# LeapLabTHU/LAUDNet

Hardware: AMD Instinct MI355X
Metric: images/sec, LAUD-ResNet101 @224 bs256 (dynamic-inference hot path) (higher is better)
Workload: dtype bf16x3 (fp32 tensors; each fp32 product = 3 bf16 MFMA products of hi/lo splits, fp32 accumulate)

## Files before the change

include/ldn_hip.h:

```cpp
#ifndef LDN_HIP_H
#define LDN_HIP_H

#include <stddef.h>
#include <stdint.h>

#ifdef __cplusplus
extern "C" {
#endif

#define LDN_OK 0
#define LDN_EINVAL (-1)
#define LDN_EHIP (-2)

const char* ldn_last_error(void);
int ldn_version(void);
int ldn_debug_violations(int* count, int* first_code, int reset);
int ldn_plan_timeouts(int* count, int reset);
const int* ldn_fault_flag(void);
int ldn_device_cus(int* cus);
#define LDN_MATH_DEFAULT (-1)
#define LDN_MATH_FP32 0
#define LDN_MATH_BF16X3 1
int ldn_default_math_mode(void);

int ldn_spatial_masker(const float* x, int B, int Hi, int Wi, int C, const float* w ,
                       const float* bias , int g, int S, float* mask, float* logits, float* work,
                       const int32_t* carry_prefix, const float* carry_mask, void* stream);
size_t ldn_spatial_masker_workspace_bytes(int B, int Hi, int Wi, int C, int S);

int ldn_mask_to_index(const float* patch_mask, int B, int Sy, int Sx, int Ho, int Wo, int stride, int32_t* idx3,
                      int32_t* pos3, int32_t* idx1, int32_t* pos1, int32_t* nbr, int32_t* cnt,
                      int32_t* img_prefix3, int32_t* img_prefix1, float* stats, int32_t* work, void* stream);
size_t ldn_mask_to_index_workspace_bytes(int B, int Ho, int Wo, int stride);
int ldn_plan_work_zeroed(int yes);
int ldn_coarsen_cell_means(const float* fine, int B, int S, int C, float* coarse, void* stream);

int ldn_layer_index(const float* image_mask, int B, int Ho, int Wo, int stride, int tile_gy, int tile_gx, int32_t* idx3,
                    int32_t* pos3, int32_t* idx1, int32_t* pos1, int32_t* nbr, int32_t* cnt, int32_t* img_prefix3,
                    int32_t* img_prefix1, float* stats, void* stream);
int ldn_layer_head(const float* pool, int B, int nparts, int C, const float* w , const float* bias , int g,
                   float* mask , float* logits , void* stream);
int ldn_mask_plan_fits(int S, int Sx, int Ho, int Wo, int stride);
int ldn_mask_plan(const float* patch_mask, const float* pool, int C, const float* w, const float* bias, float* mask_out,
                  float* logits, int B, int S, int Sx, int Ho, int Wo, int stride, int patch_major, int32_t* idx3,
                  int32_t* pos3, int32_t* idx1, int32_t* pos1, int32_t* nbr, int32_t* cnt, int32_t* img_prefix3,
                  int32_t* img_prefix1, float* stats, int32_t* work, void* stream);

int ldn_gather_rows(const float* src, int ld_src, const int32_t* rows, const int32_t* count, int cap, int C,
                    float* packed, int ld_packed, void* stream);
int ldn_scatter_add_relu(const float* packed, int ld_packed, const int32_t* rows, const int32_t* count, int cap,
                         int C, const float* identity, int ld_id, float* out, int ld_out, void* stream);

int ldn_conv_rows(const float* a, int lda, const int32_t* a_rows, int taps, const int32_t* m_count, int m_cap,
                  const float* w, int cin, int cout, const float* scale, const float* shift, int relu,
                  const int32_t* relu_if_neg, const int32_t* out_rows, const float* residual, int ldr,
                  float* out, int ldo, int math_mode, void* stream);

int ldn_conv_rows_split(const float* a, int lda, const int32_t* a_rows, int taps, const int32_t* m_count, int m_cap,
                        const void* w_split, int cin, int cout, const float* scale, const float* shift, int relu,
                        const int32_t* relu_if_neg, const int32_t* out_rows, const float* residual, int ldr, float* out,
                        int ldo, const float* post_sub, const float* chan_mask, int rows_per_image, int shift_classes,
                        const int32_t* pix_map, int Hi, int Wi, int Ho, int Wo, int stride, const float* ln_stats,
                        const float* ln_c1, void* stream);
int ldn_conv_rows_f32(const float* a, int lda, const int32_t* a_rows, int taps, const int32_t* m_count, int m_cap,
                        const float* w, int cin, int cout, const float* scale, const float* shift, int relu,
                        const int32_t* relu_if_neg, const int32_t* out_rows, const float* residual, int ldr, float* out,
                        int ldo, const float* post_sub, const float* chan_mask, int rows_per_image, int shift_classes,
                        const int32_t* pix_map, int Hi, int Wi, int Ho, int Wo, int stride, const float* ln_stats,
                        const float* ln_c1, void* stream);

int ldn_hint_rows(int rows);

int ldn_wgrad_rows_ok(int cin, int cout, int taps);
size_t ldn_wgrad_rows_workspace_bytes(int m_cap, int cin, int cout, int taps);
int ldn_wgrad_rows(const float* dy, int lddy, const float* a, int lda, int a_valid, const int32_t* a_rows, int taps,
                   const int32_t* m_count, int m_cap, int cin, int cout, float* dw, float* work, int math_mode, void* stream);

int ldn_wgrad_grouped_rows_ok(int C, int gw);
size_t ldn_wgrad_grouped_rows_workspace_bytes(int m_cap, int C, int gw);
int ldn_wgrad_grouped_rows(const float* dy, int lddy, const float* a, int lda, int a_valid, const int32_t* nbr, const int32_t* m_count,
                           int m_cap, int C, int gw, float* dw, float* work, int math_mode, void* stream);

int ldn_rows_chanmask(float* u, int ldu, const int32_t* row_prefix, int B, const float* chan_mask, const int32_t* m_count, int m_cap,
                      int C, void* stream);

size_t ldn_rows_act_bwd_workspace_bytes(int m_cap, int C, int B);
int ldn_rows_act_bwd(const float* dh, int lddh, const float* u, int ldu, const float* post_sub, const float* scale, const float* shift,
                     const float* chan_mask, const int32_t* row_prefix, int B, const float* zy, int ldzy, const int32_t* m_count,
                     int m_cap, int C, float* du, int lddu, float* g_shift, float* g_scale_num, float* g_mask, float* work,
                     void* stream);

int ldn_conv_rows_pool(const float* a, int lda, const int32_t* a_rows, const int32_t* m_count, int m_cap, const void* w,
                       int cin, int cout, const float* scale, const float* shift, int relu, const int32_t* relu_if_neg,
                       const int32_t* out_rows, const float* residual, int ldr, float* out, int ldo, float* pool, int S,
                       int Sx, int Ho, int Wo, int math_mode, void* stream);

int ldn_conv_rows_ps(const float* a, int lda, int a_presplit, const int32_t* a_rows, const int32_t* m_count, int m_cap,
                     const void* w_split, int cin, int cout, const float* scale, const float* shift, int relu,
                     const int32_t* relu_if_neg, const int32_t* out_rows, const float* residual, int ldr, float* out, int ldo,
                     int out_presplit, float* pool, int S, int Sx, int Ho, int Wo, void* stream);
int ldn_conv3x3_rows_ps(const void* a_presplit, int lda, const int32_t* nbr, const int32_t* m_count, int m_cap, const void* w_split,
                        int cin, int cout, const float* scale, const float* shift, int relu, void* out, int ldo, int out_presplit,
                        int rows_hint, void* stream);
int ldn_row_stats(const float* x, int ld, int rows, int C, float eps, float* stats, void* stream);
int ldn_row_stats_list(const float* x, int ld, int rows, int C, float eps, const int32_t* list, const int32_t* count, float* stats,
                       void* stream);

int ldn_channel_masker_splits(int HW);
int ldn_channel_masker(const float* x, int B, int HW, int C, const float* w1, const float* b1, const float* w2,
                       const float* b2, int hidden, int G, int gran, const float* mask_in, float* mask,
                       float* logits, int32_t* ch_idx, int32_t* ch_cnt, float* work, const float* gap_partial,
                       int gap_splits, void* stream);
size_t ldn_channel_masker_workspace_bytes(int B, int HW, int C);

int ldn_forward_stats(const int32_t* cnt, int B, const float* denom, const float* st_in, int st_cols, const double* terms,
                      double static_flops, int n_blocks, float* st_out, float* perc, float* flops, void* stream);

int ldn_conv_image(const float* a, int lda, int B, int Hi, int Wi, int ksize, int stride, int Ho, int Wo,
                   const float* w, int cin, int cout, const int32_t* k_idx, const int32_t* k_cnt, int kgran,
                   const int32_t* n_idx, const int32_t* n_cnt, const float* scale, const float* shift,
                   int shift_classes, const float* post_sub, int relu, const float* residual, int ldr,
                   float* out, int ldo, float* colsum, int out_format, int math_mode, void* stream);

int ldn_bottleneck_head(const float* x, int ldx, int B, int HW, int cin, const void* w1_split, int width,
                        const int32_t* ch_idx, const int32_t* ch_cnt, const float* scale1, const float* shift1,
                        const float* post_sub1, void* h1_split, int ldh, void* stream);
int ldn_bottleneck_head_f32(const float* x, int ldx, int B, int HW, int cin, const float* w1, int width,
                            const int32_t* ch_idx, const int32_t* ch_cnt, const float* scale1, const float* shift1,
                            const float* post_sub1, float* h1, int ldh, void* stream);
int ldn_bottleneck_tail_f32(const void* h1, int ldh, int B, int H, int Wd, int stride, int width, const void* w2_pairs_f32,
                            const void* w3_pairs_f32, int cout, const int32_t* ch_idx, const int32_t* ch_cnt, const float* scale2,
                            const float* shift2_tab, const float* post_sub2, const float* shift3, const float* residual,
                            int ldr, float* out, int ldo, float* colsum, void* stream);
int ldn_bottleneck_tail_splits(int H, int Wd, int width, int stride);
int ldn_bottleneck_tail(const void* h1_split, int ldh, int B, int H, int Wd, int stride, int width, const void* w2_pairs,
                        const void* w3_pairs, int cout, const int32_t* ch_idx, const int32_t* ch_cnt, const float* scale2,
                        const float* shift2_tab, const float* post_sub2, const float* shift3, const float* residual,
                        int ldr, float* out, int ldo, float* colsum, void* stream);
size_t ldn_x_split_bytes(size_t pixels, int cin);
int ldn_bottleneck_head_split(const float* x, int ldx, int B, int HW, int cin, const void* w1_split, int width,
                              const int32_t* ch_idx, const int32_t* ch_cnt, const float* scale1, const float* shift1,
                              const float* post_sub1, void* h1_split, int ldh, void* x_split, void* stream);
int ldn_bottleneck_tail_proj_fits(int H, int Wd, int width, int cin);
int ldn_bottleneck_tail_proj(const void* h1_split, int ldh, int B, int H, int Wd, int width, const void* w2_pairs,
                             const void* w3_pairs, int cout, const int32_t* ch_idx, const int32_t* ch_cnt, const float* scale2,
                             const float* shift2_tab, const float* post_sub2, const float* shift3d, const void* x_split,
                             int cin, const void* wd_pairs, float* out, int ldo, float* colsum, void* stream);

int ldn_bottleneck_smallmap_fits(int H, int Wd, int cin, int width, int cout);
int ldn_bottleneck_smallmap(const float* x, int ldx, int B, int H, int Wd, int cin, int width, const void* w1_split,
                            const void* w2_pairs, const void* w3_pairs, int cout, const int32_t* ch_idx, const int32_t* ch_cnt,
                            const float* scale1, const float* shift1, const float* post_sub1, const float* scale2,
                            const float* shift2_tab, const float* post_sub2, const float* shift3, const float* residual, int ldr,
                            float* out, int ldo, float* colsum, void* stream);

typedef struct ldn_chain_block {
    const void* w1_split; const float* scale1; const float* shift1; const float* post_sub1;
    const void* w2_pairs; const void* w3_pairs; const float* scale2; const float* shift2_tab; const float* post_sub2;
    const float* shift3;
    const float* mw1; const float* mb1; const float* mw2; const float* mb2;
} ldn_chain_block;
int ldn_bottleneck_chain_fits(int H, int Wd, int C, int width, int hidden, int G);
int ldn_bottleneck_chain(const float* x_in, float* x_work, int ldx, int B, int H, int Wd, int C, int width,
                         const ldn_chain_block* blocks, int nblocks, int hidden, int G, int gran, const float* gap_in,
                         int gap_splits, float* colsum, float* masks, int32_t* ch_idx, int32_t* ch_cnt, void* h1_split,
                         int ldh, void* stream);
int ldn_bottleneck_chain_f32(const float* x_in, float* x_work, int ldx, int B, int H, int Wd, int C, int width,
                         const ldn_chain_block* blocks, int nblocks, int hidden, int G, int gran, const float* gap_in,
                         int gap_splits, float* colsum, float* masks, int32_t* ch_idx, int32_t* ch_cnt, float* h1,
                         int ldh, void* stream);

size_t ldn_stem_weight_bytes(int cout);
int ldn_stem_conv_pool(const float* x, int B, int H, int W, const void* w_frag, const float* shift, int cout, float* out,
                       int Hp, int Wp, void* stream);
int ldn_stem_gap_splits(int H, int W);
int ldn_stem_conv_pool_gap(const float* x, int B, int H, int W, const void* w_frag, const float* shift, int cout,
                           float* out, int Hp, int Wp, float* gap, void* stream);

size_t ldn_stem3_weight_bytes(int cout);
int ldn_stem3_conv(const float* x, int B, int H, int W, const void* w_frag, const float* shift, int cout, int relu, float* out,
                   int Ho, int Wo, void* stream);

int ldn_conv_packed(const float* a, int lda, int B, const int32_t* row_prefix, const int32_t* m_count, int m_cap,
                    const int32_t* a_map, int taps, const int32_t* out_map, const int32_t* pix_map, int Hi, int Wi,
                    int Ho, int Wo, int stride, const float* w, int cin, int cout, const int32_t* k_idx,
                    const int32_t* k_cnt, int kgran, const int32_t* n_idx, const int32_t* n_cnt, const float* scale,
                    const float* shift, int shift_classes, const float* post_sub, int relu,
                    const int32_t* relu_if_neg, const float* residual, int ldr, float* out, int ldo, int math_mode,
                    void* stream);

int ldn_grouped_conv3x3_rows(const float* a, int lda, const int32_t* nbr, const int32_t* m_count, int m_cap,
                             const float* w, int C, int group_width, const float* scale, const float* shift, int relu,
                             float* out, int ldo, void* stream);
size_t ldn_grouped16_weight_bytes(int C);
int ldn_grouped16_conv3x3_rows(const float* a, int lda, const int32_t* nbr, const int32_t* m_count, int m_cap,
                               const void* w_frag, int C, const float* scale, const float* shift, int relu, float* out,
                               int ldo, void* stream);

int ldn_grouped16_images_fit(int Hi, int Wi, int C);
int ldn_grouped16_conv3x3_images(const float* a, int lda, const int32_t* m_count, int images_cap, int Hi, int Wi, int Ho, int Wo,
                                 int stride, const void* w_frag, int C, const float* scale, const float* shift, int relu, float* out,
                                 int ldo, void* stream);
int ldn_grouped_conv3x3_image(const float* a, int lda, int B, int Hi, int Wi, int stride, int Ho, int Wo, const float* w,
                              int C, int group_width, const int32_t* ch_idx, const int32_t* ch_cnt, const float* scale,
                              const float* shift, int relu, float* out, int ldo, void* stream);
int ldn_se_packed(float* a, int lda, const int32_t* row_prefix, int B, int C, int S, const float* w1, const float* b1,
                  const float* w2, const float* b2, const int32_t* ch_idx, const int32_t* ch_cnt, int max_rows_per_image,
                  float* work, void* stream);
size_t ldn_se_packed_workspace_bytes(int B, int C, int max_rows_per_image);

int ldn_grouped16_images_bands(int Hi, int Wi, int Ho, int stride, int C);
int ldn_grouped16_conv3x3_images_gap(const float* a, int lda, const int32_t* m_count, int images_cap, int Hi, int Wi, int Ho, int Wo,
                                     int stride, const void* w_frag, int C, const float* scale, const float* shift, int relu, float* out,
                                     int ldo, float* gap_partial, void* stream);
int ldn_se_gate_slots(const float* gap_partial, int splits, const int32_t* m_count, int images_cap, int rows_per_image, int C, int S,
                      const float* w1, const float* b1, const float* w2, const float* b2, float* gate, void* stream);
int ldn_conv_rows_gated(const float* a, int lda, const int32_t* m_count, int m_cap, const void* w_split, int cin, int cout,
                        const float* scale, const float* shift, int relu, const int32_t* relu_if_neg, const int32_t* out_rows,
                        const float* residual, int ldr, float* out, int ldo, const float* gate, int gate_rows, void* stream);

int ldn_packed_mha(const float* qkv, int ld_qkv, const int32_t* tok_rows, const int32_t* img_prefix, int B, int heads,
                   int head_dim, int max_tokens, float scale, float* out, int ldo, void* stream);
int ldn_packed_mha_heads(const float* qkv, int ld_qkv, const int32_t* tok_rows, const int32_t* img_prefix, int B, int heads,
                         int head_dim, int max_tokens, float scale, const float* head_keep, float* out, int ldo, void* stream);

#ifdef __cplusplus
}
#endif
#endif
```

laudnet_amd/_lib.py:

```python
from __future__ import annotations

import ctypes as C
import os

import torch

_PKG = os.path.dirname(os.path.abspath(__file__))
LIB_PATH = os.environ.get("LDN_LIB_PATH", os.path.join(_PKG, "libldn_hip.so"))

_P = C.c_void_p
_I = C.c_int

SIGNATURES = {
    "ldn_last_error": ([], C.c_char_p),
    "ldn_version": ([], _I),
    "ldn_debug_violations": ([C.POINTER(_I), C.POINTER(_I), _I], _I),
    "ldn_plan_timeouts": ([C.POINTER(_I), _I], _I),
    "ldn_fault_flag": ([], C.POINTER(_I)),
    "ldn_device_cus": ([C.POINTER(_I)], _I),
    "ldn_default_math_mode": ([], _I),
    "ldn_spatial_masker": ([_P, _I, _I, _I, _I, _P, _P, _I, _I, _P, _P, _P, _P, _P, _P], _I),
    "ldn_spatial_masker_workspace_bytes": ([_I, _I, _I, _I, _I], C.c_size_t),
    "ldn_mask_to_index": ([_P, _I, _I, _I, _I, _I, _I, _P, _P, _P, _P, _P, _P, _P, _P, _P, _P, _P], _I),
    "ldn_mask_to_index_workspace_bytes": ([_I, _I, _I, _I], C.c_size_t),
    "ldn_mask_plan_fits": ([_I, _I, _I, _I, _I], _I),
    "ldn_hint_rows": ([_I], _I),
    "ldn_layer_index": ([_P, _I, _I, _I, _I, _I, _I, _P, _P, _P, _P, _P, _P, _P, _P, _P, _P], _I),
    "ldn_layer_head": ([_P, _I, _I, _I, _P, _P, _I, _P, _P, _P], _I),
    "ldn_mask_plan": ([_P, _P, _I, _P, _P, _P, _P, _I, _I, _I, _I, _I, _I, _I, _P, _P, _P, _P, _P, _P, _P, _P, _P, _P, _P], _I),
    "ldn_conv_rows_pool": ([_P, _I, _P, _P, _I, _P, _I, _I, _P, _P, _I, _P, _P, _P, _I, _P, _I, _P, _I, _I, _I, _I, _I, _P], _I),
    "ldn_conv_rows_ps": ([_P, _I, _I, _P, _P, _I, _P, _I, _I, _P, _P, _I, _P, _P, _P, _I, _P, _I, _I, _P, _I, _I, _I, _I, _P], _I),
    "ldn_conv3x3_rows_ps": ([_P, _I, _P, _P, _I, _P, _I, _I, _P, _P, _I, _P, _I, _I, _I, _P], _I),
    "ldn_gather_rows": ([_P, _I, _P, _P, _I, _I, _P, _I, _P], _I),
    "ldn_scatter_add_relu": ([_P, _I, _P, _P, _I, _I, _P, _I, _P, _I, _P], _I),
    "ldn_conv_rows": ([_P, _I, _P, _I, _P, _I, _P, _I, _I, _P, _P, _I, _P, _P, _P, _I, _P, _I, _I, _P], _I),
    "ldn_conv_rows_split": ([_P, _I, _P, _I, _P, _I, _P, _I, _I, _P, _P, _I, _P, _P, _P, _I, _P, _I, _P, _P, _I, _I, _P, _I, _I, _I,
                             _I, _I, _P, _P, _P], _I),
    "ldn_conv_rows_f32": ([_P, _I, _P, _I, _P, _I, _P, _I, _I, _P, _P, _I, _P, _P, _P, _I, _P, _I, _P, _P, _I, _I, _P, _I, _I, _I,
                             _I, _I, _P, _P, _P], _I),
    "ldn_wgrad_rows_ok": ([_I, _I, _I], _I),
    "ldn_wgrad_rows_workspace_bytes": ([_I, _I, _I, _I], C.c_size_t),
    "ldn_wgrad_rows": ([_P, _I, _P, _I, _I, _P, _I, _P, _I, _I, _I, _P, _P, _I, _P], _I),
    "ldn_wgrad_grouped_rows_ok": ([_I, _I], _I),
    "ldn_wgrad_grouped_rows_workspace_bytes": ([_I, _I, _I], C.c_size_t),
    "ldn_wgrad_grouped_rows": ([_P, _I, _P, _I, _I, _P, _P, _I, _I, _I, _P, _P, _I, _P], _I),
    "ldn_rows_chanmask": ([_P, _I, _P, _I, _P, _P, _I, _I, _P], _I),
    "ldn_rows_act_bwd_workspace_bytes": ([_I, _I, _I], C.c_size_t),
    "ldn_rows_act_bwd": ([_P, _I, _P, _I, _P, _P, _P, _P, _P, _I, _P, _I, _P, _I, _I, _P, _I, _P, _P, _P, _P, _P], _I),
    "ldn_row_stats": ([_P, _I, _I, _I, C.c_float, _P, _P], _I),
    "ldn_row_stats_list": ([_P, _I, _I, _I, C.c_float, _P, _P, _P, _P], _I),
    "ldn_channel_masker_splits": ([_I], _I),
    "ldn_channel_masker": ([_P, _I, _I, _I, _P, _P, _P, _P, _I, _I, _I, _P, _P, _P, _P, _P, _P, _P, _I, _P], _I),
    "ldn_channel_masker_workspace_bytes": ([_I, _I, _I], C.c_size_t),
    "ldn_forward_stats": ([_P, _I, _P, _P, _I, _P, C.c_double, _I, _P, _P, _P, _P], _I),
    "ldn_conv_packed": ([_P, _I, _I, _P, _P, _I, _P, _I, _P, _P, _I, _I, _I, _I, _I, _P, _I, _I, _P, _P, _I, _P, _P, _P, _P,
                         _I, _P, _I, _P, _P, _I, _P, _I, _I, _P], _I),
    "ldn_grouped_conv3x3_rows": ([_P, _I, _P, _P, _I, _P, _I, _I, _P, _P, _I, _P, _I, _P], _I),
    "ldn_grouped16_weight_bytes": ([_I], C.c_size_t),
    "ldn_grouped16_conv3x3_rows": ([_P, _I, _P, _P, _I, _P, _I, _P, _P, _I, _P, _I, _P], _I),
    "ldn_grouped16_images_fit": ([_I, _I, _I], _I),
    "ldn_grouped16_conv3x3_images": ([_P, _I, _P, _I, _I, _I, _I, _I, _I, _P, _I, _P, _P, _I, _P, _I, _P], _I),
    "ldn_plan_work_zeroed": ([_I], _I),
    "ldn_coarsen_cell_means": ([_P, _I, _I, _I, _P, _P], _I),
    "ldn_grouped16_images_bands": ([_I, _I, _I, _I, _I], _I),
    "ldn_grouped16_conv3x3_images_gap": ([_P, _I, _P, _I, _I, _I, _I, _I, _I, _P, _I, _P, _P, _I, _P, _I, _P, _P], _I),
    "ldn_se_gate_slots": ([_P, _I, _P, _I, _I, _I, _I, _P, _P, _P, _P, _P, _P], _I),
    "ldn_conv_rows_gated": ([_P, _I, _P, _I, _P, _I, _I, _P, _P, _I, _P, _P, _P, _I, _P, _I, _P, _I, _P], _I),
    "ldn_grouped_conv3x3_image": ([_P, _I, _I, _I, _I, _I, _I, _I, _P, _I, _I, _P, _P, _P, _P, _I, _P, _I, _P], _I),
    "ldn_se_packed": ([_P, _I, _P, _I, _I, _I, _P, _P, _P, _P, _P, _P, _I, _P, _P], _I),
    "ldn_se_packed_workspace_bytes": ([_I, _I, _I], C.c_size_t),
    "ldn_conv_image": ([_P, _I, _I, _I, _I, _I, _I, _I, _I, _P, _I, _I, _P, _P, _I, _P, _P, _P, _P, _I, _P, _I,
                        _P, _I, _P, _I, _P, _I, _I, _P], _I),
    "ldn_bottleneck_head": ([_P, _I, _I, _I, _I, _P, _I, _P, _P, _P, _P, _P, _P, _I, _P], _I),
    "ldn_bottleneck_head_f32": ([_P, _I, _I, _I, _I, _P, _I, _P, _P, _P, _P, _P, _P, _I, _P], _I),
    "ldn_bottleneck_tail_splits": ([_I, _I, _I, _I], _I),
    "ldn_bottleneck_tail": ([_P, _I, _I, _I, _I, _I, _I, _P, _P, _I, _P, _P, _P, _P, _P, _P, _P, _I, _P, _I, _P, _P], _I),
    "ldn_bottleneck_tail_f32": ([_P, _I, _I, _I, _I, _I, _I, _P, _P, _I, _P, _P, _P, _P, _P, _P, _P, _I, _P, _I, _P, _P], _I),
    "ldn_x_split_bytes": ([C.c_size_t, _I], C.c_size_t),
    "ldn_bottleneck_head_split": ([_P, _I, _I, _I, _I, _P, _I, _P, _P, _P, _P, _P, _P, _I, _P, _P], _I),
    "ldn_bottleneck_tail_proj_fits": ([_I, _I, _I, _I], _I),
    "ldn_bottleneck_tail_proj": ([_P, _I, _I, _I, _I, _I, _P, _P, _I, _P, _P, _P, _P, _P, _P, _P, _I, _P, _P, _I, _P, _P], _I),
    "ldn_stem_weight_bytes": ([_I], C.c_size_t),
    "ldn_stem_conv_pool": ([_P, _I, _I, _I, _P, _P, _I, _P, _I, _I, _P], _I),
    "ldn_stem_gap_splits": ([_I, _I], _I),
    "ldn_stem_conv_pool_gap": ([_P, _I, _I, _I, _P, _P, _I, _P, _I, _I, _P, _P], _I),
    "ldn_stem3_weight_bytes": ([_I], C.c_size_t),
    "ldn_stem3_conv": ([_P, _I, _I, _I, _P, _P, _I, _I, _P, _I, _I, _P], _I),
    "ldn_packed_mha": ([_P, _I, _P, _P, _I, _I, _I, _I, C.c_float, _P, _I, _P], _I),
    "ldn_packed_mha_heads": ([_P, _I, _P, _P, _I, _I, _I, _I, C.c_float, _P, _P, _I, _P], _I),
    "ldn_bottleneck_chain_fits": ([_I, _I, _I, _I, _I, _I], _I),
    "ldn_bottleneck_smallmap_fits": ([_I, _I, _I, _I, _I], _I),
    "ldn_bottleneck_smallmap": ([_P, _I, _I, _I, _I, _I, _I, _P, _P, _P, _I, _P, _P, _P, _P, _P, _P, _P, _P, _P, _P, _I, _P, _I, _P, _P], _I),
    "ldn_bottleneck_chain": ([_P, _P, _I, _I, _I, _I, _I, _I, _P, _I, _I, _I, _I, _P, _I, _P, _P, _P, _P, _P, _I, _P], _I),
    "ldn_bottleneck_chain_f32": ([_P, _P, _I, _I, _I, _I, _I, _I, _P, _I, _I, _I, _I, _P, _I, _P, _P, _P, _P, _P, _I, _P], _I),
}

_lib = None


class LdnError(RuntimeError):
    pass


def load():
    global _lib
    if _lib is not None:
        return _lib
    if not os.path.exists(LIB_PATH):
        raise LdnError(f"{LIB_PATH} not found: build it with `python -m laudnet_amd.build` "
                       "(laudnet_amd has no CPU or PyTorch fallback for the hot path)")
    lib = C.CDLL(LIB_PATH)
    for name, (argtypes, restype) in SIGNATURES.items():
        fn = getattr(lib, name)
        fn.argtypes = argtypes
        fn.restype = restype
    _lib = lib
    return lib


def ptr(t):
    if t is None:
        return None
    return C.c_void_p(t.data_ptr())


def stream_ptr(t=None):
    return C.c_void_p(torch.cuda.current_stream(t.device if t is not None else None).cuda_stream)


_SYNC_CALLS = os.environ.get("LDN_SYNC_CALLS", "0") != "0"
_n_calls = 0


_fault = None


def _arm_fault_flag():
    global _fault
    if _fault is None:
        p = load().ldn_fault_flag()
        _fault = p if p else False


def check(status: int, what: str, fault_ok: bool = False):
    if status != 0:
        msg = load().ldn_last_error()
        raise LdnError(f"{what} failed ({status}): {msg.decode() if msg else '?'}")
    if _fault and not fault_ok and _fault[0] != 0:
        raise LdnError(f"{what}: a device-side bounded wait ran into its time bound since the last reset -- results computed since are "
                       "invalid (ops.plan_timeouts() counts the events, ops.plan_timeouts(reset=True) re-arms)")
    if _SYNC_CALLS:
        global _n_calls
        import sys
        import torch
        _n_calls += 1
        print(f"[ldn] {_n_calls} {what} ...", end="", file=sys.stderr, flush=True)
        if torch.cuda.is_current_stream_capturing():
            print(" (capturing)", file=sys.stderr, flush=True)
            return
        torch.cuda.synchronize()
        print(" ok", file=sys.stderr, flush=True)


def require_device(*tensors):
    cur = None
    for t in tensors:
        if t is None:
            continue
        if not t.is_cuda:
            raise LdnError("laudnet_amd ops need tensors on a HIP device (cuda:N); there is no CPU path")
        if cur is None:
            cur = torch.cuda.current_device()
            if _fault is None:
                _arm_fault_flag()
        if t.device.index != cur:
            raise LdnError(f"tensor on {t.device} but the current device is cuda:{cur}: wrap the call in "
                           f"torch.cuda.device({t.device.index}) (kernels are launched on the current device's stream)")
```

laudnet_amd/csrc/ldn_chain_ld.h:

```cpp
#pragma once
#include "ldn_common.h"

namespace ldn {

#ifndef LDN_LD_PRIO
#define LDN_LD_PRIO 0
#endif
#ifndef LDN_LD_R2MAX
#define LDN_LD_R2MAX 4
#endif
#ifndef LDN_LD3_ABLATE
#define LDN_LD3_ABLATE 0
#endif
#ifndef LDN_LD3_DEFER
#define LDN_LD3_DEFER 0
#endif
#ifndef LDN_LD3_STORE_STEP
#define LDN_LD3_STORE_STEP 1
#endif
#ifndef LDN_LD2_STAGED
#define LDN_LD2_STAGED 0
#endif
#ifndef LDN_LD3_STAGED
#define LDN_LD3_STAGED 1
#endif

constexpr int LD_SYNC_OFF = T_KIDX_BYTES;
constexpr int LD_SYNC_BYTES = 256;
constexpr int LD_LOADER = 7;
constexpr int LD_SPIN_LIMIT = 1 << 20;

__device__ unsigned g_ld_stalls = 0u;
__device__ int* g_ld_fault_dev = nullptr;
#ifdef LDN_TRACE
__device__ unsigned long long* g_ld_trace = nullptr;
#define LT(x) x = __builtin_amdgcn_s_memtime();
#define LD_TIMED(slot, stmt) { const unsigned long long t0_ = __builtin_amdgcn_s_memtime(); stmt; q.t[slot] += __builtin_amdgcn_s_memtime() - t0_; }
#define LD_SPAN(slot, a, b) q.t[slot] += (b) - (a);
#else
#define LT(x)
#define LD_TIMED(slot, stmt) { stmt; }
#define LD_SPAN(slot, a, b)
#endif

struct LdSync {
    unsigned landed;
    unsigned pad0[15];
    unsigned done[16];
    unsigned pad1[32];
};
static_assert(sizeof(LdSync) == LD_SYNC_BYTES, "LdSync layout");

struct LdSeq {
    unsigned base;
    unsigned seen;
#ifdef LDN_TRACE
    unsigned long long t[8];
#endif
};

__device__ __forceinline__ unsigned ld_lds_read(const unsigned* p) {
    unsigned v;
    asm volatile("ds_read_b32 %0, %1\n\ts_waitcnt lgkmcnt(0)" : "=&v"(v) : "v"(lds_off(p)) : "memory");
    return v;
}
__device__ __forceinline__ void ld_lds_write(unsigned* p, unsigned v) {
    asm volatile("ds_write_b32 %0, %1\n\ts_nop 0" ::"v"(lds_off(p)), "v"(v) : "memory");
}

__device__ __forceinline__ void ld_wait_landed(LdSync* sy, unsigned need, unsigned& seen) {
    if (seen >= need) return;
    for (int spin = 0;; ++spin) {
        seen = __builtin_amdgcn_readfirstlane(ld_lds_read(&sy->landed));
        if (seen >= need) break;
        if (spin >= LD_SPIN_LIMIT) {
            if ((threadIdx.x & 63) == 0) {
                atomicAdd(&g_ld_stalls, 1u);
                if (g_ld_fault_dev) __hip_atomic_store(g_ld_fault_dev, 1, __ATOMIC_RELAXED, __HIP_MEMORY_SCOPE_SYSTEM);
            }
            seen = 0x7fffffffu;
            break;
        }
        __builtin_amdgcn_s_sleep(2);
    }
}
__device__ __forceinline__ void ld_post_done(LdSync* sy, int wave, unsigned seq_plus_1) {
    asm volatile("" ::: "memory");
    if ((threadIdx.x & 63) == 0) ld_lds_write(&sy->done[wave], seq_plus_1);
    asm volatile("" ::: "memory");
}
__device__ __forceinline__ void ld_wait_done(LdSync* sy, int ncomp, unsigned need, bool& dead) {
    if (dead) return;
    const int lane = threadIdx.x & 63;
    for (int spin = 0;; ++spin) {
        const unsigned v = ld_lds_read(&sy->done[lane & 15]);
        if (__ballot(lane < ncomp && v < need) == 0ull) break;
        if (spin >= LD_SPIN_LIMIT) {
            if (lane == 0) {
                atomicAdd(&g_ld_stalls, 1u);
                if (g_ld_fault_dev) __hip_atomic_store(g_ld_fault_dev, 1, __ATOMIC_RELAXED, __HIP_MEMORY_SCOPE_SYSTEM);
            }
            dead = true;
            break;
        }
        __builtin_amdgcn_s_sleep(2);
    }
}
#ifdef LDN_DEBUG
__device__ int g_chain_stall = -1;
#endif
__device__ __forceinline__ void ld_publish(LdSync* sy, unsigned landed) {
#ifdef LDN_DEBUG
    if ((int)blockIdx.x == g_chain_stall) return;
#endif
    asm volatile("" ::: "memory");
    if ((threadIdx.x & 63) == 0) ld_lds_write(&sy->landed, landed);
    asm volatile("" ::: "memory");
}


__device__ __forceinline__ u32x4 ld_global16(const unsigned char* sbase, unsigned off) {
    typedef const __attribute__((address_space(1))) u32x4* gptr;
    return *(gptr)(sbase + off);
}

__device__ __forceinline__ f32x4 ld_global_f4(const float* ptr) {
    typedef const __attribute__((address_space(1))) f32x4* gptr;
    return *(gptr)(ptr);
}

__device__ __forceinline__ unsigned ld_bias(int i) { return (unsigned)(3 - (i & 3)) * 1024u; }
template <int MAXP>
__device__ __forceinline__ void ld_dma_run(const unsigned (&vo)[MAXP], int n, const unsigned char* sbase, unsigned lds_base) {
    const void* sb = uniform_ptr(sbase - 3072);
#pragma unroll
    for (int g = 0; g < MAXP / 4; ++g) {
        if (4 * g >= n) break;
        const unsigned v4[4] = {vo[4 * g], vo[4 * g + 1], vo[4 * g + 2], vo[4 * g + 3]};
        dma16_pieces_abl<4>(v4, sb, (unsigned)__builtin_amdgcn_readfirstlane((int)(lds_base + (unsigned)g * 4096u)));
    }
}

template <int NS>
__device__ __forceinline__ void head_ld(const HeadArgs& p, const int b, unsigned char* const smem, const int lds_total, const int tid, LdSeq& q) {
    constexpr int W = NS * 32;
    constexpr int MAXP = NS * 4;
    int* const s_nidx = reinterpret_cast<int*>(smem);
    LdSync* const sy = reinterpret_cast<LdSync*>(smem + LD_SYNC_OFF);
    float* const s_tab = reinterpret_cast<float*>(smem + LD_SYNC_OFF + LD_SYNC_BYTES);
    unsigned char* const s_ring = smem + LD_SYNC_OFF + LD_SYNC_BYTES + 3 * W * 4;

    const int lane = tid & 63;
    const int wave = __builtin_amdgcn_readfirstlane(tid >> 6);
    const int l31 = lane & 31, h = lane >> 5;
    const int npix = p.HW;
    const long row0 = (long)b * p.HW;
    const int ncomp = ceil_div(npix, 32);

    const int Nb = min(p.n_cnt[b], W);
    const int nsub = __builtin_amdgcn_readfirstlane(ceil_div(Nb, 32));
    const int nwp = __builtin_amdgcn_readfirstlane(4 * max(nsub, 1));
    const int wslot = nwp * 1024;
    if (tid < W + 32) s_nidx[tid] = tid < Nb ? p.n_idx[(size_t)b * W + tid] : -1;
    if (tid < LD_SYNC_BYTES / 4) reinterpret_cast<unsigned*>(sy)[tid] = 0u;
    __syncthreads();
    for (int i = tid; i < 3 * W; i += 512) {
        const int k = i / W, n = i - k * W;
        const int ch = s_nidx[n];
        const float* src = k == 0 ? p.sc1 : (k == 1 ? p.sh1 : p.ps1);
        s_tab[i] = ch >= 0 ? src[ch] : 0.f;
    }
    const int avail = lds_total - (LD_SYNC_OFF + LD_SYNC_BYTES + 3 * W * 4);
    int DX = 3;
    if ((avail - ncomp * DX * 4096) / wslot < 3) DX = 2;
    DX = __builtin_amdgcn_readfirstlane(DX);
    const int RW = __builtin_amdgcn_readfirstlane(min(4, (avail - ncomp * DX * 4096) / wslot));
    unsigned char* const s_x = s_ring + RW * wslot;
    const int nchunks = p.cin / 32;
    const unsigned base = q.base;
    q.base = base + (unsigned)nchunks;
#ifdef LDN_TRACE
    unsigned long long ta, tb, tc;
    LT(ta)
#endif

    if (wave == LD_LOADER) {
        if (nsub == 0) return;
        unsigned wo[MAXP];
#pragma unroll
        for (int i = 0; i < MAXP; ++i) {
            const int rw = 8 * i + (lane >> 3);
            const int ch = s_nidx[min(rw, max(Nb, 1) - 1)];
            wo[i] = (unsigned)(max(ch, 0) * p.cin * 4 + (((lane & 7) ^ ((rw >> 1) & 7)) << 4)) + ld_bias(i);
        }
        const unsigned lds_w = lds_off(s_ring);
        bool dead = false;
        int slot = 0;
        for (int c = 0; c < nchunks; ++c) {
            if (c >= RW) LD_TIMED(5, ld_wait_done(sy, ncomp, base + (unsigned)(c - RW + 1), dead))
            ld_dma_run<MAXP>(wo, nwp, p.w1s + (long)c * 128, lds_w + (unsigned)slot * (unsigned)wslot);
            slot = slot + 1 == RW ? 0 : slot + 1;
            if (c > 0) { wait_vm_rt<62, 63>(nwp); ld_publish(sy, base + (unsigned)c); }
        }
        wait_vm<0>();
        ld_publish(sy, base + (unsigned)nchunks);
        LT(tb)
        LD_SPAN(0, ta, tb)
        return;
    }
    if (wave >= ncomp) return;

    const unsigned lds_x = lds_off(s_x) + (unsigned)wave * (unsigned)(DX * 4096);
    unsigned char* const my_x = s_x + wave * DX * 4096;
    unsigned xo[4];
#pragma unroll
    for (int i = 0; i < 4; ++i) {
        const int rl = 8 * i + (lane >> 3);
        const int r = wave * 32 + rl;
        xo[i] = (unsigned)((min(r, npix - 1) * p.ldx) * 4 + (((lane & 7) ^ ((rl >> 1) & 7)) << 4)) + ld_bias(i);
    }
    const unsigned char* const xbase = reinterpret_cast<const unsigned char*>(p.x + row0 * p.ldx) - 3072;
    auto dma_x = [&](int c, int xs) {
        const int cc = min(c, nchunks - 1);
        dma16_pieces_abl<4>(xo, uniform_ptr(xbase + (long)cc * 128), (unsigned)__builtin_amdgcn_readfirstlane((int)(lds_x + (unsigned)xs * 4096u)));
    };

    f32x16 acc[NS];
#pragma unroll
    for (int j = 0; j < NS; ++j)
#pragma unroll
        for (int r = 0; r < 16; ++r) acc[j][r] = 0.f;

    if (nsub == 0) return;
    for (int c = 0; c < DX - 1; ++c) dma_x(c, c);
    const unsigned xsw = ((unsigned)l31 >> 1) & 7u;
    bf16x8 bh[2], bl[2];
    int xs = 0, ws_i = 0;
    for (int c = 0; c < nchunks; ++c) {
        wait_vm_rt<15, 16>(4 * (DX - 2));
        {
            const unsigned char* xsl = my_x + xs * 4096 + l31 * 128;
#pragma unroll
            for (int half = 0; half < 2; ++half) {
                const unsigned sl = 4u * half + 2u * h;
                const f32x4 x0 = *reinterpret_cast<const f32x4*>(xsl + ((sl ^ xsw) << 4));
                const f32x4 x1 = *reinterpret_cast<const f32x4*>(xsl + (((sl + 1) ^ xsw) << 4));
#pragma unroll
                for (int e = 0; e < 8; ++e) {
                    const float v = e < 4 ? x0[e] : x1[e - 4];
                    const __bf16 hb = (__bf16)v;
                    bh[half][e] = hb;
                    bl[half][e] = (__bf16)(v - (float)hb);
                }
            }
        }
        dma_x(c + DX - 1, xs == 0 ? DX - 1 : xs - 1);
        LD_TIMED(5, ld_wait_landed(sy, base + (unsigned)c + 1u, q.seen))
        const unsigned char* ws = s_ring + ws_i * wslot + l31 * 128;
        bf16x8 a0h, a0l, a1h, a1l;
        const unsigned sl0 = 2u * h, sl1 = 4u + 2u * h;
        auto frag0 = [&](int j) {
            a0h = *reinterpret_cast<const bf16x8*>(ws + j * 4096 + ((sl0 ^ xsw) << 4));
            a0l = *reinterpret_cast<const bf16x8*>(ws + j * 4096 + (((sl0 + 1) ^ xsw) << 4));
        };
        auto frag1 = [&](int j) {
            a1h = *reinterpret_cast<const bf16x8*>(ws + j * 4096 + ((sl1 ^ xsw) << 4));
            a1l = *reinterpret_cast<const bf16x8*>(ws + j * 4096 + (((sl1 + 1) ^ xsw) << 4));
        };
#define LDN_HEADLD_STEP(J)                                                                                \
        frag1(J);                                                                                         \
        __builtin_amdgcn_sched_barrier(0);                                                                \
        LDN_K16(false, acc[J], a0h, a0l, bh[0], bl[0])                                                    \
        __builtin_amdgcn_sched_barrier(0);                                                                \
        if (J > 0) frag0(J > 0 ? J - 1 : 0);                                                              \
        __builtin_amdgcn_sched_barrier(0);                                                                \
        LDN_K16(false, acc[J], a1h, a1l, bh[1], bl[1])                                                    \
        __builtin_amdgcn_sched_barrier(0);
        if (nsub > 0) {
            frag0(nsub - 1);
            switch (nsub) {
                default:
                    if constexpr (NS >= 8) { LDN_HEADLD_STEP(7) }
                    [[fallthrough]];
                case 7:
                    if constexpr (NS >= 8) { LDN_HEADLD_STEP(6) }
                    [[fallthrough]];
                case 6:
                    if constexpr (NS >= 8) { LDN_HEADLD_STEP(5) }
                    [[fallthrough]];
                case 5:
                    if constexpr (NS >= 8) { LDN_HEADLD_STEP(4) }
                    [[fallthrough]];
                case 4:
                    if constexpr (NS >= 4) { LDN_HEADLD_STEP(3) }
                    [[fallthrough]];
                case 3:
                    if constexpr (NS >= 4) { LDN_HEADLD_STEP(2) }
                    [[fallthrough]];
                case 2:
                    LDN_HEADLD_STEP(1)
                    [[fallthrough]];
                case 1:
                    LDN_HEADLD_STEP(0)
            }
        }
#undef LDN_HEADLD_STEP
        ld_post_done(sy, wave, base + (unsigned)c + 1u);
        xs = xs + 1 == DX ? 0 : xs + 1;
        ws_i = ws_i + 1 == RW ? 0 : ws_i + 1;
    }
    wait_vm<0>();
    LT(tb)
    LD_SPAN(0, ta, tb)

    const int pm = wave * 32 + l31;
    unsigned char* orow = p.h1 + (row0 + min(pm, npix - 1)) * p.h1_row_bytes;
#pragma unroll
    for (int j = 0; j < NS; ++j) {
        if (j >= nsub) continue;
#pragma unroll
        for (int q4 = 0; q4 < 4; ++q4) {
            const int n0 = 32 * j + 8 * q4 + 4 * h;
            const f32x4 sc = *reinterpret_cast<const f32x4*>(s_tab + n0);
            const f32x4 sh = *reinterpret_cast<const f32x4*>(s_tab + W + n0);
            const f32x4 ps = *reinterpret_cast<const f32x4*>(s_tab + 2 * W + n0);
            unsigned hi2[2], lo2[2];
#pragma unroll
            for (int d = 0; d < 2; ++d) {
                const float v0 = fmaxf(acc[j][4 * q4 + 2 * d] * sc[2 * d] + sh[2 * d], 0.f) - ps[2 * d];
                const float v1 = fmaxf(acc[j][4 * q4 + 2 * d + 1] * sc[2 * d + 1] + sh[2 * d + 1], 0.f) - ps[2 * d + 1];
                const bf16x2 hh = {(__bf16)v0, (__bf16)v1};
                const bf16x2 ll = {(__bf16)(v0 - (float)hh[0]), (__bf16)(v1 - (float)hh[1])};
                hi2[d] = __builtin_bit_cast(unsigned, hh);
                lo2[d] = __builtin_bit_cast(unsigned, ll);
            }
            u32x4 outv;
#pragma unroll
            for (int d = 0; d < 2; ++d) {
                const auto r = __builtin_amdgcn_permlane32_swap(hi2[d], lo2[d], false, false);
                outv[d] = r[0];
                outv[2 + d] = r[1];
            }
            if (pm < npix) *reinterpret_cast<u32x4*>(orow + (4 * j + q4) * 32 + h * 16) = outv;
        }
    }
    LT(tc)
    LD_SPAN(1, tb, tc)
}

constexpr int LD_CW = 32;
template <int NS>
__device__ __forceinline__ void tail_ld(const TailArgs& p, const int b, unsigned char* const smem, const int lds_total, const int tid, LdSeq& q) {
    constexpr int W = NS * 32;
    constexpr int MAXP = NS * 4;
    constexpr int MAXH = 28;
    constexpr int NP = W;
    constexpr int W3_ROW = LD_CW * 8;
    int* const s_kidx = reinterpret_cast<int*>(smem);
    LdSync* const sy = reinterpret_cast<LdSync*>(smem + LD_SYNC_OFF);
    unsigned char* const s_lo = smem + LD_SYNC_OFF + LD_SYNC_BYTES;
    unsigned char* const s_h1 = s_lo;
    unsigned char* const s_w2 = s_h1 + 2 * p.slice_bytes;
    unsigned char* const s_w3 = s_lo;
    unsigned char* const s_scr = smem + lds_total - 7 * 4096;
    float* const s_tab = reinterpret_cast<float*>(s_scr - 18 * NP * 4);

    int lane = tid & 63;
    const int wave = __builtin_amdgcn_readfirstlane(tid >> 6);
    int l31 = lane & 31, h = lane >> 5;
    const int npix = p.Ho * p.Wo;
    const int ncomp = ceil_div(npix, 32);
    const int NR = npix, NRp = round_up(NR, 8);
    const int ZR = NRp;
    const long pix0 = (long)b * npix;

    const int Kb = min(p.k_cnt[b], W);
    const int nsub = __builtin_amdgcn_readfirstlane(ceil_div(Kb, 32));
    const int Kp = nsub * 32;
    const int P2 = __builtin_amdgcn_readfirstlane(Kp / 8);
    const int slot2 = Kp * 128, slot3 = Kp * 128;
    if (tid < W + 32) s_kidx[tid] = tid < Kb ? p.k_idx[(size_t)b * W + tid] : -1;
    if (tid < 64) reinterpret_cast<float*>(s_h1 + (tid >> 5) * p.slice_bytes + ZR * 128)[tid & 31] = 0.f;
    __syncthreads();

    const int avail2 = lds_total - (LD_SYNC_OFF + LD_SYNC_BYTES) - 2 * p.slice_bytes;
    const int R2 = __builtin_amdgcn_readfirstlane(nsub > 0 ? min(LDN_LD_R2MAX, avail2 / slot2) : LDN_LD_R2MAX);
    const int avail3 = lds_total - (LD_SYNC_OFF + LD_SYNC_BYTES) - 18 * NP * 4 - 7 * 4096;
    const int R3 = __builtin_amdgcn_readfirstlane(nsub > 0 ? min(4, avail3 / slot3) : 4);
    const int nchunks = nsub * 9;
    const int nchunk3 = p.cout / LD_CW;
    const int nq = NRp / 8;
    const unsigned base2 = q.base, base3 = base2 + (unsigned)nchunks;
    q.base = base3 + (unsigned)nchunk3;
    constexpr int TMIN = 3;
    static_assert(TMIN == 3 && MAXH == 28, "the slice schedule below is written out for taps 3 .. 8 and <= 28 pieces");

    const bool loader = wave == LD_LOADER;
    const bool consumer = wave < ncomp;
#ifdef LDN_TRACE
    unsigned long long ta, tb, tc, td;
    LT(ta)
#endif
    bool dead = false;

    f32x16 acc[NS];
    if (loader) {
#if LDN_LD2_STAGED
        constexpr int NH = NS / 2;
        const int nhi = (nsub + 1) / 2;
        unsigned colo[NH];
        unsigned dsto[NH];
        const int hp = max(Kp / 2, 1);
#pragma unroll
        for (int i = 0; i < NH; ++i) {
            const int e = 64 * i + lane;
            const int gh = e / hp, v = e - gh * hp;
            const int ch = 2 * v < Kb ? s_kidx[2 * v] : 0;
            colo[i] = (unsigned)((ch >> 1) * 16);
            dsto[i] = gh < 2 ? ((unsigned)(gh * Kp * 32 + v * 32) | (unsigned)gh) : ~0u;
        }
        unsigned ro[2][NH][4];
        auto slice_rows = [&](int s_) {
#pragma unroll
            for (int hf = 0; hf < 2; ++hf)
#pragma unroll
                for (int i = 0; i < NH; ++i) {
                    const int gh = (int)(dsto[i] & 1u);
#pragma unroll
                    for (int qq = 0; qq < 4; ++qq) {
                        const int kch = s_kidx[32 * s_ + 2 * (8 * hf + 4 * gh + qq)];
                        ro[hf][i][qq] = (unsigned)((max(kch, 0) >> 1) * (W / 2) * 16) + colo[i];
                    }
                }
        };
        u32x4 LA[NH][4], LB[NH][4];
        auto load_half = [&](int t_, int hf, u32x4 (&L_)[NH][4]) {
            const unsigned char* src = reinterpret_cast<const unsigned char*>(uniform_ptr(p.w2p + (long)t_ * ((W / 2) * (W / 2) * 16)));
#pragma unroll
            for (int i = 0; i < NH; ++i)
                if (i < nhi)
#pragma unroll
                    for (int qq = 0; qq < 4; ++qq) L_[i][qq] = ld_global16(src, ro[hf][i][qq]);
        };
        auto store_half = [&](unsigned char* slotp, int hf, const u32x4 (&L_)[NH][4]) {
            const int lo = Kp * 16;
            unsigned char* hb = slotp + hf * (Kp * 64);
#pragma unroll
            for (int i = 0; i < NH; ++i)
                if (i < nhi && dsto[i] != ~0u) {
                    unsigned char* d = hb + (dsto[i] & ~31u);
                    *reinterpret_cast<u32x4*>(d) = u32x4{L_[i][0][0], L_[i][1][0], L_[i][2][0], L_[i][3][0]};
                    *reinterpret_cast<u32x4*>(d + lo) = u32x4{L_[i][0][1], L_[i][1][1], L_[i][2][1], L_[i][3][1]};
                    *reinterpret_cast<u32x4*>(d + 16) = u32x4{L_[i][0][2], L_[i][1][2], L_[i][2][2], L_[i][3][2]};
                    *reinterpret_cast<u32x4*>(d + lo + 16) = u32x4{L_[i][0][3], L_[i][1][3], L_[i][2][3], L_[i][3][3]};
                }
        };
        const unsigned lds_h1 = lds_off(s_h1);
        const unsigned char* const h1b = p.h1 + pix0 * p.h1_row_bytes;
        auto h1_piece = [&](int i, const void* sb, unsigned dst) {
            const int r = 8 * i + (lane >> 3);
            const unsigned o = (unsigned)(min(r, NR - 1) * (int)p.h1_row_bytes + (((lane & 7) ^ ((r >> 1) & 7)) << 4));
            dma16_pieces<1>({o}, sb, (unsigned)__builtin_amdgcn_readfirstlane((int)(dst + (unsigned)i * 1024u)));
        };
        if (nchunks > 0) {
            const void* sb0 = uniform_ptr(h1b);
            for (int i = 0; i < nq; ++i) h1_piece(i, sb0, lds_h1);
            slice_rows(0);
            load_half(0, 0, LA);
            load_half(0, 1, LB);
        }
        int slot = 0;
        int sn = 0, tn = 1;
        for (int c = 0; c < nchunks; ++c) {
            const int sc = c / 9, tc = c - 9 * sc;
            const bool nxt = c + 1 < nchunks;
            if (c >= R2) LD_TIMED(6, ld_wait_done(sy, ncomp, base2 + (unsigned)(c - R2 + 1), dead))
            if (tc == 0) wait_vm<0>();
            unsigned char* const slotp = s_w2 + slot * slot2;
            slot = slot + 1 == R2 ? 0 : slot + 1;
            store_half(slotp, 0, LA);
            if (nxt) {
                if (tn == 0) slice_rows(sn);
                load_half(tn, 0, LA);
            }
            store_half(slotp, 1, LB);
            ld_publish(sy, base2 + (unsigned)c + 1u);
            if (nxt) load_half(tn, 1, LB);
            if (tc >= TMIN && sc + 1 < nsub) {
                const void* hsb = uniform_ptr(h1b + (long)(sc + 1) * 128);
                const unsigned hdst = lds_h1 + (unsigned)((sc + 1) & 1) * (unsigned)p.slice_bytes;
                for (int i = tc - TMIN; i < nq; i += 6) h1_piece(i, hsb, hdst);
            }
            if (++tn == 9) { tn = 0; ++sn; }
        }
#else
        unsigned ho[MAXH];
#pragma unroll
        for (int i = 0; i < MAXH; ++i) {
            const int r = 8 * i + (lane >> 3);
            ho[i] = (unsigned)(min(r, NR - 1) * (int)p.h1_row_bytes + (((lane & 7) ^ ((r >> 1) & 7)) << 4));
        }
        unsigned un[MAXP];
        unsigned no[MAXP];
        const int hp = max(Kp / 2, 1);
#pragma unroll
        for (int i = 0; i < MAXP; ++i) {
            const int e = 64 * i + lane;
            const int u = min(e / hp, 15), v = e - (e / hp) * hp;
            const int ch = 2 * v < Kb ? s_kidx[2 * v] : 0;
            un[i] = (unsigned)u;
            no[i] = (unsigned)((ch >> 1) * 16) + ld_bias(i);
        }
        const unsigned lds_h1 = lds_off(s_h1), lds_w2 = lds_off(s_w2);
        const unsigned char* const h1b = p.h1 + pix0 * p.h1_row_bytes;
        if (nchunks > 0) {
#pragma unroll
            for (int i = 0; i < MAXH; ++i)
                if (i < nq) dma16_pieces<1>({ho[i]}, uniform_ptr(h1b), (unsigned)__builtin_amdgcn_readfirstlane((int)(lds_h1 + (unsigned)i * 1024u)));
        }
        int slot = 0;
        for (int s = 0; s < nsub; ++s) {
            unsigned vo[MAXP];
#pragma unroll
            for (int i = 0; i < MAXP; ++i) {
                const int kch = s_kidx[32 * s + 2 * (int)un[i]];
                vo[i] = (unsigned)((max(kch, 0) >> 1) * (W / 2) * 16) + no[i];
            }
            const unsigned char* const hsrc = h1b + (long)(s + 1) * 128;
            const unsigned hdst = lds_h1 + (unsigned)((s + 1) & 1) * (unsigned)p.slice_bytes;
            const bool more = s + 1 < nsub;
            for (int t = 0; t < 9; ++t) {
                const int c = 9 * s + t;
                if (c >= R2) LD_TIMED(6, ld_wait_done(sy, ncomp, base2 + (unsigned)(c - R2 + 1), dead))
                ld_dma_run<MAXP>(vo, P2, p.w2p + (long)t * ((W / 2) * (W / 2) * 16), lds_w2 + (unsigned)slot * (unsigned)slot2);
                slot = slot + 1 == R2 ? 0 : slot + 1;
                int pieces = P2;
                if (t >= TMIN && more) {
                    const void* hsb = uniform_ptr(hsrc);
#define LDN_LD_H1(I) if ((I) < nq) { dma16_pieces<1>({ho[(I)]}, hsb, (unsigned)__builtin_amdgcn_readfirstlane((int)(hdst + (unsigned)(I) * 1024u))); ++pieces; }
                    switch (t) {
                        case 3: LDN_LD_H1(0) LDN_LD_H1(6) LDN_LD_H1(12) LDN_LD_H1(18) LDN_LD_H1(24) break;
                        case 4: LDN_LD_H1(1) LDN_LD_H1(7) LDN_LD_H1(13) LDN_LD_H1(19) LDN_LD_H1(25) break;
                        case 5: LDN_LD_H1(2) LDN_LD_H1(8) LDN_LD_H1(14) LDN_LD_H1(20) LDN_LD_H1(26) break;
                        case 6: LDN_LD_H1(3) LDN_LD_H1(9) LDN_LD_H1(15) LDN_LD_H1(21) LDN_LD_H1(27) break;
                        case 7: LDN_LD_H1(4) LDN_LD_H1(10) LDN_LD_H1(16) LDN_LD_H1(22) break;
                        default: LDN_LD_H1(5) LDN_LD_H1(11) LDN_LD_H1(17) LDN_LD_H1(23) break;
                    }
#undef LDN_LD_H1
                }
                if (c > 0) { wait_vm_rt<62, 63>(pieces); ld_publish(sy, base2 + (unsigned)c); }
            }
        }
#endif
        wait_vm<0>();
        ld_publish(sy, base2 + (unsigned)nchunks);
        LT(tb)
        LD_SPAN(2, ta, tb)
        __syncthreads();
#if LDN_LD3_STAGED
        unsigned so[NS][4];
#pragma unroll
        for (int i = 0; i < NS; ++i)
#pragma unroll
            for (int qq = 0; qq < 4; ++qq) {
                const int u = 16 * i + 8 * ((lane >> 5) & 1) + 2 * ((lane >> 4) & 1) + (qq & 1) + 4 * (qq >> 1);
                const int kch = 2 * u < Kp ? s_kidx[2 * u] : -1;
                so[i][qq] = (unsigned)(((long)(max(kch, 0) >> 1) * p.cout + 2 * (lane & 15)) * 8);
            }
        u32x4 L[NS][4];
        auto load_chunk = [&](int cc) {
            const unsigned char* src = reinterpret_cast<const unsigned char*>(uniform_ptr(p.w3p + (long)cc * (LD_CW * 8)));
#pragma unroll
            for (int i = 0; i < NS; ++i)
                if (i < nsub)
#pragma unroll
                    for (int qq = 0; qq < 4; ++qq) L[i][qq] = ld_global16(src, so[i][qq]);
        };
        auto store_chunk = [&](unsigned char* slotp) {
#pragma unroll
            for (int i = 0; i < NS; ++i)
                if (i < nsub) {
                    unsigned char* d = slotp + (4 * i + (lane >> 4)) * 1024 + (lane & 15) * 32;
                    *reinterpret_cast<u32x4*>(d) = u32x4{L[i][0][0], L[i][1][0], L[i][2][0], L[i][3][0]};
                    *reinterpret_cast<u32x4*>(d + 512) = u32x4{L[i][0][1], L[i][1][1], L[i][2][1], L[i][3][1]};
                    *reinterpret_cast<u32x4*>(d + 16) = u32x4{L[i][0][2], L[i][1][2], L[i][2][2], L[i][3][2]};
                    *reinterpret_cast<u32x4*>(d + 528) = u32x4{L[i][0][3], L[i][1][3], L[i][2][3], L[i][3][3]};
                }
        };
        if (nchunk3 > 0 && nsub > 0) load_chunk(0);
        __syncthreads();
        if (nsub > 0) {
            int slot3i = 0;
            for (int cc = 0; cc < nchunk3; ++cc) {
                if (cc >= R3) LD_TIMED(7, ld_wait_done(sy, ncomp, base3 + (unsigned)(cc - R3 + 1), dead))
                store_chunk(s_w3 + slot3i * slot3);
                slot3i = slot3i + 1 == R3 ? 0 : slot3i + 1;
                ld_publish(sy, base3 + (unsigned)cc + 1u);
                if (cc + 1 < nchunk3) load_chunk(cc + 1);
            }
        }
#else
        const unsigned lds_w3 = lds_off(s_w3);
        unsigned w3o[MAXP];
#pragma unroll
        for (int i = 0; i < MAXP; ++i) {
            const int u = 4 * i + (lane >> 4);
            const int kch = 2 * u < Kp ? s_kidx[2 * u] : -1;
            w3o[i] = (unsigned)(((long)(max(kch, 0) >> 1) * p.cout + 2 * (lane & 15)) * 8) + ld_bias(i);
        }
        if (nchunk3 > 0 && nsub > 0) ld_dma_run<MAXP>(w3o, P2, p.w3p, lds_w3);
        __syncthreads();
        if (nsub > 0) {
            int slot3i = 1 == R3 ? 0 : 1;
            for (int cc = 1; cc < nchunk3; ++cc) {
                if (cc >= R3) LD_TIMED(7, ld_wait_done(sy, ncomp, base3 + (unsigned)(cc - R3 + 1), dead))
                ld_dma_run<MAXP>(w3o, P2, p.w3p + (long)cc * (LD_CW * 8), lds_w3 + (unsigned)slot3i * (unsigned)slot3);
                slot3i = slot3i + 1 == R3 ? 0 : slot3i + 1;
                wait_vm_rt<62, 63>(P2);
                ld_publish(sy, base3 + (unsigned)cc);
            }
            wait_vm<0>();
        }
#endif
        ld_publish(sy, base3 + (unsigned)nchunk3);
        LT(tc)
        LD_SPAN(4, tb, tc)
        return;
    }

    const int pm = wave * 32 + l31;
    const bool pvalid = pm < npix;
    const int oy = pm / p.Wo, ox = pm % p.Wo;
    const int cls = (((oy - 1 < 0) | ((oy + 1 >= p.Hi) << 1)) * 4 + ((ox - 1 < 0) | ((ox + 1 >= p.Wi) << 1)));
    if (consumer) {
#pragma unroll
        for (int j = 0; j < NS; ++j)
#pragma unroll
            for (int r = 0; r < 16; ++r) acc[j][r] = 0.f;
        int trow[9];
#pragma unroll
        for (int t = 0; t < 9; ++t) {
            const int iy = oy + t / 3 - 1, ix = ox + t % 3 - 1;
            const bool ok = pvalid && iy >= 0 && iy < p.Hi && ix >= 0 && ix < p.Wi;
            trow[t] = ok ? iy * p.Wi + ix : ZR;
        }
        const unsigned RL = (unsigned)Kp * 8u;
        unsigned arow[8];
#pragma unroll
        for (int i = 0; i < 8; ++i) arow[i] = (unsigned)(4 * h + (i & 3) + 8 * (i >> 2)) * RL + (unsigned)l31 * 8u;
        unsigned bq[4];
#pragma unroll
        for (int i = 0; i < 4; ++i) bq[i] = (unsigned)((2 * (i >> 1) + h) * Kp * 32 + (i & 1) * Kp * 16 + l31 * 16);
#ifndef LDN_LD2_STYLE
#define LDN_LD2_STYLE 1
#endif
#ifndef LDN_LD_ABLATE
#define LDN_LD_ABLATE 0
#endif
#if LDN_LD_ABLATE & 2
#define LD_ABL_RD(PTR_, I_) (u32x2{(unsigned)(I_) + (unsigned)l31, (unsigned)(I_) * 3u + (unsigned)h})
#else
#define LD_ABL_RD(PTR_, I_) (*reinterpret_cast<const u32x2*>(PTR_))
#endif
#if LDN_LD_ABLATE & 1
#define LD_ABL_HI(E_) (u32x4{E_[0][0], E_[0][1], E_[1][0], E_[1][1]})
#define LD_ABL_LO(E_) (u32x4{E_[2][0], E_[2][1], E_[3][0], E_[3][1]})
#else
#define LD_ABL_HI(E_) (u32x4{E_[0][0], E_[1][0], E_[2][0], E_[3][0]})
#define LD_ABL_LO(E_) (u32x4{E_[0][1], E_[1][1], E_[2][1], E_[3][1]})
#endif
#if LDN_LD_ABLATE & 4
#define LD_ABL_K16(ACC_, AH_, AL_, BH_, BL_) asm volatile("" ::"v"(AH_), "v"(AL_), "v"(BH_), "v"(BL_));
#else
#define LD_ABL_K16(ACC_, AH_, AL_, BH_, BL_) LDN_K16(false, ACC_, AH_, AL_, BH_, BL_)
#endif
#if LDN_LD2_STYLE == 1
        int slot = 0;
        for (int s = 0; s < nsub; ++s) {
            const unsigned char* hs = s_h1 + (s & 1) * p.slice_bytes;
#pragma unroll
            for (int t = 0; t < 9; ++t) {
                const int c = 9 * s + t;
                LD_TIMED(6, ld_wait_landed(sy, base2 + (unsigned)c + 1u, q.seen))
                const unsigned char* ws = s_w2 + slot * slot2;
                slot = slot + 1 == R2 ? 0 : slot + 1;
                {
                    const unsigned rbase = (unsigned)trow[t] * 128u, rx = ((unsigned)trow[t] >> 1) & 7u;
                    bf16x8 bh[2], bl[2];
#pragma unroll
                    for (int half = 0; half < 2; ++half) {
                        const unsigned sl = 2u * (2u * half + h);
                        bh[half] = *reinterpret_cast<const bf16x8*>(hs + rbase + ((sl ^ rx) << 4));
                        bl[half] = *reinterpret_cast<const bf16x8*>(hs + rbase + (((sl + 1) ^ rx) << 4));
                    }
#if LDN_LD2_STAGED
#pragma unroll
                    for (int j = 0; j < NS; ++j) {
                        if (j < nsub) {
                            const bf16x8 ah0 = *reinterpret_cast<const bf16x8*>(ws + bq[0] + j * 512);
                            const bf16x8 al0 = *reinterpret_cast<const bf16x8*>(ws + bq[1] + j * 512);
                            const bf16x8 ah1 = *reinterpret_cast<const bf16x8*>(ws + bq[2] + j * 512);
                            const bf16x8 al1 = *reinterpret_cast<const bf16x8*>(ws + bq[3] + j * 512);
                            LDN_K16(false, acc[j], ah0, al0, bh[0], bl[0])
                            LDN_K16(false, acc[j], ah1, al1, bh[1], bl[1])
                            __builtin_amdgcn_sched_group_barrier(0x100, 4, 0);
                            __builtin_amdgcn_sched_group_barrier(0x008, 6, 0);
                        }
                    }
                }
#else
#pragma unroll
                    for (int j = 0; j < NS; ++j) {
                        if (j < nsub) {
                            u32x2 e0[4], e1[4];
#pragma unroll
                            for (int qq = 0; qq < 4; ++qq) e0[qq] = LD_ABL_RD(ws + arow[qq] + j * 256, qq);
#pragma unroll
                            for (int qq = 0; qq < 4; ++qq) e1[qq] = LD_ABL_RD(ws + arow[4 + qq] + j * 256, 4 + qq);
                            {
                                const u32x4 ahu = LD_ABL_HI(e0);
                                const u32x4 alu = LD_ABL_LO(e0);
                                const bf16x8 ah = __builtin_bit_cast(bf16x8, ahu), al = __builtin_bit_cast(bf16x8, alu);
                                LD_ABL_K16(acc[j], ah, al, bh[0], bl[0])
                            }
                            {
                                const u32x4 ahu = LD_ABL_HI(e1);
                                const u32x4 alu = LD_ABL_LO(e1);
                                const bf16x8 ah = __builtin_bit_cast(bf16x8, ahu), al = __builtin_bit_cast(bf16x8, alu);
                                LD_ABL_K16(acc[j], ah, al, bh[1], bl[1])
                            }
                            __builtin_amdgcn_sched_group_barrier(0x100, 8, 0);
                            __builtin_amdgcn_sched_group_barrier(0x008, 6, 0);
                        }
                    }
                }
#endif
                ld_post_done(sy, wave, base2 + (unsigned)c + 1u);
            }
        }
#else
        struct Ent { u32x2 e0[4], e1[4]; };
        bf16x8 bh[2], bl[2];
        Ent cur;
        auto rdB = [&](const unsigned char* hs_, int tr, bf16x8 (&dh)[2], bf16x8 (&dl)[2]) {
            asm volatile("" : "+v"(tr));
            const unsigned rbase = (unsigned)tr * 128u, rx = ((unsigned)tr >> 1) & 7u;
#pragma unroll
            for (int half = 0; half < 2; ++half) {
                const unsigned sl = 2u * (2u * half + h);
                dh[half] = *reinterpret_cast<const bf16x8*>(hs_ + rbase + ((sl ^ rx) << 4));
                dl[half] = *reinterpret_cast<const bf16x8*>(hs_ + rbase + (((sl + 1) ^ rx) << 4));
            }
        };
        auto rdBh = [&](const unsigned char* hs_, int tr, int half, bf16x8& dh, bf16x8& dl) {
            asm volatile("" : "+v"(tr));
            const unsigned rbase = (unsigned)tr * 128u, rx = ((unsigned)tr >> 1) & 7u;
            const unsigned sl = 2u * (2u * half + h);
            dh = *reinterpret_cast<const bf16x8*>(hs_ + rbase + ((sl ^ rx) << 4));
            dl = *reinterpret_cast<const bf16x8*>(hs_ + rbase + (((sl + 1) ^ rx) << 4));
        };
        auto rdE = [&](const unsigned char* ws_, int j, Ent& d) {
#pragma unroll
            for (int qq = 0; qq < 4; ++qq) d.e0[qq] = *reinterpret_cast<const u32x2*>(ws_ + arow[qq] + j * 256);
#pragma unroll
            for (int qq = 0; qq < 4; ++qq) d.e1[qq] = *reinterpret_cast<const u32x2*>(ws_ + arow[4 + qq] + j * 256);
        };
#define LDN_LD2_ASM(E_, AH_, AL_)                                                                         \
            const bf16x8 AH_ = __builtin_bit_cast(bf16x8, (u32x4{E_[0][0], E_[1][0], E_[2][0], E_[3][0]})); \
            const bf16x8 AL_ = __builtin_bit_cast(bf16x8, (u32x4{E_[0][1], E_[1][1], E_[2][1], E_[3][1]}));
#define LDN_LD2_STEP(J) {                                                                                 \
            Ent nxt;                                                                                      \
            rdE(ws, J - 1, nxt);                                                                          \
            __builtin_amdgcn_sched_barrier(0);                                                            \
            { LDN_LD2_ASM(cur.e0, ah0, al0) LDN_LD2_ASM(cur.e1, ah1, al1)                                 \
              LDN_K16(false, acc[J], ah0, al0, bh[0], bl[0])                                              \
              LDN_K16(false, acc[J], ah1, al1, bh[1], bl[1]) }                                            \
            __builtin_amdgcn_sched_barrier(0);                                                            \
            cur = nxt; }
        int slot = 0;
        const unsigned char* ws = s_w2;
        bool pre = false;
        for (int s = 0; s < nsub; ++s) {
            const unsigned char* hs = s_h1 + (s & 1) * p.slice_bytes;
#pragma unroll
            for (int t = 0; t < 9; ++t) {
                const int c = 9 * s + t;
                if (!pre) {
                    LD_TIMED(6, ld_wait_landed(sy, base2 + (unsigned)c + 1u, q.seen))
                    rdB(hs, trow[t], bh, bl);
                    rdE(ws, nsub - 1, cur);
                }
                slot = slot + 1 == R2 ? 0 : slot + 1;
                const unsigned char* wsn = s_w2 + slot * slot2;
                const unsigned char* hsn = t == 8 ? s_h1 + ((s + 1) & 1) * p.slice_bytes : hs;
                const int trn = trow[(t + 1) % 9];
                switch (nsub) {
                    default:
                        if constexpr (NS >= 8) LDN_LD2_STEP(7)
                        [[fallthrough]];
                    case 7:
                        if constexpr (NS >= 8) LDN_LD2_STEP(6)
                        [[fallthrough]];
                    case 6:
                        if constexpr (NS >= 8) LDN_LD2_STEP(5)
                        [[fallthrough]];
                    case 5:
                        if constexpr (NS >= 8) LDN_LD2_STEP(4)
                        [[fallthrough]];
                    case 4:
                        if constexpr (NS >= 4) LDN_LD2_STEP(3)
                        [[fallthrough]];
                    case 3:
                        if constexpr (NS >= 4) LDN_LD2_STEP(2)
                        [[fallthrough]];
                    case 2:
                        LDN_LD2_STEP(1)
                        [[fallthrough]];
                    case 1: {
                        LDN_LD2_ASM(cur.e0, ah0, al0) LDN_LD2_ASM(cur.e1, ah1, al1)
                        __builtin_amdgcn_sched_barrier(0);
                        pre = false;
                        if (c + 1 < nchunks) {
                            const unsigned need = base2 + (unsigned)c + 2u;
                            if (q.seen < need) q.seen = __builtin_amdgcn_readfirstlane(ld_lds_read(&sy->landed));
                            pre = q.seen >= need;
                        }
                        if (pre) rdE(wsn, nsub - 1, cur);
                        __builtin_amdgcn_sched_barrier(0);
                        LDN_K16(false, acc[0], ah0, al0, bh[0], bl[0])
                        __builtin_amdgcn_sched_barrier(0);
                        if (pre) rdBh(hsn, trn, 0, bh[0], bl[0]);
                        __builtin_amdgcn_sched_barrier(0);
                        LDN_K16(false, acc[0], ah1, al1, bh[1], bl[1])
                        __builtin_amdgcn_sched_barrier(0);
                        if (pre) rdBh(hsn, trn, 1, bh[1], bl[1]);
                    }
                }
                ld_post_done(sy, wave, base2 + (unsigned)c + 1u);
                ws = wsn;
            }
        }
#undef LDN_LD2_ASM
#undef LDN_LD2_STEP
#endif
    }
    LT(tb)
    LD_SPAN(2, ta, tb)
    __syncthreads();
    asm volatile("" : "+v"(lane));
    l31 = lane & 31;
    h = lane >> 5;

    {
        const int t7 = tid;
        constexpr int TB = 5;
        for (int i = t7; i < NP; i += 448) {
            const int ch = i < Kb ? s_kidx[i] : -1;
            const float a = p.sc2[max(ch, 0)], c = p.ps2[max(ch, 0)];
            s_tab[i] = ch >= 0 ? a : 0.f;
            s_tab[NP + i] = ch >= 0 ? c : 0.f;
        }
        for (int i0 = t7; i0 < 16 * NP; i0 += 448 * TB) {
            float v[TB];
#pragma unroll
            for (int u = 0; u < TB; ++u) {
                const int i = min(i0 + 448 * u, 16 * NP - 1);
                const int k = i / NP, n = i - k * NP;
                const int ch = n < Kb ? s_kidx[n] : -1;
                const float x = p.sh2[k * W + max(ch, 0)];
                v[u] = ch >= 0 ? x : 0.f;
            }
#pragma unroll
            for (int u = 0; u < TB; ++u)
                if (i0 + 448 * u < 16 * NP) s_tab[2 * NP + i0 + 448 * u] = v[u];
        }
    }
    __syncthreads();

    if (!consumer) return;

#pragma unroll
    for (int j = 0; j < NS; ++j) {
        float v[16];
#pragma unroll
        for (int q4 = 0; q4 < 4; ++q4) {
            const int n0 = 32 * j + 8 * q4 + 4 * h;
            const f32x4 sc = *reinterpret_cast<const f32x4*>(s_tab + n0);
            const f32x4 ps = *reinterpret_cast<const f32x4*>(s_tab + NP + n0);
            const f32x4 sh = *reinterpret_cast<const f32x4*>(s_tab + 2 * NP + cls * NP + n0);
#pragma unroll
            for (int e = 0; e < 4; ++e)
                v[4 * q4 + e] = fmaxf(acc[j][4 * q4 + e] * sc[e] + sh[e], 0.f) - ps[e];
        }
#pragma unroll
        for (int t = 0; t < 2; ++t)
#pragma unroll
            for (int d = 0; d < 4; ++d) {
                const float x0 = v[8 * t + 2 * d], x1 = v[8 * t + 2 * d + 1];
                const bf16x2 hi = {(__bf16)x0, (__bf16)x1};
                const bf16x2 lo = {(__bf16)(x0 - (float)hi[0]), (__bf16)(x1 - (float)hi[1])};
                acc[j][8 * t + d] = __builtin_bit_cast(float, hi);
                acc[j][8 * t + 4 + d] = __builtin_bit_cast(float, lo);
            }
        asm volatile("" : "+v"(acc[j]) :: "memory");
        __builtin_amdgcn_sched_barrier(0);
    }
    auto frag_hi = [&](int j, int t) -> bf16x8 {
        const f32x4 x = {acc[j][8 * t], acc[j][8 * t + 1], acc[j][8 * t + 2], acc[j][8 * t + 3]};
        return __builtin_bit_cast(bf16x8, x);
    };
    auto frag_lo = [&](int j, int t) -> bf16x8 {
        const f32x4 x = {acc[j][8 * t + 4], acc[j][8 * t + 5], acc[j][8 * t + 6], acc[j][8 * t + 7]};
        return __builtin_bit_cast(bf16x8, x);
    };

    LT(tc)
    LD_SPAN(3, tb, tc)
    const int trw = lane >> 3, tcq = lane & 7;
    const unsigned a3_lane = (unsigned)(2 * h * W3_ROW + l31 * 8);
    const unsigned a3q = (unsigned)(h * 1024 + l31 * 16);
    float* const scr = reinterpret_cast<float*>(s_scr + wave * 4096);
#if LDN_LD3_DEFER && LDN_LD3_STAGED
    int slot = 0;
    f32x4 res[4], xr[4], sh;
    int c0p = 0;
    auto epi_read = [&]() {
        __builtin_amdgcn_wave_barrier();
#pragma unroll
        for (int it = 0; it < 4; ++it) {
            const int row = trw + 8 * it;
            xr[it] = *reinterpret_cast<const f32x4*>(scr + row * 32 + ((tcq ^ (row & 7)) << 2));
        }
    };
    auto epi_store = [&]() {
        wait_vm<0>();
        asm volatile("" : "+v"(res[0]), "+v"(res[1]), "+v"(res[2]), "+v"(res[3]), "+v"(sh));
        f32x4 csum = {0.f, 0.f, 0.f, 0.f};
#pragma unroll
        for (int it = 0; it < 4; ++it) {
            const int prow = wave * 32 + trw + 8 * it;
            f32x4 x = xr[it] + sh + res[it];
#pragma unroll
            for (int e = 0; e < 4; ++e) x[e] = fmaxf(x[e], 0.f);
            if (prow < npix) {
                __builtin_nontemporal_store(x, reinterpret_cast<f32x4*>(p.out + (size_t)(pix0 + prow) * p.ldo + c0p + tcq * 4));
                csum += x;
            }
        }
        xr[0] = csum;
    };
    auto epi_gap = [&]() {
        if (p.colsum) {
            f32x4 csum = xr[0];
#pragma unroll
            for (int e = 0; e < 4; ++e) csum[e] = sum_lane_bits_345(csum[e]);
            if (trw == 0) *reinterpret_cast<f32x4*>(p.colsum + ((size_t)b * 8 + wave) * p.cout + c0p + tcq * 4) = csum;
        }
    };
    for (int cc = 0; cc < nchunk3; ++cc) {
        const int c0 = cc * LD_CW;
        const bool pend = cc > 0;
        f32x16 acc3;
#pragma unroll
        for (int r = 0; r < 16; ++r) acc3[r] = 0.f;
        LD_TIMED(7, ld_wait_landed(sy, base3 + (unsigned)cc + 1u, q.seen))
        const unsigned char* ws = s_w3 + slot * slot3;
        slot = slot + 1 == R3 ? 0 : slot + 1;
        const int js = min(LDN_LD3_STORE_STEP, nsub - 1), jg = min(js + 1, nsub - 1);
        bool todo = pend;
#pragma unroll
        for (int j = 0; j < NS; ++j) {
            if (j < nsub) {
                bf16x8 ah[2], al[2];
#pragma unroll
                for (int t = 0; t < 2; ++t) {
                    ah[t] = *reinterpret_cast<const bf16x8*>(ws + a3q + (4 * j + 2 * t) * 1024);
                    al[t] = *reinterpret_cast<const bf16x8*>(ws + a3q + (4 * j + 2 * t) * 1024 + 512);
                }
#pragma unroll
                for (int t = 0; t < 2; ++t) {
                    const bf16x8 hb = frag_hi(j, t), lb = frag_lo(j, t);
                    LDN_K16(false, acc3, ah[t], al[t], hb, lb)
                }
                __builtin_amdgcn_sched_group_barrier(0x100, 4, 0);
                __builtin_amdgcn_sched_group_barrier(0x008, 6, 0);
                if (pend) {
                    if (j == 0) epi_read();
                    if (j == js) epi_store();
                    if (j == jg) { epi_gap(); todo = false; }
                }
            }
        }
        if (todo) { epi_read(); epi_store(); epi_gap(); }
        ld_post_done(sy, wave, base3 + (unsigned)cc + 1u);
        __builtin_amdgcn_wave_barrier();
#pragma unroll
        for (int q4 = 0; q4 < 4; ++q4) {
            const f32x4 v = {acc3[4 * q4], acc3[4 * q4 + 1], acc3[4 * q4 + 2], acc3[4 * q4 + 3]};
            *reinterpret_cast<f32x4*>(scr + l31 * 32 + (((2 * q4 + h) ^ (l31 & 7)) << 2)) = v;
        }
#pragma unroll
        for (int it = 0; it < 4; ++it) {
            const int prow = wave * 32 + trw + 8 * it;
            const float* src = (p.residual && prow < npix) ? p.residual + (size_t)(pix0 + prow) * p.ldr + c0 + tcq * 4 : g_tail_zero;
            res[it] = __builtin_nontemporal_load(reinterpret_cast<const f32x4*>(src));
        }
        sh = ld_global_f4(p.sh3 + c0 + tcq * 4);
        c0p = c0;
    }
    if (nchunk3 > 0) { epi_read(); epi_store(); epi_gap(); }
#else
    int slot = 0;
    for (int cc = 0; cc < nchunk3; ++cc) {
        const int c0 = cc * LD_CW;
        f32x4 res[4];
#pragma unroll
        for (int it = 0; it < 4; ++it) {
            const int prow = wave * 32 + trw + 8 * it;
            const float* src = (p.residual && prow < npix) ? p.residual + (size_t)(pix0 + prow) * p.ldr + c0 + tcq * 4 : g_tail_zero;
#if LDN_LD3_ABLATE & 3
            res[it] = f32x4{(float)prow, 0.f, 1.f, 2.f};
#else
            res[it] = __builtin_nontemporal_load(reinterpret_cast<const f32x4*>(src));
#endif
        }
        f32x4 sh = ld_global_f4(p.sh3 + c0 + tcq * 4);
        f32x16 acc3;
#pragma unroll
        for (int r = 0; r < 16; ++r) acc3[r] = 0.f;
        LD_TIMED(7, ld_wait_landed(sy, base3 + (unsigned)cc + 1u, q.seen))
        const unsigned char* ws = s_w3 + slot * slot3;
        slot = slot + 1 == R3 ? 0 : slot + 1;
#if LDN_LD3_STAGED
#pragma unroll
        for (int j = 0; j < NS; ++j) {
            if (j < nsub) {
                bf16x8 ah[2], al[2];
#pragma unroll
                for (int t = 0; t < 2; ++t) {
                    ah[t] = *reinterpret_cast<const bf16x8*>(ws + a3q + (4 * j + 2 * t) * 1024);
                    al[t] = *reinterpret_cast<const bf16x8*>(ws + a3q + (4 * j + 2 * t) * 1024 + 512);
                }
#pragma unroll
                for (int t = 0; t < 2; ++t) {
                    const bf16x8 hb = frag_hi(j, t), lb = frag_lo(j, t);
#if LDN_LD3_ABLATE & 4
                    asm volatile("" :: "v"(ah[t]), "v"(al[t]), "v"(hb), "v"(lb));
#else
                    LDN_K16(false, acc3, ah[t], al[t], hb, lb)
#endif
                }
                __builtin_amdgcn_sched_group_barrier(0x100, 4, 0);
                __builtin_amdgcn_sched_group_barrier(0x008, 6, 0);
            }
        }
#else
#pragma unroll
        for (int j = 0; j < NS; ++j) {
            if (j < nsub) {
                u32x2 e[2][4];
#pragma unroll
                for (int t = 0; t < 2; ++t)
#pragma unroll
                    for (int qq = 0; qq < 4; ++qq)
                        e[t][qq] = *reinterpret_cast<const u32x2*>(ws + a3_lane + (16 * j + 8 * t + (qq & 1) + 4 * (qq >> 1)) * W3_ROW);
#pragma unroll
                for (int t = 0; t < 2; ++t) {
                    const u32x4 ahu = {e[t][0][0], e[t][1][0], e[t][2][0], e[t][3][0]};
                    const u32x4 alu = {e[t][0][1], e[t][1][1], e[t][2][1], e[t][3][1]};
                    const bf16x8 ah = __builtin_bit_cast(bf16x8, ahu), al = __builtin_bit_cast(bf16x8, alu);
                    const bf16x8 hb = frag_hi(j, t), lb = frag_lo(j, t);
                    LDN_K16(false, acc3, ah, al, hb, lb)
                }
                __builtin_amdgcn_sched_group_barrier(0x100, 8, 0);
                __builtin_amdgcn_sched_group_barrier(0x008, 6, 0);
            }
        }
#endif
        ld_post_done(sy, wave, base3 + (unsigned)cc + 1u);
#if LDN_LD3_ABLATE & 1
        asm volatile("" :: "v"(acc3), "v"(res[0]), "v"(res[3]), "v"(sh));
        continue;
#endif
        wait_vm<0>();
        asm volatile("" : "+v"(res[0]), "+v"(res[1]), "+v"(res[2]), "+v"(res[3]), "+v"(sh));
#pragma unroll
        for (int q4 = 0; q4 < 4; ++q4) {
            const f32x4 v = {acc3[4 * q4], acc3[4 * q4 + 1], acc3[4 * q4 + 2], acc3[4 * q4 + 3]};
            *reinterpret_cast<f32x4*>(scr + l31 * 32 + (((2 * q4 + h) ^ (l31 & 7)) << 2)) = v;
        }
        asm volatile("s_waitcnt lgkmcnt(0)" ::: "memory");
        __builtin_amdgcn_wave_barrier();
        f32x4 csum = {0.f, 0.f, 0.f, 0.f};
#pragma unroll
        for (int it = 0; it < 4; ++it) {
            const int row = trw + 8 * it, prow = wave * 32 + row;
            f32x4 x = *reinterpret_cast<const f32x4*>(scr + row * 32 + ((tcq ^ (row & 7)) << 2));
            x = x + sh + res[it];
#pragma unroll
            for (int e = 0; e < 4; ++e) x[e] = fmaxf(x[e], 0.f);
            if (prow < npix) {
#if !(LDN_LD3_ABLATE & 2)
                __builtin_nontemporal_store(x, reinterpret_cast<f32x4*>(p.out + (size_t)(pix0 + prow) * p.ldo + c0 + tcq * 4));
#endif
                csum += x;
            }
        }
        if (p.colsum) {
#pragma unroll
            for (int e = 0; e < 4; ++e) csum[e] = sum_lane_bits_345(csum[e]);
            if (trw == 0) *reinterpret_cast<f32x4*>(p.colsum + ((size_t)b * 8 + wave) * p.cout + c0 + tcq * 4) = csum;
        }
        asm volatile("s_waitcnt lgkmcnt(0)" ::: "memory");
        __builtin_amdgcn_wave_barrier();
    }
#endif
    LT(td)
    LD_SPAN(4, tc, td)
}

template <int NS>
__global__ __launch_bounds__(512, 2) void k_chain_ld(const ChainArgs p) {
    constexpr int W = NS * 32;
    extern __shared__ __attribute__((aligned(16))) unsigned char smem[];
    const int b = blockIdx.x;
    const int HW = p.H * p.Wd;
    {
        const int wave = threadIdx.x >> 6, lane = threadIdx.x & 63;
        if (wave >= ceil_div(HW, 32))
            for (int c = lane * 4; c < p.C; c += 256)
                *reinterpret_cast<f32x4*>(p.colsum + ((size_t)b * 8 + wave) * p.C + c) = f32x4{0.f, 0.f, 0.f, 0.f};
    }
#if LDN_LD_PRIO
    {
        const int w = __builtin_amdgcn_readfirstlane(threadIdx.x >> 6);
        if (w == LD_LOADER) __builtin_amdgcn_s_setprio(3);
        else if (w >= 4) __builtin_amdgcn_s_setprio(LDN_LD_PRIO);
    }
#endif
    LdSeq q;
#ifdef LDN_TRACE
    for (int k = 0; k < 8; ++k) q.t[k] = 0;
    unsigned long long c0, c1, c2, c3, c4, c5, c6, am = 0, ah = 0, at = 0, af = 0;
#endif
    for (int i = 0; i < p.nblocks; ++i) {
        CT(c0)
        const ChainBlock* cb = p.blocks + i;
        float* const mask_i = p.masks + (size_t)i * p.B * p.G;
        int32_t* const idx_i = p.ch_idx + (size_t)i * p.B * W;
        int32_t* const cnt_i = p.ch_cnt + (size_t)i * p.B;
        const float* const xin = i == 0 ? p.x_in : p.x_work;
        {
            float* const s_f = reinterpret_cast<float*>(smem);
            int* const s_w = reinterpret_cast<int*>(s_f + p.C + (p.hidden > 0 ? p.hidden : 1) + 2 * p.G);
            channel_mlp_body<512>(b, i == 0 ? p.gap_in : p.colsum, HW, p.C, i == 0 ? p.gap_splits : 8, uniform_ptr(cb->mw1),
                                  uniform_ptr(cb->mb1), uniform_ptr(cb->mw2), uniform_ptr(cb->mb2), p.hidden, p.G, p.gran, nullptr,
                                  mask_i, nullptr, idx_i, cnt_i, s_f, s_w, nullptr, true);
        }
        CT(c1)
        phase_fence();
        CT(c2)
        q.base = 0u;
        q.seen = 0u;
        {
            HeadArgs ha;
            ha.x = xin; ha.ldx = p.ldx; ha.B = p.B; ha.HW = HW; ha.cin = p.C; ha.W = W;
            ha.w1s = uniform_ptr(cb->w1s); ha.n_idx = idx_i; ha.n_cnt = cnt_i;
            ha.sc1 = uniform_ptr(cb->sc1); ha.sh1 = uniform_ptr(cb->sh1); ha.ps1 = uniform_ptr(cb->ps1);
            ha.h1 = p.h1; ha.h1_row_bytes = p.h1_row_bytes; ha.pix_per_blk = HW; ha.mblocks = 1; ha.xs = nullptr;
            head_ld<NS>(ha, b, smem, p.lds_total, opaque_tid(), q);
        }
        CT(c3)
        phase_fence();
        CT(c4)
        {
            TailArgs ta;
            ta.h1 = p.h1; ta.h1_row_bytes = p.h1_row_bytes;
            ta.B = p.B; ta.Hi = p.H; ta.Wi = p.Wd; ta.Ho = p.H; ta.Wo = p.Wd; ta.W = W; ta.cout = p.C;
            ta.w2p = uniform_ptr(cb->w2p); ta.w3p = uniform_ptr(cb->w3p); ta.k_idx = idx_i; ta.k_cnt = cnt_i;
            ta.sc2 = uniform_ptr(cb->sc2); ta.sh2 = uniform_ptr(cb->sh2); ta.ps2 = uniform_ptr(cb->ps2); ta.sh3 = uniform_ptr(cb->sh3);
            ta.residual = xin; ta.ldr = p.ldx; ta.out = p.x_work; ta.ldo = p.ldx; ta.colsum = p.colsum;
            ta.rows_per_blk = p.H; ta.mblocks = 1; ta.slice_bytes = p.slice_bytes; ta.pxs = nullptr; ta.pw = nullptr;
            tail_ld<NS>(ta, b, smem, p.lds_total, opaque_tid(), q);
        }
        CT(c5)
        phase_fence();
        CT(c6)
#ifdef LDN_TRACE
        am += c1 - c0; ah += c3 - c2; at += c5 - c4; af += (c2 - c1) + (c4 - c3) + (c6 - c5);
#endif
    }
#ifdef LDN_TRACE
    if (g_chain_trace && threadIdx.x == 0) {
        unsigned long long* r = g_chain_trace + (size_t)b * 4;
        r[0] = am; r[1] = ah; r[2] = at; r[3] = af;
    }
    if (g_ld_trace && (threadIdx.x & 63) == 0) {
        unsigned long long* r = g_ld_trace + ((size_t)b * 8 + (threadIdx.x >> 6)) * 8;
        for (int k = 0; k < 8; ++k) r[k] = q.t[k];
    }
#endif
}

}
```

laudnet_amd/csrc/ldn_tail.hip:

```cpp
#include "ldn_common.h"
#include "ldn_mlp.h"
#include <type_traits>
#include <stdlib.h>

namespace ldn {

struct TailArgs {
    const unsigned char* h1; long h1_row_bytes;
    int B, Hi, Wi, Ho, Wo, W, cout;
    const unsigned char* w2p;
    const unsigned char* w3p;
    const int32_t* k_idx; const int32_t* k_cnt;
    const float* sc2; const float* sh2; const float* ps2;
    const float* sh3;
    const float* residual; int ldr; float* out; int ldo;
    float* colsum;
    int rows_per_blk, mblocks;
    int slice_bytes;
    const unsigned char* pxs; const unsigned char* pw;
};
constexpr int T_PROJ_CIN = 64;

__device__ __attribute__((aligned(16))) float g_tail_zero[4] = {0.f, 0.f, 0.f, 0.f};

#ifndef LDN_TAIL_PRIO
#define LDN_TAIL_PRIO 0
#endif
#ifdef LDN_TRACE
__device__ unsigned long long* g_tail_trace = nullptr;
__device__ unsigned long long* g_chain_trace = nullptr;
__device__ unsigned long long* g_head_trace = nullptr;
#define TT(x) x = __builtin_amdgcn_s_memtime();
#define TT_ADD(acc, a, b) acc += (b) - (a);
#else
#define TT(x)
#define TT_ADD(acc, a, b)
#endif

#ifndef LDN_TAIL_ABLATE
#define LDN_TAIL_ABLATE 0
#endif
#if LDN_TAIL_ABLATE & 4
template <typename A, typename B, typename C> __device__ __forceinline__ C t_mfma_bf16(A a, B b, C c) { asm volatile("" ::"v"(a), "v"(b)); return c; }
#else
#define t_mfma_bf16(a, b, c) __builtin_amdgcn_mfma_f32_32x32x16_bf16(a, b, c, 0, 0, 0)
#endif

__device__ __forceinline__ void dma16_abl(const void* gsrc, unsigned lds_base) {
#if LDN_TAIL_ABLATE & 1
    return;
#endif
    dma16(gsrc, lds_base);
}
template <int NF> __device__ __forceinline__ void dma16_pieces_abl(const unsigned (&vo)[4], const void* sbase, unsigned lds_base) {
#if LDN_TAIL_ABLATE & 1
    return;
#endif
    dma16_pieces<NF>(vo, sbase, lds_base);
}

#define LDN_K16(F32_, ACC_, AH_, AL_, BH_, BL_) \
    if constexpr (F32_) { \
        const f32x4 ka0_ = __builtin_bit_cast(f32x4, AH_), ka1_ = __builtin_bit_cast(f32x4, AL_); \
        const f32x4 kb0_ = __builtin_bit_cast(f32x4, BH_), kb1_ = __builtin_bit_cast(f32x4, BL_); \
        _Pragma("unroll") for (int ki_ = 0; ki_ < 4; ++ki_) ACC_ = __builtin_amdgcn_mfma_f32_32x32x2f32(ka0_[ki_], kb0_[ki_], ACC_, 0, 0, 0); \
        _Pragma("unroll") for (int ki_ = 0; ki_ < 4; ++ki_) ACC_ = __builtin_amdgcn_mfma_f32_32x32x2f32(ka1_[ki_], kb1_[ki_], ACC_, 0, 0, 0); \
    } else { \
        ACC_ = t_mfma_bf16(AL_, BH_, ACC_); \
        ACC_ = t_mfma_bf16(AH_, BL_, ACC_); \
        ACC_ = t_mfma_bf16(AH_, BH_, ACC_); \
    }

constexpr int T_KIDX_BYTES = 1280;
constexpr int T_W2_SLOTS = 3;

#define LDN_TAIL_CHUNK_MFMA(WS_, HS_, TR_) {                                                                  \
            const unsigned char* ws = (WS_); \
            const unsigned rbase = (unsigned)(TR_) * 128u, rx = ((unsigned)(TR_) >> 1) & 7u; \
            bf16x8 bh[2], bl[2]; \
    _Pragma("unroll") \
            for (int half = 0; half < 2; ++half) { \
                const unsigned sl = 2u * (2u * half + h); \
                bh[half] = *reinterpret_cast<const bf16x8*>((HS_) + rbase + ((sl ^ rx) << 4)); \
                bl[half] = *reinterpret_cast<const bf16x8*>((HS_) + rbase + (((sl + 1) ^ rx) << 4)); \
            } \
    _Pragma("unroll") \
            for (int j = 0; j < NS; ++j) { \
                if (j < nsub) { \
                    u32x2 e0[4], e1[4]; \
    _Pragma("unroll") \
                    for (int q = 0; q < 4; ++q) e0[q] = *reinterpret_cast<const u32x2*>(ws + a_lane + q * W2_ROW + j * 256); \
    _Pragma("unroll") \
                    for (int q = 0; q < 4; ++q) e1[q] = *reinterpret_cast<const u32x2*>(ws + a_lane + (8 + q) * W2_ROW + j * 256); \
                     \
                     \
                    { \
                        const u32x4 ahu = F32 ? u32x4{e0[0][0], e0[0][1], e0[1][0], e0[1][1]} : u32x4{e0[0][0], e0[1][0], e0[2][0], e0[3][0]}; \
                        const u32x4 alu = F32 ? u32x4{e0[2][0], e0[2][1], e0[3][0], e0[3][1]} : u32x4{e0[0][1], e0[1][1], e0[2][1], e0[3][1]}; \
                        const bf16x8 ah = __builtin_bit_cast(bf16x8, ahu), al = __builtin_bit_cast(bf16x8, alu); \
                        LDN_K16(F32, acc[j], ah, al, bh[0], bl[0]) \
                    } \
                    { \
                        const u32x4 ahu = F32 ? u32x4{e1[0][0], e1[0][1], e1[1][0], e1[1][1]} : u32x4{e1[0][0], e1[1][0], e1[2][0], e1[3][0]}; \
                        const u32x4 alu = F32 ? u32x4{e1[2][0], e1[2][1], e1[3][0], e1[3][1]} : u32x4{e1[0][1], e1[1][1], e1[2][1], e1[3][1]}; \
                        const bf16x8 ah = __builtin_bit_cast(bf16x8, ahu), al = __builtin_bit_cast(bf16x8, alu); \
                        LDN_K16(F32, acc[j], ah, al, bh[1], bl[1]) \
                    } \
                    __builtin_amdgcn_sched_group_barrier(0x100, 8, 0); \
                    __builtin_amdgcn_sched_group_barrier(0x008, 6, 0); \
                } \
            } \
}

template <int NS, int ST = 1, bool PROJ = false, bool F32 = false>
__device__ __forceinline__ void tail_body(const TailArgs& p, const int b, const int mb, unsigned char* const smem, const int tid) {
    static_assert(!PROJ || (NS == 2 && ST == 1), "the folded projection exists for the 64-wide stride-1 block (stage 1's first block)");
    static_assert(!(PROJ && F32), "the folded projection is a bf16x3 form");
    constexpr int W = NS * 32;
    constexpr int SLICE_BUFS = ST == 2 ? 2 : (NS == 2 ? 1 : 2);
    constexpr int W2_ROW = NS * 256;
    constexpr int W2_SLOT = 16 * W2_ROW;
    constexpr int CW = (NS == 8 || PROJ) ? 32 : 64;
    constexpr int NCS = CW / 32;
    constexpr int W3_ROW = CW * 8;
    constexpr int RPI = 1024 / W3_ROW;
    constexpr int PROWS = PROJ ? T_PROJ_CIN / 2 : 0;
    constexpr int W3_SLOT = (W / 2 + PROWS) * W3_ROW;
    constexpr int NP = W;
    int* const s_kidx = reinterpret_cast<int*>(smem);
    unsigned char* const s_h1 = smem + T_KIDX_BYTES;
    unsigned char* const s_w2 = s_h1 + SLICE_BUFS * p.slice_bytes;
    unsigned char* const s_w3 = smem + T_KIDX_BYTES;
    float* const s_tab = reinterpret_cast<float*>(s_w3 + 2 * W3_SLOT);
    unsigned char* const s_scr = reinterpret_cast<unsigned char*>(s_tab + 18 * NP);

    int lane = tid & 63;
    const int wave = __builtin_amdgcn_readfirstlane(tid >> 6);
    int l31 = lane & 31, h = lane >> 5;
#ifdef LDN_TRACE
    unsigned long long tr0, tr1 = 0, tr2 = 0, tr3 = 0, tr4 = 0, ta = 0, tb = 0, w2wait = 0, w3wait = 0, w3bar = 0, w3epi = 0, w3k = 0;
    TT(tr0)
#endif
    const int y0 = mb * p.rows_per_blk;
    const int rows = min(p.rows_per_blk, p.Ho - y0);
    const int npix = rows * p.Wo;
    const int yin0 = max(ST * y0 - 1, 0), yin1 = min(ST * (y0 + rows - 1) + 1, p.Hi - 1);
    const int NR = (yin1 - yin0 + 1) * p.Wi;
    const int NRp = round_up(NR, 8);
    const int ZR = ST == 2 ? p.slice_bytes / 128 - 1 : NRp;
    int plo[4] = {0, 0, 0, 0}, pw[4] = {1, 1, 1, 1}, pn[4] = {0, 0, 0, 0}, clo[4] = {0, 0, 0, 0};
    if constexpr (ST == 2) {
#pragma unroll
        for (int g = 0; g < 4; ++g) {
            const int py = g >> 1, px = g & 1;
            const int rlo = py ? max(y0 - 1, 0) : y0;
            const int rhi = min(y0 + rows - 1, (p.Hi - 1 - py) >> 1);
            const int chi = min(p.Wo - 1, (p.Wi - 1 - px) >> 1);
            plo[g] = rlo; clo[g] = 0;
            pw[g] = max(chi + 1, 1);
            pn[g] = (rhi >= rlo && chi >= 0 && p.Hi - 1 - py >= 0 && p.Wi - 1 - px >= 0) ? (rhi - rlo + 1) * (chi + 1) : 0;
        }
    }
    const long in_row0 = (long)b * p.Hi * p.Wi + (long)yin0 * p.Wi;
    const long out_row0 = (long)b * p.Ho * p.Wo + (long)y0 * p.Wo;

    const int Kb = min(p.k_cnt[b], W);
    const int nsub = ceil_div(Kb, 32);
    const int Kp = nsub * 32;
    if (tid < W + 32) s_kidx[tid] = tid < Kb ? p.k_idx[(size_t)b * W + tid] : -1;
    LDN_DCHECK(p.k_cnt[b] >= 0 && p.k_cnt[b] <= W && (p.k_cnt[b] & 1) == 0, 301);
    if (tid < Kb) {
        const int ch = p.k_idx[(size_t)b * W + tid];
        LDN_DCHECK(ch >= 0 && ch < W, 302);
        LDN_DCHECK((tid & 1) ? (ch == p.k_idx[(size_t)b * W + tid - 1] + 1) : ((ch & 1) == 0), 303);
// ... 349 lines not shown
            }
            }
            f32x4 sh = *reinterpret_cast<const f32x4*>(p.sh3 + c0 + tc * 4);
            f32x16 acc3;
            TT(ta)
#pragma unroll
            for (int r = 0; r < 16; ++r) acc3[r] = 0.f;
#pragma unroll
            for (int j = 0; j < NS; ++j) {
                if (j < nsub && active) {
                    u32x2 e[2][4];
#pragma unroll
                    for (int t = 0; t < 2; ++t)
#pragma unroll
                        for (int q = 0; q < 4; ++q)
                            e[t][q] = *reinterpret_cast<const u32x2*>(ws + a3_lane + (16 * j + 8 * t + (q & 1) + 4 * (q >> 1)) * W3_ROW + cs * 256);
#pragma unroll
                    for (int t = 0; t < 2; ++t) {
                        const u32x4 ahu = F32 ? u32x4{e[t][0][0], e[t][0][1], e[t][1][0], e[t][1][1]} : u32x4{e[t][0][0], e[t][1][0], e[t][2][0], e[t][3][0]};
                        const u32x4 alu = F32 ? u32x4{e[t][2][0], e[t][2][1], e[t][3][0], e[t][3][1]} : u32x4{e[t][0][1], e[t][1][1], e[t][2][1], e[t][3][1]};
                        const bf16x8 ah = __builtin_bit_cast(bf16x8, ahu), al = __builtin_bit_cast(bf16x8, alu);
                        const bf16x8 hb = frag_hi(j, t), lb = frag_lo(j, t);
                        LDN_K16(F32, acc3, ah, al, hb, lb)
                    }
                    __builtin_amdgcn_sched_group_barrier(0x100, 8, 0);
                    __builtin_amdgcn_sched_group_barrier(0x008, 6, 0);
                }
            }
            if constexpr (PROJ) {
                if (active) {
#pragma unroll
                    for (int jj = 0; jj < T_PROJ_CIN / 32; ++jj) {
                        u32x2 e[2][4];
#pragma unroll
                        for (int t = 0; t < 2; ++t)
#pragma unroll
                            for (int q = 0; q < 4; ++q)
                                e[t][q] = *reinterpret_cast<const u32x2*>(ws + a3_lane + (Kp / 2 + 16 * jj + 8 * t + (q & 1) + 4 * (q >> 1)) * W3_ROW + cs * 256);
#pragma unroll
                        for (int t = 0; t < 2; ++t) {
                            const u32x4 ahu = {e[t][0][0], e[t][1][0], e[t][2][0], e[t][3][0]};
                            const u32x4 alu = {e[t][0][1], e[t][1][1], e[t][2][1], e[t][3][1]};
                            const bf16x8 ah = __builtin_bit_cast(bf16x8, ahu), al = __builtin_bit_cast(bf16x8, alu);
                            acc3 = t_mfma_bf16(al, pjh[2 * jj + t], acc3);
                            acc3 = t_mfma_bf16(ah, pjl[2 * jj + t], acc3);
                            acc3 = t_mfma_bf16(ah, pjh[2 * jj + t], acc3);
                        }
                        __builtin_amdgcn_sched_group_barrier(0x100, 8, 0);
                        __builtin_amdgcn_sched_group_barrier(0x008, 6, 0);
                    }
                }
            }
            TT(tb)
            TT_ADD(w3k, ta, tb)
            if (cs == NCS - 1) wait_vm<0>();
            if constexpr (PROJ) asm volatile("" : "+v"(sh));
            else asm volatile("" : "+v"(res[0]), "+v"(res[PROJ ? 0 : 1]), "+v"(res[PROJ ? 0 : 2]), "+v"(res[PROJ ? 0 : 3]), "+v"(sh));
            TT(ta)
            TT_ADD(w3wait, tb, ta)
#pragma unroll
            for (int q4 = 0; q4 < 4; ++q4) {
                const f32x4 v = {acc3[4 * q4], acc3[4 * q4 + 1], acc3[4 * q4 + 2], acc3[4 * q4 + 3]};
                *reinterpret_cast<f32x4*>(scr + l31 * 32 + (((2 * q4 + h) ^ (l31 & 7)) << 2)) = v;
            }
            asm volatile("s_waitcnt lgkmcnt(0)" ::: "memory");
            __builtin_amdgcn_wave_barrier();
            f32x4 csum = {0.f, 0.f, 0.f, 0.f};
#pragma unroll
            for (int it = 0; it < 4; ++it) {
                const int row = trw + 8 * it, prow = wave * 32 + row;
                f32x4 x = *reinterpret_cast<const f32x4*>(scr + row * 32 + ((tc ^ (row & 7)) << 2));
                if constexpr (PROJ) x = x + sh;
                else x = x + sh + res[PROJ ? 0 : it];
#pragma unroll
                for (int e = 0; e < 4; ++e) x[e] = fmaxf(x[e], 0.f);
                if (prow < npix) {
                    __builtin_nontemporal_store(x, reinterpret_cast<f32x4*>(p.out + (size_t)(out_row0 + prow) * p.ldo + c0 + tc * 4));
                    csum += x;
                }
            }
            if (p.colsum) {
#pragma unroll
                for (int e = 0; e < 4; ++e) csum[e] = sum_lane_bits_345(csum[e]);
                if (trw == 0)
                    *reinterpret_cast<f32x4*>(p.colsum + ((size_t)b * (p.mblocks * 8) + mb * 8 + wave) * p.cout + c0 + tc * 4) = csum;
            }
            asm volatile("s_waitcnt lgkmcnt(0)" ::: "memory");
            __builtin_amdgcn_wave_barrier();
            TT(tb)
            TT_ADD(w3epi, ta, tb)
        }
        TT(ta)
        lds_barrier();
        TT(tb)
        TT_ADD(w3bar, ta, tb)
    }
#ifdef LDN_TRACE
    TT(tr4)
    if (g_tail_trace && lane == 0) {
        unsigned long long* r = g_tail_trace + (((size_t)mb * p.B + b) * 8 + wave) * 12;
        r[0] = tr0; r[1] = tr1; r[2] = tr2; r[3] = tr3; r[4] = tr4; r[5] = w2wait; r[6] = w3k; r[7] = w3wait; r[8] = w3epi; r[9] = w3bar;
        r[10] = nsub; r[11] = 0;
    }
#endif
}

template <int NS, int ST, bool PROJ = false, bool F32 = false>
__global__ __launch_bounds__(512, ((NS == 2 && ST == 1) ? 4 : 2)) void k_tail(const TailArgs p) {
    extern __shared__ __attribute__((aligned(16))) unsigned char smem[];
    tail_body<NS, ST, PROJ, F32>(p, blockIdx.x % p.B, blockIdx.x / p.B, smem, threadIdx.x);
}

LDN_DEFINE_TU_VIOLATIONS(tu_violations_tail)

static int tail_region_pixels(int R, int Hi, int Wi, int st) {
    if (st == 2) return min(R + 1, (Hi + 1) / 2) * ((Wi - 1) / 2 + 1);
    return min(R + 2, Hi) * Wi;
}

static size_t tail_lds2(int R, int Hi, int Wi, int NS, int st) {
    const int nr = tail_region_pixels(R, Hi, Wi, st);
    const size_t slice = (size_t)round_up((round_up(nr, 8) + 1) * 128, 1024);
    return (size_t)T_KIDX_BYTES + (st == 2 ? 2 : (NS == 2 ? 1 : 2)) * slice + (size_t)T_W2_SLOTS * 16 * NS * 256;
}

static int tail_rows_per_block(int Hi, int Wi, int NS, int st, int* mblocks) {
    const int Ho = (Hi - 1) / st + 1, Wo = (Wi - 1) / st + 1;
    int R = 256 / Wo;
    if (R < 1) return 0;
    if (R > Ho) R = Ho;
    auto fits = [&](int r) {
        return tail_lds2(r, Hi, Wi, NS, st) <= 160 * 1024 && (st == 2 || NS == 2 || round_up(tail_region_pixels(r, Hi, Wi, st), 8) / 8 <= 72);
    };
    while (R > 1 && !fits(R)) --R;
    if (!fits(R)) return 0;
    const int mbk = ceil_div(Ho, R);
    *mblocks = mbk;
    int best = ceil_div(Ho, mbk), best_waves = 1 << 30;
    for (int r = ceil_div(Ho, mbk); r <= R; ++r) {
        if (r * (mbk - 1) >= Ho) break;
        int waves = 0;
        for (int i = 0; i < mbk; ++i) waves += ceil_div(min(r, Ho - r * i) * Wo, 32);
        if (waves < best_waves) { best_waves = waves; best = r; }
    }
    return best;
}

template <int NS, int ST, bool PROJ = false, bool F32 = false>
static int launch_tail(TailArgs& a, hipStream_t st) {
    constexpr int W = NS * 32;
    const int R = a.rows_per_blk;
    const int nr = tail_region_pixels(R, a.Hi, a.Wi, ST);
    a.slice_bytes = round_up((round_up(nr, 8) + 1) * 128, 1024);
    const size_t lds2 = tail_lds2(R, a.Hi, a.Wi, NS, ST);
    const size_t lds3 = (size_t)T_KIDX_BYTES + 2 * (size_t)(W / 2 + (PROJ ? T_PROJ_CIN / 2 : 0)) * ((NS == 8 || PROJ) ? 32 : 64) * 8 + (size_t)18 * W * 4 + 8 * 4096;
    const size_t lds = lds2 > lds3 ? lds2 : lds3;
    LDN_REQUIRE(lds <= 160 * 1024, "ldn_bottleneck_tail: %zu B of LDS exceed 160 KiB (map %dx%d, width %d)", lds, a.Ho, a.Wo, W);
    LDN_REQUIRE(ST == 2 || NS == 2 || round_up(nr, 8) / 8 <= 72, "ldn_bottleneck_tail: input region of %d pixels too large for the slice pipeline", nr);
    LDN_REQUIRE(allow_dynamic_lds(reinterpret_cast<const void*>(&k_tail<NS, ST, PROJ, F32>), lds), "k_tail: cannot reserve %zu B of LDS", lds);
    hipLaunchKernelGGL((k_tail<NS, ST, PROJ, F32>), dim3((unsigned)a.B * a.mblocks), dim3(512), lds, st, a);
    LDN_CHECK_LAUNCH("k_tail");
    return LDN_OK;
}

}

using namespace ldn;

#ifdef LDN_TRACE
extern "C" int ldn_debug_set_chain_trace(void* buf) {
    unsigned long long* q = static_cast<unsigned long long*>(buf);
    return hipMemcpyToSymbol(HIP_SYMBOL(g_chain_trace), &q, sizeof(q)) == hipSuccess ? 0 : -2;
}
extern "C" int ldn_debug_set_ld_trace(void* buf);
extern "C" int ldn_debug_set_head_trace(void* buf) {
    unsigned long long* q = static_cast<unsigned long long*>(buf);
    return hipMemcpyToSymbol(HIP_SYMBOL(g_head_trace), &q, sizeof(q)) == hipSuccess ? 0 : -2;
}
extern "C" int ldn_debug_set_tail_trace(void* buf) {
    unsigned long long* q = static_cast<unsigned long long*>(buf);
    return hipMemcpyToSymbol(HIP_SYMBOL(g_tail_trace), &q, sizeof(q)) == hipSuccess ? 0 : -2;
}
#endif

extern "C" int ldn_bottleneck_tail_splits(int H, int Wd, int width, int stride) {
    int mbk = 0;
    if (H < 1 || Wd < 1 || (stride != 1 && stride != 2) || (Wd - 1) / stride + 1 > 256 || (width != 64 && width != 128 && width != 256)) return 0;
    if (tail_rows_per_block(H, Wd, width / 32, stride, &mbk) == 0) return 0;
    return mbk * 8;
}

static int bottleneck_tail_impl(const void* h1_split, int ldh, int B, int H, int Wd, int stride, int width, const void* w2_pairs,
                                const void* w3_pairs, int cout, const int32_t* ch_idx, const int32_t* ch_cnt,
                                const float* scale2, const float* shift2_tab, const float* post_sub2,
                                const float* shift3, const float* residual, int ldr, float* out, int ldo,
                                float* colsum, const void* x_split, const void* wd_pairs, bool f32, void* stream);

extern "C" int ldn_bottleneck_tail(const void* h1_split, int ldh, int B, int H, int Wd, int stride, int width, const void* w2_pairs,
                                   const void* w3_pairs, int cout, const int32_t* ch_idx, const int32_t* ch_cnt,
                                   const float* scale2, const float* shift2_tab, const float* post_sub2,
                                   const float* shift3, const float* residual, int ldr, float* out, int ldo,
                                   float* colsum, void* stream) {
    return bottleneck_tail_impl(h1_split, ldh, B, H, Wd, stride, width, w2_pairs, w3_pairs, cout, ch_idx, ch_cnt, scale2, shift2_tab,
                                post_sub2, shift3, residual, ldr, out, ldo, colsum, nullptr, nullptr, false, stream);
}

extern "C" int ldn_bottleneck_tail_f32(const void* h1, int ldh, int B, int H, int Wd, int stride, int width, const void* w2_pairs_f32,
                                       const void* w3_pairs_f32, int cout, const int32_t* ch_idx, const int32_t* ch_cnt,
                                       const float* scale2, const float* shift2_tab, const float* post_sub2,
                                       const float* shift3, const float* residual, int ldr, float* out, int ldo,
                                       float* colsum, void* stream) {
    return bottleneck_tail_impl(h1, ldh, B, H, Wd, stride, width, w2_pairs_f32, w3_pairs_f32, cout, ch_idx, ch_cnt, scale2, shift2_tab,
                                post_sub2, shift3, residual, ldr, out, ldo, colsum, nullptr, nullptr, true, stream);
}

extern "C" int ldn_bottleneck_tail_proj_fits(int H, int Wd, int width, int cin) {
    int mbk = 0;
    if (H < 1 || Wd < 1 || Wd > 256 || width != 64 || cin != ldn::T_PROJ_CIN) return 0;
    return ldn::tail_rows_per_block(H, Wd, 2, 1, &mbk) > 0 ? 1 : 0;
}

extern "C" int ldn_bottleneck_tail_proj(const void* h1_split, int ldh, int B, int H, int Wd, int width, const void* w2_pairs,
                                        const void* w3_pairs, int cout, const int32_t* ch_idx, const int32_t* ch_cnt,
                                        const float* scale2, const float* shift2_tab, const float* post_sub2, const float* shift3d,
                                        const void* x_split, int cin, const void* wd_pairs, float* out, int ldo,
                                        float* colsum, void* stream) {
    LDN_REQUIRE(x_split && wd_pairs, "ldn_bottleneck_tail_proj: null pointer");
    LDN_REQUIRE(width == 64 && cin == ldn::T_PROJ_CIN, "ldn_bottleneck_tail_proj: the folded projection exists for width 64, cin 64 (got %d, %d; ldn_bottleneck_tail_proj_fits == 0)", width, cin);
    LDN_REQUIRE((uintptr_t)x_split % 16 == 0 && (uintptr_t)wd_pairs % 16 == 0, "ldn_bottleneck_tail_proj: x_split / wd_pairs must be 16-byte aligned");
    return bottleneck_tail_impl(h1_split, ldh, B, H, Wd, 1, width, w2_pairs, w3_pairs, cout, ch_idx, ch_cnt, scale2, shift2_tab,
                                post_sub2, shift3d, nullptr, 0, out, ldo, colsum, x_split, wd_pairs, false, stream);
}

static int bottleneck_tail_impl(const void* h1_split, int ldh, int B, int H, int Wd, int stride, int width, const void* w2_pairs,
                                const void* w3_pairs, int cout, const int32_t* ch_idx, const int32_t* ch_cnt,
                                const float* scale2, const float* shift2_tab, const float* post_sub2,
                                const float* shift3, const float* residual, int ldr, float* out, int ldo,
                                float* colsum, const void* x_split, const void* wd_pairs, bool f32, void* stream) {
    LDN_REQUIRE(h1_split && w2_pairs && w3_pairs && ch_idx && ch_cnt && scale2 && shift2_tab && post_sub2 && shift3 && out,
                "ldn_bottleneck_tail: null pointer");
    LDN_REQUIRE(width == 64 || width == 128 || width == 256, "ldn_bottleneck_tail: width must be 64, 128 or 256 (got %d)", width);
    LDN_REQUIRE(stride == 1 || stride == 2, "ldn_bottleneck_tail: stride must be 1 or 2 (got %d)", stride);
    LDN_REQUIRE(B > 0 && H > 0 && Wd > 0 && (Wd - 1) / stride + 1 <= 256, "ldn_bottleneck_tail: bad geometry (output map width must be <= 256)");
    LDN_REQUIRE(cout > 0 && cout % 64 == 0, "ldn_bottleneck_tail: cout must be a multiple of 64 (got %d)", cout);
    LDN_REQUIRE(ldh >= width && ldh % 8 == 0, "ldn_bottleneck_tail: ldh must be a multiple of 8 and >= width");
    LDN_REQUIRE(ldo >= cout && ldo % 4 == 0 && (!residual || (ldr >= cout && ldr % 4 == 0)), "ldn_bottleneck_tail: bad ldo / ldr");
    LDN_REQUIRE((uintptr_t)h1_split % 16 == 0 && (uintptr_t)w2_pairs % 16 == 0 && (uintptr_t)w3_pairs % 16 == 0 &&
                (uintptr_t)out % 16 == 0 && (uintptr_t)residual % 16 == 0 && (uintptr_t)shift3 % 16 == 0 && (uintptr_t)colsum % 16 == 0,
                "ldn_bottleneck_tail: pointers must be 16-byte aligned");
    LDN_REQUIRE((long)9 * (width / 2) * (width / 2) * 16 < (1L << 31), "ldn_bottleneck_tail: weights too large");
    TailArgs a{};
    a.h1 = static_cast<const unsigned char*>(h1_split);
    a.h1_row_bytes = (long)ldh * 4;
    a.B = B; a.Hi = H; a.Wi = Wd; a.Ho = (H - 1) / stride + 1; a.Wo = (Wd - 1) / stride + 1; a.W = width; a.cout = cout;
    a.w2p = static_cast<const unsigned char*>(w2_pairs);
    a.w3p = static_cast<const unsigned char*>(w3_pairs);
    a.k_idx = ch_idx; a.k_cnt = ch_cnt;
    a.sc2 = scale2; a.sh2 = shift2_tab; a.ps2 = post_sub2; a.sh3 = shift3;
    a.residual = residual; a.ldr = ldr; a.out = out; a.ldo = ldo; a.colsum = colsum;
    a.pxs = static_cast<const unsigned char*>(x_split); a.pw = static_cast<const unsigned char*>(wd_pairs);
    a.rows_per_blk = tail_rows_per_block(H, Wd, width / 32, stride, &a.mblocks);
    LDN_REQUIRE(a.rows_per_blk > 0, "ldn_bottleneck_tail: a %dx%d map of width %d (stride %d) does not fit the workgroup (ldn_bottleneck_tail_splits == 0)", H, Wd, width, stride);
    hipStream_t st = static_cast<hipStream_t>(stream);
    if (f32) {
        LDN_REQUIRE(!x_split, "ldn_bottleneck_tail: the folded projection is a bf16x3 form");
        if (stride == 2) {
            if (width == 64) return launch_tail<2, 2, false, true>(a, st);
            if (width == 128) return launch_tail<4, 2, false, true>(a, st);
            return launch_tail<8, 2, false, true>(a, st);
        }
        if (width == 64) return launch_tail<2, 1, false, true>(a, st);
        if (width == 128) return launch_tail<4, 1, false, true>(a, st);
        return launch_tail<8, 1, false, true>(a, st);
    }
    if (stride == 2) {
        if (width == 64) return launch_tail<2, 2>(a, st);
        if (width == 128) return launch_tail<4, 2>(a, st);
        return launch_tail<8, 2>(a, st);
    }
    if (x_split) return launch_tail<2, 1, true>(a, st);
    if (width == 64) return launch_tail<2, 1>(a, st);
    if (width == 128) return launch_tail<4, 1>(a, st);
    return launch_tail<8, 1>(a, st);
}

namespace ldn {

struct HeadArgs {
    const float* x; int ldx;
    int B, HW, cin, W;
    const unsigned char* w1s;
    const int32_t* n_idx; const int32_t* n_cnt;
    const float* sc1; const float* sh1; const float* ps1;
    unsigned char* h1; long h1_row_bytes;
    int pix_per_blk, mblocks;
    unsigned char* xs;
};

constexpr int H_XROWS = 256;

template <int NS, bool F32 = false, bool PRE_ROWS = false>
__device__ __forceinline__ void head_body(const HeadArgs& p, const int b, const int mb, unsigned char* const smem, const int lds_total, const int tid) {
    constexpr int W = NS * 32;
    int* const s_nidx = reinterpret_cast<int*>(smem);
    float* const s_tab = reinterpret_cast<float*>(smem + T_KIDX_BYTES);
    unsigned char* const s_ring = smem + T_KIDX_BYTES + 3 * W * 4;
// ... 306 lines not shown
    };

    if (!active) {
        dma_w_all(0);
        for (int S = 0; S < nstep; ++S) {
            wait_vm<0>();
            lds_barrier();
            dma_w_all(S + 1);
        }
        wait_vm<0>();
        return;
    }

    f32x16 acc[NS];
#pragma unroll
    for (int j = 0; j < NS; ++j)
#pragma unroll
        for (int r = 0; r < 16; ++r) acc[j][r] = 0.f;

    bf16x8 bh[2][2], bl[2][2];
    f32x4 raw[4];
    const unsigned xsw = ((unsigned)l31 >> 1) & 7u;
    auto read_raw = [&](int s) {
        const unsigned char* xs = my_r + (s & 1) * RSLOT + l31 * 128;
#pragma unroll
        for (int half = 0; half < 2; ++half) {
            const unsigned sl = 4u * half + 2u * h;
            raw[2 * half] = *reinterpret_cast<const f32x4*>(xs + ((sl ^ xsw) << 4));
            raw[2 * half + 1] = *reinterpret_cast<const f32x4*>(xs + (((sl + 1) ^ xsw) << 4));
        }
    };
    auto split_b = [&](int half, bf16x8 (&dh)[2], bf16x8 (&dl)[2]) {
#pragma unroll
        for (int e = 0; e < 8; ++e) {
            const float v = e < 4 ? raw[2 * half][e] : raw[2 * half + 1][e - 4];
            const __bf16 hb = (__bf16)v;
            dh[half][e] = hb;
            dl[half][e] = (__bf16)(v - (float)hb);
        }
    };

    dma_w_all(0);
#pragma unroll
    for (int k = 0; k < 4; ++k) dma_r(0, k);
#pragma unroll
    for (int k = 0; k < 4; ++k) dma_r(1, k);
    wait_vm<4>();
    read_raw(0);
    split_b(0, bh[0], bl[0]);
    split_b(1, bh[0], bl[0]);
    asm volatile("s_waitcnt lgkmcnt(0)" ::: "memory");
    __builtin_amdgcn_sched_barrier(0);
#pragma unroll
    for (int k = 0; k < 4; ++k) dma_r(2, k);
    wait_vm<4>();

    auto step = [&](int S, auto cur_c) {
        constexpr int CUR = decltype(cur_c)::value;
        wait_vm<4>();
        lds_barrier();
        const unsigned char* wsl = s_w + (S & 1) * WSLOT + l31 * 128;
        int stage = 0;
        auto extra = [&]() {
            if (stage == 0) dma_w_all(S + 1);
            else if (stage == 1) { wait_vm_rt<15, 16>(4 + 2 * nw); read_raw(S + 1); }
            else if (stage == 2) split_b(0, bh[CUR ^ 1], bl[CUR ^ 1]);
            else if (stage == 3) split_b(1, bh[CUR ^ 1], bl[CUR ^ 1]);
            else if (stage == 4) {
                asm volatile("s_waitcnt lgkmcnt(0)" ::: "memory");
#pragma unroll
                for (int k = 0; k < 4; ++k) dma_r(S + 3, k);
            }
            ++stage;
        };
#pragma unroll
        for (int half = 0; half < 2; ++half) {
            const unsigned uu = 2u * (2u * half + h);
#pragma unroll
            for (int j = 0; j < NS; ++j) {
                if (j < nsub) {
                    const bf16x8 ah = *reinterpret_cast<const bf16x8*>(wsl + j * 4096 + ((uu ^ xsw) << 4));
                    const bf16x8 al = *reinterpret_cast<const bf16x8*>(wsl + j * 4096 + (((uu + 1) ^ xsw) << 4));
                    acc[j] = t_mfma_bf16(al, bh[CUR][half], acc[j]);
                    acc[j] = t_mfma_bf16(ah, bl[CUR][half], acc[j]);
                    acc[j] = t_mfma_bf16(ah, bh[CUR][half], acc[j]);
                    __builtin_amdgcn_sched_group_barrier(0x100, 2, 0);
                    __builtin_amdgcn_sched_group_barrier(0x008, 3, 0);
                }
                if (j <= 2 && j < nsub) { __builtin_amdgcn_sched_barrier(0); extra(); __builtin_amdgcn_sched_barrier(0); }
            }
        }
        while (stage < 5) extra();
        __builtin_amdgcn_sched_barrier(0);
    };
    for (int S = 0; S < nstep; S += 2) {
        step(S, std::integral_constant<int, 0>{});
        step(S + 1, std::integral_constant<int, 1>{});
    }
    wait_vm<0>();

    const int pm = wave * 32 + l31;
    unsigned char* orow = p.h1 + (row0 + min(pm, npix - 1)) * p.h1_row_bytes;
#pragma unroll
    for (int j = 0; j < NS; ++j) {
        if (j >= nsub) continue;
#pragma unroll
        for (int q4 = 0; q4 < 4; ++q4) {
            const int n0 = 32 * j + 8 * q4 + 4 * h;
            const f32x4 sc = *reinterpret_cast<const f32x4*>(s_tab + n0);
            const f32x4 sh = *reinterpret_cast<const f32x4*>(s_tab + W + n0);
            const f32x4 ps = *reinterpret_cast<const f32x4*>(s_tab + 2 * W + n0);
            unsigned hi2[2], lo2[2];
#pragma unroll
            for (int d = 0; d < 2; ++d) {
                const float v0 = fmaxf(acc[j][4 * q4 + 2 * d] * sc[2 * d] + sh[2 * d], 0.f) - ps[2 * d];
                const float v1 = fmaxf(acc[j][4 * q4 + 2 * d + 1] * sc[2 * d + 1] + sh[2 * d + 1], 0.f) - ps[2 * d + 1];
                const bf16x2 hh = {(__bf16)v0, (__bf16)v1};
                const bf16x2 ll = {(__bf16)(v0 - (float)hh[0]), (__bf16)(v1 - (float)hh[1])};
                hi2[d] = __builtin_bit_cast(unsigned, hh);
                lo2[d] = __builtin_bit_cast(unsigned, ll);
            }
            u32x4 outv;
#pragma unroll
            for (int d = 0; d < 2; ++d) {
                const auto r = __builtin_amdgcn_permlane32_swap(hi2[d], lo2[d], false, false);
                outv[d] = r[0];
                outv[2 + d] = r[1];
            }
            if (pm < npix) *reinterpret_cast<u32x4*>(orow + (4 * j + q4) * 32 + h * 16) = outv;
        }
    }
}

template <int NS, bool F32 = false>
__global__ __launch_bounds__(512, 2) void k_head(const HeadArgs p) {
    extern __shared__ __attribute__((aligned(16))) unsigned char smem[];
#ifdef LDN_HEAD_V2
    if constexpr (!F32) {
        if (p.xs == nullptr && p.cin % 64 == 0) {
            head_body2<NS>(p, blockIdx.x % p.B, blockIdx.x / p.B, smem, threadIdx.x);
            return;
        }
    }
#endif
#ifdef LDN_HEAD_NO_PRE
    head_body<NS, F32, false>(p, blockIdx.x % p.B, blockIdx.x / p.B, smem, 160 * 1024, threadIdx.x);
#else
    head_body<NS, F32, true>(p, blockIdx.x % p.B, blockIdx.x / p.B, smem, 160 * 1024, threadIdx.x);
#endif
}

template <int NS, bool F32 = false>
static int launch_head(HeadArgs& a, hipStream_t st) {
    const size_t lds = 160 * 1024;
    LDN_REQUIRE(allow_dynamic_lds(reinterpret_cast<const void*>(&k_head<NS, F32>), lds), "k_head: cannot reserve %zu B of LDS", lds);
    hipLaunchKernelGGL((k_head<NS, F32>), dim3((unsigned)a.B * a.mblocks), dim3(512), lds, st, a);
    LDN_CHECK_LAUNCH("k_head");
    return LDN_OK;
}

}

static int bottleneck_head_impl(const float* x, int ldx, int B, int HW, int cin, const void* w1_split, int width,
                                const int32_t* ch_idx, const int32_t* ch_cnt, const float* scale1, const float* shift1,
                                const float* post_sub1, void* h1_split, int ldh, void* x_split, bool f32, void* stream);

extern "C" int ldn_bottleneck_head(const float* x, int ldx, int B, int HW, int cin, const void* w1_split, int width,
                                   const int32_t* ch_idx, const int32_t* ch_cnt, const float* scale1, const float* shift1,
                                   const float* post_sub1, void* h1_split, int ldh, void* stream) {
    return bottleneck_head_impl(x, ldx, B, HW, cin, w1_split, width, ch_idx, ch_cnt, scale1, shift1, post_sub1, h1_split, ldh, nullptr, false, stream);
}

extern "C" int ldn_bottleneck_head_f32(const float* x, int ldx, int B, int HW, int cin, const float* w1, int width,
                                       const int32_t* ch_idx, const int32_t* ch_cnt, const float* scale1, const float* shift1,
                                       const float* post_sub1, float* h1, int ldh, void* stream) {
    return bottleneck_head_impl(x, ldx, B, HW, cin, w1, width, ch_idx, ch_cnt, scale1, shift1, post_sub1, h1, ldh, nullptr, true, stream);
}

extern "C" size_t ldn_x_split_bytes(size_t pixels, int cin) { return ((pixels + 31) / 32) * (size_t)cin * 128; }

extern "C" int ldn_bottleneck_head_split(const float* x, int ldx, int B, int HW, int cin, const void* w1_split, int width,
                                         const int32_t* ch_idx, const int32_t* ch_cnt, const float* scale1, const float* shift1,
                                         const float* post_sub1, void* h1_split, int ldh, void* x_split, void* stream) {
    LDN_REQUIRE(x_split && (uintptr_t)x_split % 16 == 0, "ldn_bottleneck_head_split: x_split must be a 16-byte aligned buffer of ldn_x_split_bytes(B * HW, cin) bytes");
    return bottleneck_head_impl(x, ldx, B, HW, cin, w1_split, width, ch_idx, ch_cnt, scale1, shift1, post_sub1, h1_split, ldh, x_split, false, stream);
}

static int bottleneck_head_impl(const float* x, int ldx, int B, int HW, int cin, const void* w1_split, int width,
                                const int32_t* ch_idx, const int32_t* ch_cnt, const float* scale1, const float* shift1,
                                const float* post_sub1, void* h1_split, int ldh, void* x_split, bool f32, void* stream) {
    using namespace ldn;
    LDN_REQUIRE(x && w1_split && ch_idx && ch_cnt && scale1 && shift1 && post_sub1 && h1_split, "ldn_bottleneck_head: null pointer");
    LDN_REQUIRE(width == 64 || width == 128 || width == 256, "ldn_bottleneck_head: width must be 64, 128 or 256 (got %d)", width);
    LDN_REQUIRE(B > 0 && HW > 0 && cin > 0 && cin % 32 == 0, "ldn_bottleneck_head: cin must be a multiple of 32 (got %d)", cin);
    LDN_REQUIRE(ldx >= cin && ldx % 4 == 0 && ldh >= width && ldh % 8 == 0, "ldn_bottleneck_head: bad ldx / ldh");
    LDN_REQUIRE((uintptr_t)x % 16 == 0 && (uintptr_t)w1_split % 16 == 0 && (uintptr_t)h1_split % 16 == 0, "ldn_bottleneck_head: pointers must be 16-byte aligned");
    HeadArgs a{};
    a.x = x; a.ldx = ldx; a.B = B; a.HW = HW; a.cin = cin; a.W = width;
    a.w1s = static_cast<const unsigned char*>(w1_split);
    a.n_idx = ch_idx; a.n_cnt = ch_cnt; a.sc1 = scale1; a.sh1 = shift1; a.ps1 = post_sub1;
    a.h1 = static_cast<unsigned char*>(h1_split); a.h1_row_bytes = (long)ldh * 4;
    a.xs = static_cast<unsigned char*>(x_split);
    a.mblocks = ceil_div(HW, 256);
    a.pix_per_blk = ceil_div(HW, a.mblocks);
    if (const int up = round_up(a.pix_per_blk, 32); up <= 256 && (long)up * (a.mblocks - 1) < HW) a.pix_per_blk = up;
    hipStream_t st = static_cast<hipStream_t>(stream);
    if (f32) {
        if (width == 64) return launch_head<2, true>(a, st);
        if (width == 128) return launch_head<4, true>(a, st);
        return launch_head<8, true>(a, st);
    }
    if (width == 64) return launch_head<2>(a, st);
    if (width == 128) return launch_head<4>(a, st);
    return launch_head<8>(a, st);
}

namespace ldn {

struct ChainBlock {
    const unsigned char* w1s; const float* sc1; const float* sh1; const float* ps1;
    const unsigned char* w2p; const unsigned char* w3p; const float* sc2; const float* sh2; const float* ps2; const float* sh3;
    const float* mw1; const float* mb1; const float* mw2; const float* mb2;
};
static_assert(sizeof(ChainBlock) == 14 * 8, "ChainBlock must mirror ldn_chain_block");

struct ChainArgs {
    const ChainBlock* blocks; int nblocks;
    const float* x_in; float* x_work; int ldx;
    int B, H, Wd, C;
    int hidden, G, gran;
    const float* gap_in; int gap_splits;
    float* colsum;
    float* masks; int32_t* ch_idx; int32_t* ch_cnt;
    unsigned char* h1; long h1_row_bytes;
    int slice_bytes, lds_total;
};

__device__ __forceinline__ void phase_fence() {
    __builtin_amdgcn_fence(__ATOMIC_RELEASE, "workgroup");
    __syncthreads();
    __builtin_amdgcn_fence(__ATOMIC_ACQUIRE, "workgroup");
    asm volatile("s_dcache_inv\n\ts_waitcnt lgkmcnt(0)" ::: "memory");
}

__device__ __forceinline__ int opaque_tid() {
    int t = threadIdx.x;
    asm volatile("" : "+v"(t));
    return t;
}

#ifdef LDN_TRACE
#define CT(x) x = __builtin_amdgcn_s_memtime();
#else
#define CT(x)
#endif

template <int NS, bool F32 = false>
__global__ __launch_bounds__(512, (NS == 2 ? 4 : 2)) void k_chain(const ChainArgs p) {
    constexpr int W = NS * 32;
    extern __shared__ __attribute__((aligned(16))) unsigned char smem[];
    const int b = blockIdx.x;
    const int HW = p.H * p.Wd;
#ifdef LDN_TRACE
    unsigned long long c0, c1, c2, c3, c4, c5, c6, am = 0, ah = 0, at = 0, af = 0;
#endif
    for (int i = 0; i < p.nblocks; ++i) {
        CT(c0)
        const ChainBlock* cb = p.blocks + i;
        float* const mask_i = p.masks + (size_t)i * p.B * p.G;
        int32_t* const idx_i = p.ch_idx + (size_t)i * p.B * W;
        int32_t* const cnt_i = p.ch_cnt + (size_t)i * p.B;
        const float* const xin = i == 0 ? p.x_in : p.x_work;
        {
            float* const s_f = reinterpret_cast<float*>(smem);
            int* const s_w = reinterpret_cast<int*>(s_f + p.C + (p.hidden > 0 ? p.hidden : 1) + 2 * p.G);
            channel_mlp_body<512>(b, i == 0 ? p.gap_in : p.colsum, HW, p.C, i == 0 ? p.gap_splits : 8, uniform_ptr(cb->mw1),
                                  uniform_ptr(cb->mb1), uniform_ptr(cb->mw2), uniform_ptr(cb->mb2), p.hidden, p.G, p.gran, nullptr,
                                  mask_i, nullptr, idx_i, cnt_i, s_f, s_w);
        }
        CT(c1)
        phase_fence();
        CT(c2)
        {
            HeadArgs ha;
            ha.x = xin; ha.ldx = p.ldx; ha.B = p.B; ha.HW = HW; ha.cin = p.C; ha.W = W;
            ha.w1s = uniform_ptr(cb->w1s); ha.n_idx = idx_i; ha.n_cnt = cnt_i;
            ha.sc1 = uniform_ptr(cb->sc1); ha.sh1 = uniform_ptr(cb->sh1); ha.ps1 = uniform_ptr(cb->ps1);
            ha.h1 = p.h1; ha.h1_row_bytes = p.h1_row_bytes; ha.pix_per_blk = HW; ha.mblocks = 1; ha.xs = nullptr;
#ifdef LDN_HEAD_V2
            if constexpr (!F32) head_body2<NS>(ha, b, 0, smem, opaque_tid());
            else
#endif
            head_body<NS, F32>(ha, b, 0, smem, p.lds_total, opaque_tid());
        }
        CT(c3)
        phase_fence();
        CT(c4)
        {
            TailArgs ta;
            ta.h1 = p.h1; ta.h1_row_bytes = p.h1_row_bytes;
            ta.B = p.B; ta.Hi = p.H; ta.Wi = p.Wd; ta.Ho = p.H; ta.Wo = p.Wd; ta.W = W; ta.cout = p.C;
            ta.w2p = uniform_ptr(cb->w2p); ta.w3p = uniform_ptr(cb->w3p); ta.k_idx = idx_i; ta.k_cnt = cnt_i;
            ta.sc2 = uniform_ptr(cb->sc2); ta.sh2 = uniform_ptr(cb->sh2); ta.ps2 = uniform_ptr(cb->ps2); ta.sh3 = uniform_ptr(cb->sh3);
            ta.residual = xin; ta.ldr = p.ldx; ta.out = p.x_work; ta.ldo = p.ldx; ta.colsum = p.colsum;
            ta.rows_per_blk = p.H; ta.mblocks = 1; ta.slice_bytes = p.slice_bytes; ta.pxs = nullptr; ta.pw = nullptr;
            tail_body<NS, 1, false, F32>(ta, b, 0, smem, opaque_tid());
        }
        CT(c5)
        phase_fence();
        CT(c6)
#ifdef LDN_TRACE
        am += c1 - c0; ah += c3 - c2; at += c5 - c4; af += (c2 - c1) + (c4 - c3) + (c6 - c5);
#endif
    }
#ifdef LDN_TRACE
    if (g_chain_trace && threadIdx.x == 0) {
        unsigned long long* r = g_chain_trace + (size_t)b * 4;
        r[0] = am; r[1] = ah; r[2] = at; r[3] = af;
    }
#endif
}

}
#include "ldn_chain_ld.h"
namespace ldn {

static bool chain_fits(int H, int Wd, int width, int C, int hidden, int G) {
    const int NS = width / 32;
    const int nr = H * Wd;
    const size_t slice = (size_t)round_up((round_up(nr, 8) + 1) * 128, 1024);
    const size_t lds2 = (size_t)T_KIDX_BYTES + (NS == 2 ? 1 : 2) * slice + (size_t)T_W2_SLOTS * 16 * NS * 256;
    const size_t lds3 = (size_t)T_KIDX_BYTES + 2 * (size_t)(width / 2) * (NS == 8 ? 32 : 64) * 8 + (size_t)18 * width * 4 + 8 * 4096;
    const size_t ldsm = (size_t)(C + (hidden > 0 ? hidden : 1) + 2 * G) * 4 + 64;
    const size_t lds1 = (size_t)T_KIDX_BYTES + 3 * (size_t)width * 4 + 2 * (size_t)(round_up(nr, 32) + width) * 128;
    const size_t lds = 160 * 1024;
    return lds2 <= lds && lds3 <= lds && ldsm <= lds && lds1 <= lds && round_up(nr, 8) / 8 <= 72;
}

template <int NS, bool F32 = false>
static int launch_chain(ChainArgs& a, hipStream_t st) {
    constexpr int W = NS * 32;
    const int nr = a.H * a.Wd;
    a.slice_bytes = round_up((round_up(nr, 8) + 1) * 128, 1024);
    const size_t lds = 160 * 1024;
    LDN_REQUIRE(chain_fits(a.H, a.Wd, W, a.C, a.hidden, a.G), "ldn_bottleneck_chain: the phases need more than 160 KiB of LDS (map %dx%d, width %d; ldn_bottleneck_chain_fits == 0)", a.H, a.Wd, W);
    a.lds_total = (int)lds;
    if constexpr (!F32 && NS >= 4) {
        static const bool use_ld = [] { const char* e = getenv("LDN_CHAIN_LD"); return !(e && atoi(e) == 0); }();
        if (use_ld && nr <= 224) {
            {
                static bool armed[64] = {};
                int dev = 0;
                hipStreamCaptureStatus cs = hipStreamCaptureStatusNone;
                if (hipGetDevice(&dev) == hipSuccess && dev >= 0 && dev < 64 && !armed[dev] && hipStreamIsCapturing(st, &cs) == hipSuccess &&
                    cs == hipStreamCaptureStatusNone) {
                    int* d = fault_word_dev();
                    if (d && hipMemcpyToSymbol(HIP_SYMBOL(g_ld_fault_dev), &d, sizeof(d)) == hipSuccess) armed[dev] = true;
                    else (void)hipGetLastError();
                }
            }
            LDN_REQUIRE(allow_dynamic_lds(reinterpret_cast<const void*>(&k_chain_ld<NS>), lds), "k_chain_ld: cannot reserve %zu B of LDS", lds);
            hipLaunchKernelGGL((k_chain_ld<NS>), dim3((unsigned)a.B), dim3(512), lds, st, a);
            LDN_CHECK_LAUNCH("k_chain_ld");
            return LDN_OK;
        }
    }
    LDN_REQUIRE(allow_dynamic_lds(reinterpret_cast<const void*>(&k_chain<NS, F32>), lds), "k_chain: cannot reserve %zu B of LDS", lds);
    hipLaunchKernelGGL((k_chain<NS, F32>), dim3((unsigned)a.B), dim3(512), lds, st, a);
    LDN_CHECK_LAUNCH("k_chain");
    return LDN_OK;
}

}

#ifdef LDN_TRACE
extern "C" int ldn_debug_set_ld_trace(void* buf) {
    unsigned long long* q = static_cast<unsigned long long*>(buf);
    return hipMemcpyToSymbol(HIP_SYMBOL(ldn::g_ld_trace), &q, sizeof(q)) == hipSuccess ? 0 : -2;
}
#endif
namespace ldn {
int tu_chain_stalls(unsigned* count, int reset) {
    unsigned v = 0u;
    if (hipMemcpyFromSymbol(&v, HIP_SYMBOL(g_ld_stalls), sizeof(v)) != hipSuccess) return LDN_EHIP;
    *count += v;
    if (reset && v) {
        const unsigned z = 0u;
        if (hipMemcpyToSymbol(HIP_SYMBOL(g_ld_stalls), &z, sizeof(z)) != hipSuccess) return LDN_EHIP;
    }
    return LDN_OK;
}
}

#ifdef LDN_DEBUG
extern "C" int ldn_debug_chain_stall(int image) {
    return hipMemcpyToSymbol(HIP_SYMBOL(ldn::g_chain_stall), &image, sizeof(image)) == hipSuccess ? LDN_OK : LDN_EHIP;
}
#endif

extern "C" int ldn_bottleneck_chain_fits(int H, int Wd, int C, int width, int hidden, int G) {
    if (H < 1 || Wd < 1 || H * Wd > 256 || C < 1 || G < 1 || hidden < 0 || (width != 64 && width != 128 && width != 256)) return 0;
    return ldn::chain_fits(H, Wd, width, C, hidden, G) ? 1 : 0;
}

static int bottleneck_chain_impl(const float* x_in, float* x_work, int ldx, int B, int H, int Wd, int C, int width,
                                 const ldn_chain_block* blocks, int nblocks, int hidden, int G, int gran,
                                 const float* gap_in, int gap_splits, float* colsum, float* masks, int32_t* ch_idx,
                                 int32_t* ch_cnt, void* h1_split, int ldh, bool f32, void* stream);
extern "C" int ldn_bottleneck_chain(const float* x_in, float* x_work, int ldx, int B, int H, int Wd, int C, int width,
                                    const ldn_chain_block* blocks, int nblocks, int hidden, int G, int gran,
                                    const float* gap_in, int gap_splits, float* colsum, float* masks, int32_t* ch_idx,
                                    int32_t* ch_cnt, void* h1_split, int ldh, void* stream) {
    return bottleneck_chain_impl(x_in, x_work, ldx, B, H, Wd, C, width, blocks, nblocks, hidden, G, gran, gap_in, gap_splits, colsum, masks,
                                 ch_idx, ch_cnt, h1_split, ldh, false, stream);
}
extern "C" int ldn_bottleneck_chain_f32(const float* x_in, float* x_work, int ldx, int B, int H, int Wd, int C, int width,
                                        const ldn_chain_block* blocks, int nblocks, int hidden, int G, int gran,
                                        const float* gap_in, int gap_splits, float* colsum, float* masks, int32_t* ch_idx,
                                        int32_t* ch_cnt, float* h1, int ldh, void* stream) {
    return bottleneck_chain_impl(x_in, x_work, ldx, B, H, Wd, C, width, blocks, nblocks, hidden, G, gran, gap_in, gap_splits, colsum, masks,
                                 ch_idx, ch_cnt, h1, ldh, true, stream);
}
static int bottleneck_chain_impl(const float* x_in, float* x_work, int ldx, int B, int H, int Wd, int C, int width,
                                 const ldn_chain_block* blocks, int nblocks, int hidden, int G, int gran,
                                 const float* gap_in, int gap_splits, float* colsum, float* masks, int32_t* ch_idx,
                                 int32_t* ch_cnt, void* h1_split, int ldh, bool f32, void* stream) {
    using namespace ldn;
    LDN_REQUIRE(x_in && x_work && blocks && gap_in && colsum && masks && ch_idx && ch_cnt && h1_split, "ldn_bottleneck_chain: null pointer");
    LDN_REQUIRE(width == 64 || width == 128 || width == 256, "ldn_bottleneck_chain: width must be 64, 128 or 256 (got %d)", width);
    LDN_REQUIRE(B > 0 && H > 0 && Wd > 0 && H * Wd <= 256, "ldn_bottleneck_chain: the map must fit one workgroup (H * W <= 256, got %dx%d)", H, Wd);
    LDN_REQUIRE(C > 0 && C % 64 == 0, "ldn_bottleneck_chain: C must be a multiple of 64 (got %d)", C);
    LDN_REQUIRE(nblocks > 0 && gap_splits > 0 && hidden >= 0 && G > 0 && gran > 0 && gran % 2 == 0 && G * gran == width,
                "ldn_bottleneck_chain: bad run / masker shape (G * gran must equal width, gran even)");
    LDN_REQUIRE(ldx >= C && ldx % 4 == 0 && ldh >= width && ldh % 8 == 0, "ldn_bottleneck_chain: bad ldx / ldh");
    LDN_REQUIRE((uintptr_t)x_in % 16 == 0 && (uintptr_t)x_work % 16 == 0 && (uintptr_t)h1_split % 16 == 0 && (uintptr_t)colsum % 16 == 0 &&
                (uintptr_t)blocks % 8 == 0, "ldn_bottleneck_chain: pointers must be 16-byte aligned");
    LDN_REQUIRE((long)9 * (width / 2) * (width / 2) * 16 < (1L << 31), "ldn_bottleneck_chain: weights too large");
    ChainArgs a{};
    a.blocks = reinterpret_cast<const ChainBlock*>(blocks); a.nblocks = nblocks;
    a.x_in = x_in; a.x_work = x_work; a.ldx = ldx; a.B = B; a.H = H; a.Wd = Wd; a.C = C;
    a.hidden = hidden; a.G = G; a.gran = gran; a.gap_in = gap_in; a.gap_splits = gap_splits; a.colsum = colsum;
    a.masks = masks; a.ch_idx = ch_idx; a.ch_cnt = ch_cnt;
    a.h1 = static_cast<unsigned char*>(h1_split); a.h1_row_bytes = (long)ldh * 4;
    hipStream_t st = static_cast<hipStream_t>(stream);
    if (f32) {
        if (width == 64) return launch_chain<2, true>(a, st);
        if (width == 128) return launch_chain<4, true>(a, st);
        return launch_chain<8, true>(a, st);
    }
    if (width == 64) return launch_chain<2>(a, st);
    if (width == 128) return launch_chain<4>(a, st);
    return launch_chain<8>(a, st);
}
```

laudnet_amd/ops.py:

```python
from __future__ import annotations

import contextlib
import os
import threading
import weakref
from dataclasses import dataclass

import torch

from . import _lib as L


def _f32c(t, what):
    if t is None:
        return None
    if t.dtype != torch.float32 or not t.is_contiguous():
        raise L.LdnError(f"{what}: expected a contiguous float32 tensor, got {t.dtype} strides {t.stride()}")
    return t


def _f32rows(t, what):
    if t is None:
        return None
    if t.dtype != torch.float32 or t.dim() != 2 or t.stride(1) != 1 or t.data_ptr() % 16 != 0:
# ... 785 lines not shown
    L.require_device(a2d, w, out2d, gate)
    lib = L.load()
    cout, t, cin = w.shape
    if t != 1:
        raise L.LdnError("conv_rows_gated: 1x1 weights expected")
    if gate.shape[1] != cin or not gate.is_contiguous():
        raise L.LdnError("conv_rows_gated: gate must be a contiguous [images, cin] tensor")
    if m_cap is None:
        m_cap = a2d.shape[0]
    if (m_cap + gate_rows - 1) // gate_rows > gate.shape[0]:
        raise L.LdnError("conv_rows_gated: gate has fewer rows than the images m_cap spans")
    L.check(lib.ldn_conv_rows_gated(L.ptr(_f32rows(a2d, "a")), a2d.stride(0), L.ptr(_i32c(m_count, "m_count")), m_cap,
                                    L.ptr(split_rows_weight(w)), cin, cout, L.ptr(_f32c(scale, "scale")), L.ptr(_f32c(shift, "shift")), relu,
                                    L.ptr(_i32c(relu_if_neg, "relu_if_neg")), L.ptr(_i32c(out_rows, "out_rows")),
                                    L.ptr(_f32rows(residual2d, "residual")), residual2d.stride(0) if residual2d is not None else 0,
                                    L.ptr(_f32rows(out2d, "out")), out2d.stride(0), L.ptr(_f32c(gate, "gate")), int(gate_rows),
                                    L.stream_ptr(out2d)), "ldn_conv_rows_gated")
    return out2d


def grouped_conv3x3_image(a_nhwc, w, group_width, ch_idx, ch_cnt, scale, shift, out_nhwc, *, stride=1, relu=1):
    L.require_device(a_nhwc, w, out_nhwc, ch_idx)
    lib = L.load()
    B, Hi, Wi, lda = a_nhwc.shape
    _, Ho, Wo, ldo = out_nhwc.shape
    C = w.shape[0]
    L.check(lib.ldn_grouped_conv3x3_image(L.ptr(_f32c(a_nhwc, "a")), lda, B, Hi, Wi, stride, Ho, Wo, L.ptr(_f32c(w, "w")), C,
                                          group_width, L.ptr(_i32c(ch_idx, "ch_idx")), L.ptr(_i32c(ch_cnt, "ch_cnt")),
                                          L.ptr(_f32c(scale, "scale")), L.ptr(_f32c(shift, "shift")), relu,
                                          L.ptr(_f32c(out_nhwc, "out")), ldo, L.stream_ptr(out_nhwc)), "ldn_grouped_conv3x3_image")
    return out_nhwc


def se_packed(a2d, row_prefix, w1, b1, w2, b2, max_rows_per_image, ch_idx=None, ch_cnt=None):
    L.require_device(a2d, row_prefix)
    lib = L.load()
    B = row_prefix.numel() - 1
    S, C = w1.shape
    work = _work(lib.ldn_se_packed_workspace_bytes(B, C, max_rows_per_image), a2d.device)
    L.check(lib.ldn_se_packed(L.ptr(_f32c(a2d, "a")), a2d.stride(0), L.ptr(_i32c(row_prefix, "row_prefix")), B, C, S,
                              L.ptr(_f32c(w1, "w1")), L.ptr(_f32c(b1, "b1")), L.ptr(_f32c(w2, "w2")), L.ptr(_f32c(b2, "b2")),
                              L.ptr(_i32c(ch_idx, "ch_idx")), L.ptr(_i32c(ch_cnt, "ch_cnt")), max_rows_per_image, L.ptr(work),
                              L.stream_ptr()), "ldn_se_packed")
    return a2d


def _hi_lo(w):
    hi = w.to(torch.bfloat16)
    lo = (w - hi.float()).to(torch.bfloat16)
    return hi, lo


def pack_w2_pairs(conv2_weight, f32=False):
    W = conv2_weight.shape[0]
    w = conv2_weight.detach().float().permute(2, 3, 1, 0).reshape(9, W // 2, 2, W // 2, 2)
    w = w.permute(0, 1, 3, 4, 2).contiguous()
    if f32:
        return w
    hi, lo = _hi_lo(w)
    return torch.stack((hi, lo), dim=-2).contiguous()


def pack_w3_pairs(w3_scaled, f32=False):
    cout, W = w3_scaled.shape
    w = w3_scaled.detach().float().t().reshape(W // 2, 2, cout).permute(0, 2, 1).contiguous()
    if f32:
        return w
    hi, lo = _hi_lo(w)
    return torch.stack((hi, lo), dim=-2).contiguous()


def pack_w1_split(conv1_weight_2d, f32=False):
    W, cin = conv1_weight_2d.shape
    if f32:
        return conv1_weight_2d.detach().float().contiguous()
    w = conv1_weight_2d.detach().float().reshape(W, cin // 8, 8)
    hi, lo = _hi_lo(w)
    return torch.stack((hi, lo), dim=-2).contiguous()


def bottleneck_head(x_nhwc, w1_split, ch_idx, ch_cnt, scale1, shift1, post_sub1, h1_split, x_split=None):
    L.require_device(x_nhwc, w1_split, h1_split)
    lib = L.load()
    B, H, Wd, cin = x_nhwc.shape
    width = ch_idx.shape[1]
    if w1_split.dtype == torch.float32:
        if not w1_split.is_contiguous() or x_split is not None:
            raise L.LdnError("bottleneck_head: the fp32 form takes a contiguous fp32 weight matrix and writes no x_split")
        L.check(lib.ldn_bottleneck_head_f32(L.ptr(_f32c(x_nhwc, "x")), cin, B, H * Wd, cin, L.ptr(w1_split), width,
                                            L.ptr(_i32c(ch_idx, "ch_idx")), L.ptr(_i32c(ch_cnt, "ch_cnt")), L.ptr(_f32c(scale1, "scale1")),
                                            L.ptr(_f32c(shift1, "shift1")), L.ptr(_f32c(post_sub1, "post_sub1")),
                                            L.ptr(_f32c(h1_split, "h1")), h1_split.shape[-1], L.stream_ptr(h1_split)), "ldn_bottleneck_head_f32")
        return h1_split
    if w1_split.dtype != torch.bfloat16 or not w1_split.is_contiguous():
        raise L.LdnError("bottleneck_head: w1_split must be the contiguous bf16 tensor of pack_w1_split")
    if x_split is not None:
        if x_split.dtype != torch.float32 or not x_split.is_contiguous() or x_split.numel() * 4 < lib.ldn_x_split_bytes(B * H * Wd, cin):
            raise L.LdnError("bottleneck_head: x_split must be a contiguous fp32 buffer of x_split_buffer(B * H * W, cin)")
        L.check(lib.ldn_bottleneck_head_split(L.ptr(_f32c(x_nhwc, "x")), cin, B, H * Wd, cin, L.ptr(w1_split), width,
                                              L.ptr(_i32c(ch_idx, "ch_idx")), L.ptr(_i32c(ch_cnt, "ch_cnt")), L.ptr(_f32c(scale1, "scale1")),
                                              L.ptr(_f32c(shift1, "shift1")), L.ptr(_f32c(post_sub1, "post_sub1")),
                                              L.ptr(_f32c(h1_split, "h1")), h1_split.shape[-1], L.ptr(x_split),
                                              L.stream_ptr(h1_split)), "ldn_bottleneck_head_split")
        return h1_split
    L.check(lib.ldn_bottleneck_head(L.ptr(_f32c(x_nhwc, "x")), cin, B, H * Wd, cin, L.ptr(w1_split), width,
                                    L.ptr(_i32c(ch_idx, "ch_idx")), L.ptr(_i32c(ch_cnt, "ch_cnt")), L.ptr(_f32c(scale1, "scale1")),
                                    L.ptr(_f32c(shift1, "shift1")), L.ptr(_f32c(post_sub1, "post_sub1")),
                                    L.ptr(_f32c(h1_split, "h1")), h1_split.shape[-1], L.stream_ptr(h1_split)), "ldn_bottleneck_head")
    return h1_split


CHAIN_BLOCK_FIELDS = 14


def chain_table(rows, device):
    flat = []
    for row in rows:
        if len(row) != CHAIN_BLOCK_FIELDS:
            raise L.LdnError("chain_table: a block takes 14 tensors")
        for t in row:
            if t is not None and (not t.is_contiguous() or t.device != torch.device(device)):
                raise L.LdnError("chain_table: tensors must be contiguous and on the table's device")
            flat.append(0 if t is None else t.data_ptr())
    return torch.tensor(flat, dtype=torch.int64).view(len(rows), CHAIN_BLOCK_FIELDS).to(device)


def bottleneck_chain(x_in, x_work, table, width, hidden, G, gran, gap_in, f32=False):
    L.require_device(x_in, x_work, table, gap_in)
    lib = L.load()
    B, H, Wd, C = x_in.shape
    n = table.shape[0]
    dev = x_in.device
    if x_work.shape != x_in.shape or not (x_in.is_contiguous() and x_work.is_contiguous()) or x_in.dtype != torch.float32:
        raise L.LdnError("bottleneck_chain: x_in / x_work must be contiguous fp32 NHWC tensors of the same shape")
    if table.dtype != torch.int64 or table.dim() != 2 or table.shape[1] != CHAIN_BLOCK_FIELDS or not table.is_contiguous():
        raise L.LdnError("bottleneck_chain: table must come from chain_table")
    if gap_in.dim() != 3 or gap_in.shape[0] != B or gap_in.shape[2] != C:
        raise L.LdnError("bottleneck_chain: gap_in must be [B, splits, C]")
    masks = torch.empty(n, B, G, device=dev, dtype=torch.float32)
    ch_idx = torch.empty(n, B, width, device=dev, dtype=torch.int32)
    ch_cnt = torch.empty(n, B, device=dev, dtype=torch.int32)
    colsum = torch.empty(B, 8, C, device=dev, dtype=torch.float32)
    h1 = torch.empty(B, H, Wd, width, device=dev, dtype=torch.float32)
    L.check((lib.ldn_bottleneck_chain_f32 if f32 else lib.ldn_bottleneck_chain)(L.ptr(x_in), L.ptr(x_work), C, B, H, Wd, C, width, L.ptr(table), n, hidden, G, gran,
                                     L.ptr(_f32c(gap_in, "gap_in")), gap_in.shape[1], L.ptr(colsum), L.ptr(masks), L.ptr(ch_idx),
                                     L.ptr(ch_cnt), L.ptr(h1), width, L.stream_ptr(x_work)), "ldn_bottleneck_chain")
    return masks, ch_idx, ch_cnt, colsum


def bottleneck_chain_fits(H, W, C, width, hidden, G):
    return bool(L.load().ldn_bottleneck_chain_fits(H, W, C, width, hidden, G))


def bottleneck_tail_splits(H, W, width, stride=1):
    return L.load().ldn_bottleneck_tail_splits(H, W, width, stride)


def bottleneck_tail(h1_split, w2_pairs, w3_pairs, ch_idx, ch_cnt, scale2, shift2_tab, post_sub2, shift3, out_nhwc, *,
                    residual=None, colsum=None, stride=1):
    L.require_device(h1_split, w2_pairs, w3_pairs, out_nhwc)
    lib = L.load()
    B, H, Wd, ldh = h1_split.shape
    width = ch_idx.shape[1]
    cout = out_nhwc.shape[-1]
    Ho, Wo = (H - 1) // stride + 1, (Wd - 1) // stride + 1
    if tuple(out_nhwc.shape) != (B, Ho, Wo, cout) or (residual is not None and tuple(residual.shape[:3]) != (B, Ho, Wo)):
        raise L.LdnError(f"bottleneck_tail: out / residual must be [B={B}, {Ho}, {Wo}, cout] for an {H}x{Wd} input at stride {stride}")
    if w2_pairs.dtype != w3_pairs.dtype or w2_pairs.dtype not in (torch.bfloat16, torch.float32) or not (w2_pairs.is_contiguous() and w3_pairs.is_contiguous()):
        raise L.LdnError("bottleneck_tail: w2_pairs / w3_pairs must be the contiguous tensors of pack_w2_pairs / pack_w3_pairs (both bf16, or both fp32)")
    fn = lib.ldn_bottleneck_tail if w2_pairs.dtype == torch.bfloat16 else lib.ldn_bottleneck_tail_f32
    L.check(fn(L.ptr(_f32c(h1_split, "h1")), ldh, B, H, Wd, stride, width, L.ptr(w2_pairs), L.ptr(w3_pairs), cout,
                                    L.ptr(_i32c(ch_idx, "ch_idx")), L.ptr(_i32c(ch_cnt, "ch_cnt")), L.ptr(_f32c(scale2, "scale2")),
                                    L.ptr(_f32c(shift2_tab, "shift2_tab")), L.ptr(_f32c(post_sub2, "post_sub2")),
                                    L.ptr(_f32c(shift3, "shift3")), L.ptr(residual),
                                    residual.shape[-1] if residual is not None else 0, L.ptr(_f32c(out_nhwc, "out")), cout,
                                    L.ptr(colsum), L.stream_ptr(out_nhwc)), "ldn_bottleneck_tail")
    return out_nhwc


def x_split_buffer(pixels, cin, dev):
    return torch.empty(L.load().ldn_x_split_bytes(pixels, cin) // 4, device=dev, dtype=torch.float32)


def decode_x_split(xs, pixels, cin):
    t = xs.view(torch.bfloat16).reshape(-1, cin // 16, 2, 2, 32, 8).float()
    v = (t[:, :, :, 0] + t[:, :, :, 1]).permute(0, 3, 1, 2, 4).reshape(-1, cin)
    return v[:pixels]


def bottleneck_tail_proj_fits(H, W, width, cin):
    return bool(L.load().ldn_bottleneck_tail_proj_fits(H, W, width, cin))


def bottleneck_tail_proj(h1_split, w2_pairs, w3_pairs, ch_idx, ch_cnt, scale2, shift2_tab, post_sub2, shift3d, x_split, wd_pairs,
                         out_nhwc, *, colsum=None):
    L.require_device(h1_split, w2_pairs, w3_pairs, x_split, wd_pairs, out_nhwc)
    lib = L.load()
    B, H, Wd, ldh = h1_split.shape
    width = ch_idx.shape[1]
    cout = out_nhwc.shape[-1]
    cin = wd_pairs.shape[0] * 2
    if tuple(out_nhwc.shape) != (B, H, Wd, cout) or x_split.numel() * 4 < lib.ldn_x_split_bytes(B * H * Wd, cin) or not x_split.is_contiguous():
        raise L.LdnError(f"bottleneck_tail_proj: out must be [B={B}, {H}, {Wd}, cout], x_split the buffer bottleneck_head filled")
    for t in (w2_pairs, w3_pairs, wd_pairs):
        if t.dtype != torch.bfloat16 or not t.is_contiguous():
            raise L.LdnError("bottleneck_tail_proj: w2_pairs / w3_pairs / wd_pairs must be the contiguous bf16 tensors of pack_w2_pairs / pack_w3_pairs")
    L.check(lib.ldn_bottleneck_tail_proj(L.ptr(_f32c(h1_split, "h1")), ldh, B, H, Wd, width, L.ptr(w2_pairs), L.ptr(w3_pairs), cout,
                                         L.ptr(_i32c(ch_idx, "ch_idx")), L.ptr(_i32c(ch_cnt, "ch_cnt")), L.ptr(_f32c(scale2, "scale2")),
                                         L.ptr(_f32c(shift2_tab, "shift2_tab")), L.ptr(_f32c(post_sub2, "post_sub2")),
                                         L.ptr(_f32c(shift3d, "shift3d")), L.ptr(x_split), cin, L.ptr(wd_pairs),
                                         L.ptr(_f32c(out_nhwc, "out")), cout, L.ptr(colsum), L.stream_ptr(out_nhwc)), "ldn_bottleneck_tail_proj")
    return out_nhwc


def bottleneck_smallmap_fits(H, W, cin, width, cout):
    return bool(L.load().ldn_bottleneck_smallmap_fits(H, W, cin, width, cout))


def bottleneck_smallmap(x_nhwc, w1_split, w2_pairs, w3_pairs, ch_idx, ch_cnt, scale1, shift1, post_sub1, scale2, shift2_tab, post_sub2,
                        shift3, out_nhwc, *, residual=None, colsum=None):
    L.require_device(x_nhwc, w1_split, w2_pairs, w3_pairs, out_nhwc)
    lib = L.load()
    B, H, Wd, cin = x_nhwc.shape
    width = ch_idx.shape[1]
    cout = out_nhwc.shape[-1]
    if tuple(out_nhwc.shape) != (B, H, Wd, cout) or (residual is not None and tuple(residual.shape) != (B, H, Wd, cout)):
        raise L.LdnError(f"bottleneck_smallmap: out / residual must be [B={B}, {H}, {Wd}, cout]")
    if colsum is not None and (tuple(colsum.shape) != (B, 2, cout) or not colsum.is_contiguous()):
        raise L.LdnError("bottleneck_smallmap: colsum must be a contiguous [B, 2, cout] tensor")
    for w in (w1_split, w2_pairs, w3_pairs):
        if w.dtype != torch.bfloat16 or not w.is_contiguous():
            raise L.LdnError("bottleneck_smallmap: weights must be the contiguous bf16 tensors of pack_w1_split / pack_w2_pairs / pack_w3_pairs")
    L.check(lib.ldn_bottleneck_smallmap(L.ptr(_f32c(x_nhwc, "x")), cin, B, H, Wd, cin, width, L.ptr(w1_split), L.ptr(w2_pairs),
                                        L.ptr(w3_pairs), cout, L.ptr(_i32c(ch_idx, "ch_idx")), L.ptr(_i32c(ch_cnt, "ch_cnt")),
                                        L.ptr(_f32c(scale1, "scale1")), L.ptr(_f32c(shift1, "shift1")), L.ptr(_f32c(post_sub1, "post_sub1")),
                                        L.ptr(_f32c(scale2, "scale2")), L.ptr(_f32c(shift2_tab, "shift2_tab")),
                                        L.ptr(_f32c(post_sub2, "post_sub2")), L.ptr(_f32c(shift3, "shift3")), L.ptr(residual),
                                        cout if residual is not None else 0, L.ptr(_f32c(out_nhwc, "out")), cout, L.ptr(colsum),
                                        L.stream_ptr(out_nhwc)), "ldn_bottleneck_smallmap")
    return out_nhwc


def pack_stem_weights(w_scaled):
    cout = w_scaled.shape[0]
    if tuple(w_scaled.shape[1:]) != (3, 7, 7) or cout % 32:
        raise L.LdnError("pack_stem_weights: expected [cout % 32 == 0, 3, 7, 7]")
    w = w_scaled.detach().float().permute(0, 2, 3, 1).reshape(cout, 7, 21)
    k = torch.zeros(cout, 8, 24, device=w.device, dtype=torch.float32)
    k[:, :7, :21] = w
    k = k.reshape(cout, 24, 8)[:, :22]
    k = k.reshape(cout // 32, 32, 11, 2, 8)
    k = k.permute(0, 2, 3, 1, 4).reshape(cout // 32, 11, 64, 8)
    hi, lo = _hi_lo(k)
    return torch.stack((hi, lo), dim=-2).contiguous()


def stem_conv_pool(x_nhwc, w_frag, shift, cout, want_gap=False):
    L.require_device(x_nhwc, w_frag, shift)
    lib = L.load()
    B, H, W, cin = x_nhwc.shape
    if cin != 3 or x_nhwc.dtype != torch.float32 or not x_nhwc.is_contiguous():
        raise L.LdnError("stem_conv_pool: x must be a contiguous fp32 [B,H,W,3] tensor")
    if w_frag.dtype != torch.bfloat16 or not w_frag.is_contiguous() or w_frag.numel() * 2 != lib.ldn_stem_weight_bytes(cout):
        raise L.LdnError("stem_conv_pool: w_frag must be the contiguous bf16 tensor of pack_stem_weights")
    Hc, Wc = (H - 1) // 2 + 1, (W - 1) // 2 + 1
    Hp, Wp = (Hc - 1) // 2 + 1, (Wc - 1) // 2 + 1
    out = torch.empty(B, Hp, Wp, cout, device=x_nhwc.device, dtype=torch.float32)
    if want_gap:
        gap = torch.empty(B, lib.ldn_stem_gap_splits(H, W), cout, device=x_nhwc.device, dtype=torch.float32)
        L.check(lib.ldn_stem_conv_pool_gap(L.ptr(x_nhwc), B, H, W, L.ptr(w_frag), L.ptr(_f32c(shift, "shift")), cout, L.ptr(out), Hp, Wp,
                                           L.ptr(gap), L.stream_ptr(out)), "ldn_stem_conv_pool_gap")
        return out, gap
    L.check(lib.ldn_stem_conv_pool(L.ptr(x_nhwc), B, H, W, L.ptr(w_frag), L.ptr(_f32c(shift, "shift")), cout, L.ptr(out), Hp, Wp,
                                   L.stream_ptr(out)), "ldn_stem_conv_pool")
    return out


def pack_stem3_weights(w_scaled):
    cout = w_scaled.shape[0]
    if tuple(w_scaled.shape[1:]) != (3, 3, 3) or cout % 32:
        raise L.LdnError("pack_stem3_weights: expected [cout % 32 == 0, 3, 3, 3]")
    k = torch.zeros(cout, 3, 16, device=w_scaled.device, dtype=torch.float32)
    k[:, :, :9] = w_scaled.detach().float().permute(0, 2, 3, 1).reshape(cout, 3, 9)
    k = k.reshape(cout // 32, 32, 3, 2, 8).permute(0, 2, 3, 1, 4).reshape(cout // 32, 3, 64, 8)
    hi, lo = _hi_lo(k)
    return torch.stack((hi, lo), dim=-2).contiguous()


def stem3_conv(x_nhwc, w_frag, shift, cout, relu=True):
    L.require_device(x_nhwc, w_frag, shift)
    lib = L.load()
    B, H, W, cin = x_nhwc.shape
    if cin != 3 or x_nhwc.dtype != torch.float32 or not x_nhwc.is_contiguous():
        raise L.LdnError("stem3_conv: x must be a contiguous fp32 [B,H,W,3] tensor")
    if w_frag.dtype != torch.bfloat16 or not w_frag.is_contiguous() or w_frag.numel() * 2 != lib.ldn_stem3_weight_bytes(cout):
        raise L.LdnError("stem3_conv: w_frag must be the contiguous bf16 tensor of pack_stem3_weights")
    Ho, Wo = (H - 1) // 2 + 1, (W - 1) // 2 + 1
    out = torch.empty(B, Ho, Wo, cout, device=x_nhwc.device, dtype=torch.float32)
    L.check(lib.ldn_stem3_conv(L.ptr(x_nhwc), B, H, W, L.ptr(w_frag), L.ptr(_f32c(shift, "shift")), cout, int(bool(relu)),
                               L.ptr(out), Ho, Wo, L.stream_ptr(out)), "ldn_stem3_conv")
    return out


def token_lists(keep):
    B, Lt = keep.shape
    ix = mask_to_index(keep.reshape(B, Lt, 1).float().contiguous(), Lt, 1, 1)
# ... 24 lines not shown
```

Measured before the change: 23000.

## Route banded head and tail convs through loader-wave DMA pipelined kernels

Adds standalone banded kernels (k_head_ld, k_tail_ld) that reuse the loader-wave/consumer-wave pipelined path from the fused chain kernel for ordinary multi-block head and stride-1 tail launches. The tail gains band-relative row offsets, halo input rows and a larger h1 piece schedule (up to 40 pieces). They are enabled by default through an env/API switch when the tile fits in LDS. The goal is to overlap weight and activation loads with MFMA work in the non-chain layers. The cost is more LDS pressure and more spin-wait synchronisation between waves.

```diff
diff --git a/include/ldn_hip.h b/include/ldn_hip.h
--- a/include/ldn_hip.h
+++ b/include/ldn_hip.h
@@ -170,6 +170,9 @@
                          int gap_splits, float* colsum, float* masks, int32_t* ch_idx, int32_t* ch_cnt, float* h1,
                          int ldh, void* stream);
 
+int ldn_band_ld(int mode);
+int ldn_band_ld_form(int H, int W, int width, int stride, int f32, int is_tail);
+
 size_t ldn_stem_weight_bytes(int cout);
 int ldn_stem_conv_pool(const float* x, int B, int H, int W, const void* w_frag, const float* shift, int cout, float* out,
                        int Hp, int Wp, void* stream);
diff --git a/laudnet_amd/_lib.py b/laudnet_amd/_lib.py
--- a/laudnet_amd/_lib.py
+++ b/laudnet_amd/_lib.py
@@ -89,6 +89,8 @@
     "ldn_packed_mha": ([_P, _I, _P, _P, _I, _I, _I, _I, C.c_float, _P, _I, _P], _I),
     "ldn_packed_mha_heads": ([_P, _I, _P, _P, _I, _I, _I, _I, C.c_float, _P, _P, _I, _P], _I),
     "ldn_bottleneck_chain_fits": ([_I, _I, _I, _I, _I, _I], _I),
+    "ldn_band_ld": ([_I], _I),
+    "ldn_band_ld_form": ([_I, _I, _I, _I, _I, _I], _I),
     "ldn_bottleneck_smallmap_fits": ([_I, _I, _I, _I, _I], _I),
     "ldn_bottleneck_smallmap": ([_P, _I, _I, _I, _I, _I, _I, _P, _P, _P, _I, _P, _P, _P, _P, _P, _P, _P, _P, _P, _P, _I, _P, _I, _P, _P], _I),
     "ldn_bottleneck_chain": ([_P, _P, _I, _I, _I, _I, _I, _I, _P, _I, _I, _I, _I, _P, _I, _P, _P, _P, _P, _P, _I, _P], _I),
diff --git a/laudnet_amd/csrc/ldn_chain_ld.h b/laudnet_amd/csrc/ldn_chain_ld.h
--- a/laudnet_amd/csrc/ldn_chain_ld.h
+++ b/laudnet_amd/csrc/ldn_chain_ld.h
@@ -109,9 +109,9 @@
 #ifdef LDN_DEBUG
 __device__ int g_chain_stall = -1;
 #endif
-__device__ __forceinline__ void ld_publish(LdSync* sy, unsigned landed) {
+__device__ __forceinline__ void ld_publish(LdSync* sy, unsigned landed, [[maybe_unused]] const bool chained = true) {
 #ifdef LDN_DEBUG
-    if ((int)blockIdx.x == g_chain_stall) return;
+    if (chained && (int)blockIdx.x == g_chain_stall) return;
 #endif
     asm volatile("" ::: "memory");
     if ((threadIdx.x & 63) == 0) ld_lds_write(&sy->landed, landed);
@@ -141,8 +141,8 @@
     }
 }
 
-template <int NS>
-__device__ __forceinline__ void head_ld(const HeadArgs& p, const int b, unsigned char* const smem, const int lds_total, const int tid, LdSeq& q) {
+template <int NS, bool BAND = false>
+__device__ __forceinline__ void head_ld(const HeadArgs& p, const int b, [[maybe_unused]] const int mb, unsigned char* const smem, const int lds_total, const int tid, LdSeq& q) {
     constexpr int W = NS * 32;
     constexpr int MAXP = NS * 4;
     int* const s_nidx = reinterpret_cast<int*>(smem);
@@ -153,8 +153,9 @@
     const int lane = tid & 63;
     const int wave = __builtin_amdgcn_readfirstlane(tid >> 6);
     const int l31 = lane & 31, h = lane >> 5;
-    const int npix = p.HW;
-    const long row0 = (long)b * p.HW;
+    const int m0 = BAND ? mb * p.pix_per_blk : 0;
+    const int npix = BAND ? min(p.pix_per_blk, p.HW - m0) : p.HW;
+    const long row0 = (long)b * p.HW + m0;
     const int ncomp = ceil_div(npix, 32);
 
     const int Nb = min(p.n_cnt[b], W);
@@ -200,10 +201,10 @@
             if (c >= RW) LD_TIMED(5, ld_wait_done(sy, ncomp, base + (unsigned)(c - RW + 1), dead))
             ld_dma_run<MAXP>(wo, nwp, p.w1s + (long)c * 128, lds_w + (unsigned)slot * (unsigned)wslot);
             slot = slot + 1 == RW ? 0 : slot + 1;
-            if (c > 0) { wait_vm_rt<62, 63>(nwp); ld_publish(sy, base + (unsigned)c); }
+            if (c > 0) { wait_vm_rt<62, 63>(nwp); ld_publish(sy, base + (unsigned)c, !BAND); }
         }
         wait_vm<0>();
-        ld_publish(sy, base + (unsigned)nchunks);
+        ld_publish(sy, base + (unsigned)nchunks, !BAND);
         LT(tb)
         LD_SPAN(0, ta, tb)
         return;
@@ -349,11 +350,12 @@
 }
 
 constexpr int LD_CW = 32;
-template <int NS>
-__device__ __forceinline__ void tail_ld(const TailArgs& p, const int b, unsigned char* const smem, const int lds_total, const int tid, LdSeq& q) {
+constexpr int LD_BAND_MAXH = 40;
+template <int NS, bool BAND = false>
+__device__ __forceinline__ void tail_ld(const TailArgs& p, const int b, [[maybe_unused]] const int mb, unsigned char* const smem, const int lds_total, const int tid, LdSeq& q) {
     constexpr int W = NS * 32;
     constexpr int MAXP = NS * 4;
-    constexpr int MAXH = 28;
+    constexpr int MAXH = BAND ? LD_BAND_MAXH : 28;
     constexpr int NP = W;
     constexpr int W3_ROW = LD_CW * 8;
     int* const s_kidx = reinterpret_cast<int*>(smem);
@@ -368,11 +370,17 @@
     int lane = tid & 63;
     const int wave = __builtin_amdgcn_readfirstlane(tid >> 6);
     int l31 = lane & 31, h = lane >> 5;
-    const int npix = p.Ho * p.Wo;
+    const int y0 = BAND ? mb * p.rows_per_blk : 0;
+    const int rows = BAND ? min(p.rows_per_blk, p.Ho - y0) : p.Ho;
+    const int npix = rows * p.Wo;
     const int ncomp = ceil_div(npix, 32);
-    const int NR = npix, NRp = round_up(NR, 8);
+    const int yin0 = BAND ? max(y0 - 1, 0) : 0;
+    const int yin1 = BAND ? min(y0 + rows, p.Hi - 1) : p.Hi - 1;
+    const int NR = BAND ? (yin1 - yin0 + 1) * p.Wi : npix, NRp = round_up(NR, 8);
     const int ZR = NRp;
-    const long pix0 = (long)b * npix;
+    const long in_row0 = BAND ? (long)b * p.Hi * p.Wi + (long)yin0 * p.Wi : (long)b * npix;
+    const long out_row0 = BAND ? (long)b * p.Ho * p.Wo + (long)y0 * p.Wo : (long)b * npix;
+    const size_t gap_slot0 = BAND ? (size_t)b * (p.mblocks * 8) + mb * 8 : (size_t)b * 8;
 
     const int Kb = min(p.k_cnt[b], W);
     const int nsub = __builtin_amdgcn_readfirstlane(ceil_div(Kb, 32));
@@ -393,7 +401,7 @@
     const unsigned base2 = q.base, base3 = base2 + (unsigned)nchunks;
     q.base = base3 + (unsigned)nchunk3;
     constexpr int TMIN = 3;
-    static_assert(TMIN == 3 && MAXH == 28, "the slice schedule below is written out for taps 3 .. 8 and <= 28 pieces");
+    static_assert(TMIN == 3 && MAXH <= 42, "the slice schedule below is written out for taps 3 .. 8 and <= 42 pieces");
 
     const bool loader = wave == LD_LOADER;
     const bool consumer = wave < ncomp;
@@ -456,7 +464,7 @@
                 }
         };
         const unsigned lds_h1 = lds_off(s_h1);
-        const unsigned char* const h1b = p.h1 + pix0 * p.h1_row_bytes;
+        const unsigned char* const h1b = p.h1 + in_row0 * p.h1_row_bytes;
         auto h1_piece = [&](int i, const void* sb, unsigned dst) {
             const int r = 8 * i + (lane >> 3);
             const unsigned o = (unsigned)(min(r, NR - 1) * (int)p.h1_row_bytes + (((lane & 7) ^ ((r >> 1) & 7)) << 4));
@@ -484,7 +492,7 @@
                 load_half(tn, 0, LA);
             }
             store_half(slotp, 1, LB);
-            ld_publish(sy, base2 + (unsigned)c + 1u);
+            ld_publish(sy, base2 + (unsigned)c + 1u, !BAND);
             if (nxt) load_half(tn, 1, LB);
             if (tc >= TMIN && sc + 1 < nsub) {
                 const void* hsb = uniform_ptr(h1b + (long)(sc + 1) * 128);
@@ -512,7 +520,7 @@
             no[i] = (unsigned)((ch >> 1) * 16) + ld_bias(i);
         }
         const unsigned lds_h1 = lds_off(s_h1), lds_w2 = lds_off(s_w2);
-        const unsigned char* const h1b = p.h1 + pix0 * p.h1_row_bytes;
+        const unsigned char* const h1b = p.h1 + in_row0 * p.h1_row_bytes;
         if (nchunks > 0) {
 #pragma unroll
             for (int i = 0; i < MAXH; ++i)
@@ -537,23 +545,23 @@
                 int pieces = P2;
                 if (t >= TMIN && more) {
                     const void* hsb = uniform_ptr(hsrc);
-#define LDN_LD_H1(I) if ((I) < nq) { dma16_pieces<1>({ho[(I)]}, hsb, (unsigned)__builtin_amdgcn_readfirstlane((int)(hdst + (unsigned)(I) * 1024u))); ++pieces; }
+#define LDN_LD_H1(I) if constexpr ((I) < MAXH) { if ((I) < nq) { dma16_pieces<1>({ho[(I)]}, hsb, (unsigned)__builtin_amdgcn_readfirstlane((int)(hdst + (unsigned)(I) * 1024u))); ++pieces; } }
                     switch (t) {
-                        case 3: LDN_LD_H1(0) LDN_LD_H1(6) LDN_LD_H1(12) LDN_LD_H1(18) LDN_LD_H1(24) break;
-                        case 4: LDN_LD_H1(1) LDN_LD_H1(7) LDN_LD_H1(13) LDN_LD_H1(19) LDN_LD_H1(25) break;
-                        case 5: LDN_LD_H1(2) LDN_LD_H1(8) LDN_LD_H1(14) LDN_LD_H1(20) LDN_LD_H1(26) break;
-                        case 6: LDN_LD_H1(3) LDN_LD_H1(9) LDN_LD_H1(15) LDN_LD_H1(21) LDN_LD_H1(27) break;
-                        case 7: LDN_LD_H1(4) LDN_LD_H1(10) LDN_LD_H1(16) LDN_LD_H1(22) break;
-                        default: LDN_LD_H1(5) LDN_LD_H1(11) LDN_LD_H1(17) LDN_LD_H1(23) break;
+                        case 3: LDN_LD_H1(0) LDN_LD_H1(6) LDN_LD_H1(12) LDN_LD_H1(18) LDN_LD_H1(24) LDN_LD_H1(30) LDN_LD_H1(36) break;
+                        case 4: LDN_LD_H1(1) LDN_LD_H1(7) LDN_LD_H1(13) LDN_LD_H1(19) LDN_LD_H1(25) LDN_LD_H1(31) LDN_LD_H1(37) break;
+                        case 5: LDN_LD_H1(2) LDN_LD_H1(8) LDN_LD_H1(14) LDN_LD_H1(20) LDN_LD_H1(26) LDN_LD_H1(32) LDN_LD_H1(38) break;
+                        case 6: LDN_LD_H1(3) LDN_LD_H1(9) LDN_LD_H1(15) LDN_LD_H1(21) LDN_LD_H1(27) LDN_LD_H1(33) LDN_LD_H1(39) break;
+                        case 7: LDN_LD_H1(4) LDN_LD_H1(10) LDN_LD_H1(16) LDN_LD_H1(22) LDN_LD_H1(28) LDN_LD_H1(34) LDN_LD_H1(40) break;
+                        default: LDN_LD_H1(5) LDN_LD_H1(11) LDN_LD_H1(17) LDN_LD_H1(23) LDN_LD_H1(29) LDN_LD_H1(35) LDN_LD_H1(41) break;
                     }
 #undef LDN_LD_H1
                 }
-                if (c > 0) { wait_vm_rt<62, 63>(pieces); ld_publish(sy, base2 + (unsigned)c); }
+                if (c > 0) { wait_vm_rt<62, 63>(pieces); ld_publish(sy, base2 + (unsigned)c, !BAND); }
             }
         }
 #endif
         wait_vm<0>();
-        ld_publish(sy, base2 + (unsigned)nchunks);
+        ld_publish(sy, base2 + (unsigned)nchunks, !BAND);
         LT(tb)
         LD_SPAN(2, ta, tb)
         __syncthreads();
@@ -595,7 +603,7 @@
                 if (cc >= R3) LD_TIMED(7, ld_wait_done(sy, ncomp, base3 + (unsigned)(cc - R3 + 1), dead))
                 store_chunk(s_w3 + slot3i * slot3);
                 slot3i = slot3i + 1 == R3 ? 0 : slot3i + 1;
-                ld_publish(sy, base3 + (unsigned)cc + 1u);
+                ld_publish(sy, base3 + (unsigned)cc + 1u, !BAND);
                 if (cc + 1 < nchunk3) load_chunk(cc + 1);
             }
         }
@@ -617,12 +625,12 @@
                 ld_dma_run<MAXP>(w3o, P2, p.w3p + (long)cc * (LD_CW * 8), lds_w3 + (unsigned)slot3i * (unsigned)slot3);
                 slot3i = slot3i + 1 == R3 ? 0 : slot3i + 1;
                 wait_vm_rt<62, 63>(P2);
-                ld_publish(sy, base3 + (unsigned)cc);
+                ld_publish(sy, base3 + (unsigned)cc, !BAND);
             }
             wait_vm<0>();
         }
 #endif
-        ld_publish(sy, base3 + (unsigned)nchunk3);
+        ld_publish(sy, base3 + (unsigned)nchunk3, !BAND);
         LT(tc)
         LD_SPAN(4, tb, tc)
         return;
@@ -630,7 +638,7 @@
 
     const int pm = wave * 32 + l31;
     const bool pvalid = pm < npix;
-    const int oy = pm / p.Wo, ox = pm % p.Wo;
+    const int oy = y0 + pm / p.Wo, ox = pm % p.Wo;
     const int cls = (((oy - 1 < 0) | ((oy + 1 >= p.Hi) << 1)) * 4 + ((ox - 1 < 0) | ((ox + 1 >= p.Wi) << 1)));
     if (consumer) {
 #pragma unroll
@@ -642,7 +650,7 @@
         for (int t = 0; t < 9; ++t) {
             const int iy = oy + t / 3 - 1, ix = ox + t % 3 - 1;
             const bool ok = pvalid && iy >= 0 && iy < p.Hi && ix >= 0 && ix < p.Wi;
-            trow[t] = ok ? iy * p.Wi + ix : ZR;
+            trow[t] = ok ? (iy - yin0) * p.Wi + ix : ZR;
         }
         const unsigned RL = (unsigned)Kp * 8u;
         unsigned arow[8];
@@ -943,7 +951,7 @@
 #pragma unroll
             for (int e = 0; e < 4; ++e) x[e] = fmaxf(x[e], 0.f);
             if (prow < npix) {
-                __builtin_nontemporal_store(x, reinterpret_cast<f32x4*>(p.out + (size_t)(pix0 + prow) * p.ldo + c0p + tcq * 4));
+                __builtin_nontemporal_store(x, reinterpret_cast<f32x4*>(p.out + (size_t)(out_row0 + prow) * p.ldo + c0p + tcq * 4));
                 csum += x;
             }
         }
@@ -954,7 +962,7 @@
             f32x4 csum = xr[0];
 #pragma unroll
             for (int e = 0; e < 4; ++e) csum[e] = sum_lane_bits_345(csum[e]);
-            if (trw == 0) *reinterpret_cast<f32x4*>(p.colsum + ((size_t)b * 8 + wave) * p.cout + c0p + tcq * 4) = csum;
+            if (trw == 0) *reinterpret_cast<f32x4*>(p.colsum + (gap_slot0 + wave) * p.cout + c0p + tcq * 4) = csum;
         }
     };
     for (int cc = 0; cc < nchunk3; ++cc) {
@@ -1002,7 +1010,7 @@
 #pragma unroll
         for (int it = 0; it < 4; ++it) {
             const int prow = wave * 32 + trw + 8 * it;
-            const float* src = (p.residual && prow < npix) ? p.residual + (size_t)(pix0 + prow) * p.ldr + c0 + tcq * 4 : g_tail_zero;
+            const float* src = (p.residual && prow < npix) ? p.residual + (size_t)(out_row0 + prow) * p.ldr + c0 + tcq * 4 : g_tail_zero;
             res[it] = __builtin_nontemporal_load(reinterpret_cast<const f32x4*>(src));
         }
         sh = ld_global_f4(p.sh3 + c0 + tcq * 4);
@@ -1017,7 +1025,7 @@
 #pragma unroll
         for (int it = 0; it < 4; ++it) {
             const int prow = wave * 32 + trw + 8 * it;
-            const float* src = (p.residual && prow < npix) ? p.residual + (size_t)(pix0 + prow) * p.ldr + c0 + tcq * 4 : g_tail_zero;
+            const float* src = (p.residual && prow < npix) ? p.residual + (size_t)(out_row0 + prow) * p.ldr + c0 + tcq * 4 : g_tail_zero;
 #if LDN_LD3_ABLATE & 3
             res[it] = f32x4{(float)prow, 0.f, 1.f, 2.f};
 #else
@@ -1101,7 +1109,7 @@
             for (int e = 0; e < 4; ++e) x[e] = fmaxf(x[e], 0.f);
             if (prow < npix) {
 #if !(LDN_LD3_ABLATE & 2)
-                __builtin_nontemporal_store(x, reinterpret_cast<f32x4*>(p.out + (size_t)(pix0 + prow) * p.ldo + c0 + tcq * 4));
+                __builtin_nontemporal_store(x, reinterpret_cast<f32x4*>(p.out + (size_t)(out_row0 + prow) * p.ldo + c0 + tcq * 4));
 #endif
                 csum += x;
             }
@@ -1109,7 +1117,7 @@
         if (p.colsum) {
 #pragma unroll
             for (int e = 0; e < 4; ++e) csum[e] = sum_lane_bits_345(csum[e]);
-            if (trw == 0) *reinterpret_cast<f32x4*>(p.colsum + ((size_t)b * 8 + wave) * p.cout + c0 + tcq * 4) = csum;
+            if (trw == 0) *reinterpret_cast<f32x4*>(p.colsum + (gap_slot0 + wave) * p.cout + c0 + tcq * 4) = csum;
         }
         asm volatile("s_waitcnt lgkmcnt(0)" ::: "memory");
         __builtin_amdgcn_wave_barrier();
@@ -1168,7 +1176,7 @@
             ha.w1s = uniform_ptr(cb->w1s); ha.n_idx = idx_i; ha.n_cnt = cnt_i;
             ha.sc1 = uniform_ptr(cb->sc1); ha.sh1 = uniform_ptr(cb->sh1); ha.ps1 = uniform_ptr(cb->ps1);
             ha.h1 = p.h1; ha.h1_row_bytes = p.h1_row_bytes; ha.pix_per_blk = HW; ha.mblocks = 1; ha.xs = nullptr;
-            head_ld<NS>(ha, b, smem, p.lds_total, opaque_tid(), q);
+            head_ld<NS>(ha, b, 0, smem, p.lds_total, opaque_tid(), q);
         }
         CT(c3)
         phase_fence();
@@ -1181,7 +1189,7 @@
             ta.sc2 = uniform_ptr(cb->sc2); ta.sh2 = uniform_ptr(cb->sh2); ta.ps2 = uniform_ptr(cb->ps2); ta.sh3 = uniform_ptr(cb->sh3);
             ta.residual = xin; ta.ldr = p.ldx; ta.out = p.x_work; ta.ldo = p.ldx; ta.colsum = p.colsum;
             ta.rows_per_blk = p.H; ta.mblocks = 1; ta.slice_bytes = p.slice_bytes; ta.pxs = nullptr; ta.pw = nullptr;
-            tail_ld<NS>(ta, b, smem, p.lds_total, opaque_tid(), q);
+            tail_ld<NS>(ta, b, 0, smem, p.lds_total, opaque_tid(), q);
         }
         CT(c5)
         phase_fence();
@@ -1202,4 +1210,37 @@
 #endif
 }
 
-}
+template <int NS>
+__global__ __launch_bounds__(512, 2) void k_head_ld(const HeadArgs p) {
+    extern __shared__ __attribute__((aligned(16))) unsigned char smem[];
+    LdSeq q;
+    q.base = 0u;
+    q.seen = 0u;
+#ifdef LDN_TRACE
+    for (int k = 0; k < 8; ++k) q.t[k] = 0;
+#endif
+    head_ld<NS, true>(p, blockIdx.x % p.B, blockIdx.x / p.B, smem, 160 * 1024, threadIdx.x, q);
+}
+
+template <int NS>
+__global__ __launch_bounds__(512, 2) void k_tail_ld(const TailArgs p) {
+    extern __shared__ __attribute__((aligned(16))) unsigned char smem[];
+    const int b = blockIdx.x % p.B, mb = blockIdx.x / p.B;
+    if (threadIdx.x < LD_SYNC_BYTES / 4) reinterpret_cast<unsigned*>(smem + LD_SYNC_OFF)[threadIdx.x] = 0u;
+    if (p.colsum) {
+        const int wave = threadIdx.x >> 6, lane = threadIdx.x & 63;
+        const int rows = min(p.rows_per_blk, p.Ho - mb * p.rows_per_blk);
+        if (wave >= ceil_div(rows * p.Wo, 32))
+            for (int c = lane * 4; c < p.cout; c += 256)
+                *reinterpret_cast<f32x4*>(p.colsum + ((size_t)b * (p.mblocks * 8) + mb * 8 + wave) * p.cout + c) = f32x4{0.f, 0.f, 0.f, 0.f};
+    }
+    LdSeq q;
+    q.base = 0u;
+    q.seen = 0u;
+#ifdef LDN_TRACE
+    for (int k = 0; k < 8; ++k) q.t[k] = 0;
+#endif
+    tail_ld<NS, true>(p, b, mb, smem, 160 * 1024, threadIdx.x, q);
+}
+
+}
diff --git a/laudnet_amd/csrc/ldn_tail.hip b/laudnet_amd/csrc/ldn_tail.hip
--- a/laudnet_amd/csrc/ldn_tail.hip
+++ b/laudnet_amd/csrc/ldn_tail.hip
@@ -1,6 +1,7 @@
 #include "ldn_common.h"
 #include "ldn_mlp.h"
 #include <type_traits>
+#include <atomic>
 #include <stdlib.h>
 
 namespace ldn {
@@ -20,6 +21,13 @@
     const unsigned char* pxs; const unsigned char* pw;
 };
 constexpr int T_PROJ_CIN = 64;
+
+struct HeadArgs;
+bool band_ld_on(bool is_tail);
+bool band_ld_head_fits(int pix_per_blk, int NS);
+bool band_ld_tail_fits(int R, int Hi, int Wi, int NS);
+template <int NS> static int launch_head_ld(HeadArgs& a, hipStream_t st);
+template <int NS> static int launch_tail_ld(TailArgs& a, hipStream_t st);
 
 __device__ __attribute__((aligned(16))) float g_tail_zero[4] = {0.f, 0.f, 0.f, 0.f};
 
@@ -675,6 +683,9 @@
     const int R = a.rows_per_blk;
     const int nr = tail_region_pixels(R, a.Hi, a.Wi, ST);
     a.slice_bytes = round_up((round_up(nr, 8) + 1) * 128, 1024);
+    if constexpr (ST == 1 && !PROJ && !F32 && NS >= 4) {
+        if (band_ld_on(true) && band_ld_tail_fits(R, a.Hi, a.Wi, NS)) return launch_tail_ld<NS>(a, st);
+    }
     const size_t lds2 = tail_lds2(R, a.Hi, a.Wi, NS, ST);
     const size_t lds3 = (size_t)T_KIDX_BYTES + 2 * (size_t)(W / 2 + (PROJ ? T_PROJ_CIN / 2 : 0)) * ((NS == 8 || PROJ) ? 32 : 64) * 8 + (size_t)18 * W * 4 + 8 * 4096;
     const size_t lds = lds2 > lds3 ? lds2 : lds3;
@@ -1287,6 +1298,9 @@
 
 template <int NS, bool F32 = false>
 static int launch_head(HeadArgs& a, hipStream_t st) {
+    if constexpr (!F32 && NS >= 4) {
+        if (a.xs == nullptr && band_ld_on(false) && band_ld_head_fits(a.pix_per_blk, NS)) return launch_head_ld<NS>(a, st);
+    }
     const size_t lds = 160 * 1024;
     LDN_REQUIRE(allow_dynamic_lds(reinterpret_cast<const void*>(&k_head<NS, F32>), lds), "k_head: cannot reserve %zu B of LDS", lds);
     hipLaunchKernelGGL((k_head<NS, F32>), dim3((unsigned)a.B * a.mblocks), dim3(512), lds, st, a);
@@ -1472,6 +1486,68 @@
     return lds2 <= lds && lds3 <= lds && ldsm <= lds && lds1 <= lds && round_up(nr, 8) / 8 <= 72;
 }
 
+static void arm_ld_fault_word(hipStream_t st) {
+    static std::atomic<bool> armed[64] = {};
+    int dev = 0;
+    hipStreamCaptureStatus cs = hipStreamCaptureStatusNone;
+    if (hipGetDevice(&dev) == hipSuccess && dev >= 0 && dev < 64 && !armed[dev].load(std::memory_order_relaxed) &&
+        hipStreamIsCapturing(st, &cs) == hipSuccess && cs == hipStreamCaptureStatusNone) {
+        int* d = fault_word_dev();
+        if (d && hipMemcpyToSymbol(HIP_SYMBOL(g_ld_fault_dev), &d, sizeof(d)) == hipSuccess) armed[dev].store(true, std::memory_order_relaxed);
+        else (void)hipGetLastError();
+    }
+}
+
+constexpr int BAND_LD_DEFAULT = 1;
+static std::atomic<int>& band_ld_state() {
+    static std::atomic<int> s{[] {
+        const char* e = getenv("LDN_BAND_LD");
+        if (!e || !*e) return BAND_LD_DEFAULT;
+        const int v = atoi(e);
+        return v >= 0 && v <= 3 ? v : BAND_LD_DEFAULT;
+    }()};
+    return s;
+}
+bool band_ld_on(bool is_tail) {
+    const int v = band_ld_state().load(std::memory_order_relaxed);
+    return v == 1 || v == (is_tail ? 3 : 2);
+}
+bool band_ld_head_fits(int pix_per_blk, int NS) {
+    const int W = NS * 32;
+    const int avail = 160 * 1024 - (LD_SYNC_OFF + LD_SYNC_BYTES + 3 * W * 4);
+    return NS >= 4 && pix_per_blk >= 1 && pix_per_blk <= 224 && (avail - 7 * 2 * 4096) / (W * 128) >= 2;
+}
+bool band_ld_tail_fits(int R, int Hi, int Wi, int NS) {
+    const int W = NS * 32;
+    if (NS < 4 || R < 1 || R * Wi > 224) return false;
+    const int nr = tail_region_pixels(R, Hi, Wi, 1);
+    if (round_up(nr, 8) / 8 > LD_BAND_MAXH) return false;
+    const int slice = round_up((round_up(nr, 8) + 1) * 128, 1024);
+    const int avail2 = 160 * 1024 - (LD_SYNC_OFF + LD_SYNC_BYTES) - 2 * slice;
+    const int avail3 = 160 * 1024 - (LD_SYNC_OFF + LD_SYNC_BYTES) - 18 * W * 4 - 7 * 4096;
+    return avail2 >= 2 * W * 128 && avail3 >= 2 * W * 128;
+}
+
+template <int NS>
+static int launch_head_ld(HeadArgs& a, hipStream_t st) {
+    const size_t lds = 160 * 1024;
+    arm_ld_fault_word(st);
+    LDN_REQUIRE(allow_dynamic_lds(reinterpret_cast<const void*>(&k_head_ld<NS>), lds), "k_head_ld: cannot reserve %zu B of LDS", lds);
+    hipLaunchKernelGGL((k_head_ld<NS>), dim3((unsigned)a.B * a.mblocks), dim3(512), lds, st, a);
+    LDN_CHECK_LAUNCH("k_head_ld");
+    return LDN_OK;
+}
+
+template <int NS>
+static int launch_tail_ld(TailArgs& a, hipStream_t st) {
+    const size_t lds = 160 * 1024;
+    arm_ld_fault_word(st);
+    LDN_REQUIRE(allow_dynamic_lds(reinterpret_cast<const void*>(&k_tail_ld<NS>), lds), "k_tail_ld: cannot reserve %zu B of LDS", lds);
+    hipLaunchKernelGGL((k_tail_ld<NS>), dim3((unsigned)a.B * a.mblocks), dim3(512), lds, st, a);
+    LDN_CHECK_LAUNCH("k_tail_ld");
+    return LDN_OK;
+}
+
 template <int NS, bool F32 = false>
 static int launch_chain(ChainArgs& a, hipStream_t st) {
     constexpr int W = NS * 32;
@@ -1483,17 +1559,7 @@
     if constexpr (!F32 && NS >= 4) {
         static const bool use_ld = [] { const char* e = getenv("LDN_CHAIN_LD"); return !(e && atoi(e) == 0); }();
         if (use_ld && nr <= 224) {
-            {
-                static bool armed[64] = {};
-                int dev = 0;
-                hipStreamCaptureStatus cs = hipStreamCaptureStatusNone;
-                if (hipGetDevice(&dev) == hipSuccess && dev >= 0 && dev < 64 && !armed[dev] && hipStreamIsCapturing(st, &cs) == hipSuccess &&
-                    cs == hipStreamCaptureStatusNone) {
-                    int* d = fault_word_dev();
-                    if (d && hipMemcpyToSymbol(HIP_SYMBOL(g_ld_fault_dev), &d, sizeof(d)) == hipSuccess) armed[dev] = true;
-                    else (void)hipGetLastError();
-                }
-            }
+            arm_ld_fault_word(st);
             LDN_REQUIRE(allow_dynamic_lds(reinterpret_cast<const void*>(&k_chain_ld<NS>), lds), "k_chain_ld: cannot reserve %zu B of LDS", lds);
             hipLaunchKernelGGL((k_chain_ld<NS>), dim3((unsigned)a.B), dim3(512), lds, st, a);
             LDN_CHECK_LAUNCH("k_chain_ld");
@@ -1532,6 +1598,30 @@
     return hipMemcpyToSymbol(HIP_SYMBOL(ldn::g_chain_stall), &image, sizeof(image)) == hipSuccess ? LDN_OK : LDN_EHIP;
 }
 #endif
+
+extern "C" int ldn_band_ld(int mode) {
+    std::atomic<int>& s = ldn::band_ld_state();
+    if (mode < 0 || mode > 3) return s.load(std::memory_order_relaxed);
+    return s.exchange(mode, std::memory_order_relaxed);
+}
+
+extern "C" int ldn_band_ld_form(int H, int W, int width, int stride, int f32, int is_tail) {
+    using namespace ldn;
+    if (H < 1 || W < 1 || (width != 64 && width != 128 && width != 256) || f32 || !band_ld_on(is_tail != 0)) return 0;
+    const int NS = width / 32;
+    if (!is_tail) {
+        const long HW = (long)H * W;
+        if (HW > (1L << 30)) return 0;
+        const int mblocks = ceil_div((int)HW, 256);
+        int ppb = ceil_div((int)HW, mblocks);
+        if (const int up = round_up(ppb, 32); up <= 256 && (long)up * (mblocks - 1) < HW) ppb = up;
+        return band_ld_head_fits(ppb, NS) ? 1 : 0;
+    }
+    if (stride != 1 || W > 256) return 0;
+    int mbk = 0;
+    const int R = tail_rows_per_block(H, W, NS, 1, &mbk);
+    return R > 0 && band_ld_tail_fits(R, H, W, NS) ? 1 : 0;
+}
 
 extern "C" int ldn_bottleneck_chain_fits(int H, int Wd, int C, int width, int hidden, int G) {
     if (H < 1 || Wd < 1 || H * Wd > 256 || C < 1 || G < 1 || hidden < 0 || (width != 64 && width != 128 && width != 256)) return 0;
diff --git a/laudnet_amd/ops.py b/laudnet_amd/ops.py
--- a/laudnet_amd/ops.py
+++ b/laudnet_amd/ops.py
@@ -961,6 +961,14 @@
     return bool(L.load().ldn_bottleneck_chain_fits(H, W, C, width, hidden, G))
 
 
+def band_ld(mode=-1):
+    return L.load().ldn_band_ld(int(mode))
+
+
+def band_ld_form(H, W, width, stride=1, f32=False, is_tail=True):
+    return bool(L.load().ldn_band_ld_form(H, W, width, stride, 1 if f32 else 0, 1 if is_tail else 0))
+
+
 def bottleneck_tail_splits(H, W, width, stride=1):
     return L.load().ldn_bottleneck_tail_splits(H, W, width, stride)
 
```

Result: no change. 22990 (-0.0%).
